# huggingface/distil-whisper

Measured on AMD Instinct MI355X. Metric: training audio-seconds/s (distil-large-v3 student, 30 s clips), higher is better.
Workload: dtype bf16

## Files before the change

### distil_whisper_amd/build.py

```python
import os
import subprocess
import sys

HERE = os.path.dirname(os.path.abspath(__file__))
CSRC = os.path.join(HERE, "csrc")
LIB = os.path.join(HERE, "libdwamd.so")
SOURCES = ["gemm.hip", "gemm_tile256.hip", "gemm_tile128.hip", "gemm_wp8_nn.hip", "gemm_wp8_nt.hip", "gemm_wp8_m320.hip", "gemm_wp8_m128.hip",
           "gemm_wp16_nn.hip", "gemm_wp16_tt.hip", "gemm_wp16_small.hip", "gemm_skinny.hip", "attention.hip", "norm.hip", "loss.hip", "logmel.hip", "elementwise.hip", "optim.hip", "decode.hip"]
FLAGS = ["--offload-arch=gfx950", "-O3", "-std=c++17", "-fPIC", "-ffp-contract=fast", "-munsafe-fp-atomics"]


def kernels_sha16() -> str:
    import hashlib
    h = hashlib.sha256()
    files = sorted(os.path.join(CSRC, f) for f in os.listdir(CSRC) if f.endswith((".hip", ".h")))
    files.append(os.path.join(HERE, "..", "include", "dwamd.h"))
    for f in files:
        h.update(os.path.basename(f).encode())
        with open(f, "rb") as fh:
            h.update(fh.read())
    return h.hexdigest()[:16]


def _stale(obj, deps):
    if not os.path.exists(obj):
        return True
    t = os.path.getmtime(obj)
    return any(os.path.getmtime(d) > t for d in deps)


def build(force: bool = False, verbose: bool = False) -> str:
    hipcc = os.environ.get("HIPCC", "/opt/rocm/bin/hipcc")
    objdir = os.path.join(HERE, "build")
    os.makedirs(objdir, exist_ok=True)
    headers = [os.path.join(CSRC, "common.h"), os.path.join(CSRC, "gemm_common.h"), os.path.join(CSRC, "gemm_kernel.h"), os.path.join(CSRC, "gemm_wp.h"), os.path.join(CSRC, "gemm_wp16.h"),
               os.path.join(HERE, "..", "include", "dwamd.h")]
    objs, procs = [], []
    flags = FLAGS + (["-DDW_ABLATE"] if os.environ.get("DW_ABLATE") else [])
    flags += os.environ.get("DW_EXTRA_FLAGS", "").split()
    for src in SOURCES:
        s = os.path.join(CSRC, src)
        o = os.path.join(objdir, src.replace(".hip", ".o"))
        objs.append(o)
        if force or _stale(o, [s] + headers):
            cmd = [hipcc] + flags + ["-c", s, "-o", o]
            if verbose:
                print(" ".join(cmd))
            procs.append((src, subprocess.Popen(cmd, stdout=subprocess.PIPE, stderr=subprocess.STDOUT)))
    for src, p in procs:
        out, _ = p.communicate()
        if p.returncode != 0:
            sys.stderr.write(out.decode())
            raise RuntimeError(f"hipcc failed on {src}")
    if force or procs or _stale(LIB, objs):
        cmd = [hipcc, "--offload-arch=gfx950", "-shared", "-fPIC", "-o", LIB] + objs
        subprocess.check_call(cmd)
    return LIB



if __name__ == "__main__":
    print(build(force="--force" in sys.argv, verbose=True))
```

### distil_whisper_amd/csrc/gemm.hip

```cpp
#include "gemm_common.h"
#include <mutex>
#include <unordered_map>

bool dw_gemm_skinny_ok(const GemmP& p, int trans_a, int trans_b);
int dw_gemm_skinny_launch(const GemmP& p, hipStream_t s);
int dw_gemm_tile256_launch(const GemmP& p, int ta, int tb, hipStream_t s);
int dw_gemm_tile128_launch(const GemmP& p, int ta, int tb, hipStream_t s);
int dw_gemm_wp8_nn_launch(const GemmP& p, hipStream_t s);
int dw_gemm_wp8_nt_launch(const GemmP& p, hipStream_t s);
int dw_gemm_wp8_nn320_launch(const GemmP& p, hipStream_t s);
int dw_gemm_wp8_nt320_launch(const GemmP& p, hipStream_t s);
int dw_gemm_wp8_nn128_launch(const GemmP& p, hipStream_t s);
int dw_gemm_wp8_nt128_launch(const GemmP& p, hipStream_t s);
int dw_gemm_wp16_nn_launch(const GemmP& p, hipStream_t s);
int dw_gemm_wp16_tt_launch(const GemmP& p, hipStream_t s);
int dw_gemm_wp16_nn_small_launch(const GemmP& p, hipStream_t s);
int dw_gemm_wp16_nt_small_launch(const GemmP& p, hipStream_t s);

extern int g_attn_bwd_stage;
extern int g_attn_decode;
extern int g_attn_ablate;
extern int g_attn_fwd_waves;
extern int g_attn_fwd_pipe;
extern int g_attn_plain_order;
extern int g_attn_defer;
extern int g_attn_bwd_waves;
extern int g_logmel_mfma;
extern int g_decode_fuse_off;
extern int g_skinny_wide;
extern int g_ln_variant;
enum { GEMM_RULE = 0,
       GEMM_REFERENCE = 1,
       GEMM_FORCE_320 = 2 };
static int g_gemm_mode = GEMM_RULE;
int g_gemm_strip = 0;
int g_gemm_cus = 256;
static int g_gemm_stage_next = 1;
static int g_gemm_dynamic = 1;
static int g_gemm_small_m = 1;
static int g_gemm_row_tail = 1;

static int* gemm_sched_slot(hipStream_t s) {
    static std::mutex mu;
    static std::unordered_map<hipStream_t, int*> slots;
    std::lock_guard<std::mutex> lock(mu);
    auto it = slots.find(s);
    if (it != slots.end()) return it->second;
    hipStreamCaptureStatus st = hipStreamCaptureStatusNone;
    if (hipStreamIsCapturing(s, &st) != hipSuccess || st != hipStreamCaptureStatusNone) { (void)hipGetLastError(); return nullptr; }
    int* ptr = nullptr;
    if (hipMalloc((void**)&ptr, 64) != hipSuccess || hipMemsetAsync(ptr, 0, 64, s) != hipSuccess) { (void)hipGetLastError(); return nullptr; }
    slots[s] = ptr;
    return ptr;
}
int g_gemm_strip_budget = 4;
extern "C" int dw_debug_set(int key, int value) {
    if (key == 0) { if (value < GEMM_RULE || value > GEMM_FORCE_320) return DW_EINVAL; g_gemm_mode = value; return DW_OK; }
    if (key == 1) { g_gemm_strip = value; return DW_OK; }
    if (key == 3) { g_attn_bwd_stage = value; return DW_OK; }
    if (key == 4) { g_attn_decode = value; return DW_OK; }
    if (key == 5) { g_logmel_mfma = value; return DW_OK; }
    if (key == 6) { g_gemm_strip_budget = value; return DW_OK; }
    if (key == 7) { g_decode_fuse_off = value; return DW_OK; }
    if (key == 8) { g_skinny_wide = value; return DW_OK; }
    if (key == 10) { g_gemm_dynamic = value; return DW_OK; }
    if (key == 11) { g_gemm_stage_next = value; return DW_OK; }
    if (key == 17) { g_attn_bwd_waves = value; return DW_OK; }
    if (key == 21) { g_ln_variant = value; return DW_OK; }
    if (key == 22) { g_gemm_row_tail = value; return DW_OK; }
    if (key == 25) { if (value < 0 || value > 1) return DW_EINVAL; g_gemm_small_m = value; return DW_OK; }
    if (key == 26) { g_attn_fwd_pipe = value; return DW_OK; }
    if (key == 18) { g_attn_plain_order = value; return DW_OK; }
    if (key == 23) { if (value < 0 || value > 64) return DW_EINVAL; g_attn_defer = value; return DW_OK; }
    if (key == 16) { g_attn_fwd_waves = value; return DW_OK; }
    if (key == 15) { g_attn_ablate = value; return DW_OK; }
    if (key == 9) { if (value < 8 || value > 256 || (value & 7)) return DW_EINVAL; g_gemm_cus = value; return DW_OK; }
    return DW_EINVAL;
}

__global__ __launch_bounds__(256) void reduce_slices_kernel(const float* part, long stride, int slices, float* out,
                                                            long n, int accumulate) {
    const long i = ((long)blockIdx.x * 256 + threadIdx.x) * 4;
    if (i >= n) return;
    f32x4 acc = accumulate ? *(const f32x4*)(out + i) : f32x4{0.f, 0.f, 0.f, 0.f};
    for (int s = 0; s < slices; ++s) {
        const f32x4 v = *(const f32x4*)(part + s * stride + i);
#pragma unroll
        for (int e = 0; e < 4; ++e) acc[e] += v[e];
    }
    *(f32x4*)(out + i) = acc;
}

extern "C" int dw_reduce_slices(const float* part, int64_t stride, int slices, float* out, int64_t n, int accumulate,
                                void* stream) {
    DW_CLEAR_ERR();
    if (!part || !out || slices < 1 || n <= 0 || (n & 3) || (stride & 3) || ((uintptr_t)part & 15) ||
        ((uintptr_t)out & 15))
        return DW_EINVAL;
    hipLaunchKernelGGL(reduce_slices_kernel, dim3((n / 4 + 255) / 256), dim3(256), 0, (hipStream_t)stream, part,
                       (long)stride, slices, out, (long)n, accumulate);
    DW_CHECK_LAUNCH();
    return DW_OK;
}

__global__ __launch_bounds__(256) void reduce_slices_ld_kernel(const float* part, long slice_stride, long ld_part, int slices,
                                                               float* out, long ld_out, int rows, int cols4, int accumulate) {
    const long i = (long)blockIdx.x * 256 + threadIdx.x;
    if (i >= (long)rows * cols4) return;
    const int r = (int)(i / cols4), c = (int)(i - (long)r * cols4) * 4;
    float* o = out + (long)r * ld_out + c;
    f32x4 acc = accumulate ? *(const f32x4*)o : f32x4{0.f, 0.f, 0.f, 0.f};
    const float* src = part + (long)r * ld_part + c;
    for (int s = 0; s < slices; ++s) {
        const f32x4 v = *(const f32x4*)(src + s * slice_stride);
#pragma unroll
        for (int e = 0; e < 4; ++e) acc[e] += v[e];
    }
    *(f32x4*)o = acc;
}
extern "C" int dw_reduce_slices_ld(const float* part, int64_t slice_stride, int64_t ld_part, int slices, float* out, int64_t ld_out,
                                   int rows, int cols, int accumulate, void* stream) {
    DW_CLEAR_ERR();
    if (!part || !out || slices < 1 || rows <= 0 || cols <= 0 || (cols & 3) || (ld_part & 3) || (ld_out & 3) || (slice_stride & 3) ||
        ld_part < cols || ld_out < cols || ((uintptr_t)part & 15) || ((uintptr_t)out & 15))
        return DW_EINVAL;
    const long n = (long)rows * (cols / 4);
    hipLaunchKernelGGL(reduce_slices_ld_kernel, dim3((n + 255) / 256), dim3(256), 0, (hipStream_t)stream, part, (long)slice_stride,
                       (long)ld_part, slices, out, (long)ld_out, rows, cols / 4, accumulate);
    DW_CHECK_LAUNCH();
    return DW_OK;
}

enum GemmKernel {
    K_SKINNY,
    K_TILE128,
    K_TILE256,
    K_WP8_M128,
    K_WP16_SMALL,
    K_WP8_320,
    K_WP16_NN,
    K_WP8_NN,
    K_WP8_NT,
    K_WP16_TT,
};

static GemmKernel gemm_choose(const DwGemm* g, const GemmP& p) {
    const bool ta = g->trans_a, tb = g->trans_b, nn = !ta && !tb;
    const bool one_slice = p.split_k == 1 && !p.atomic;
    const bool ref = g_gemm_mode == GEMM_REFERENCE;
    const bool res_f32 = g->r && g->r_dtype == DW_F32 && g->c_dtype == DW_F32;
    const long cus = g_gemm_cus, tn = (g->n + 255) / 256;
    const long t256 = (long)((g->m + 255) / 256) * tn;
    const bool fits320 = !ta && one_slice && g->m % 320 == 0 && g->n % 256 == 0;
    int tile = g->tile;
    if ((tile == 0 || tile == 16) && dw_gemm_skinny_ok(p, ta, tb)) return K_SKINNY;
    bool one_round_320 = false, small_m_256 = false;
    if (tile != 128 && tile != 256) {
        tile = t256 >= 512 ? 256 : 128;
        if (tile == 128 && !ref && g_gemm_small_m && !ta && one_slice) {
            const long r128 = (((long)(g->m + 127) / 128) * tn + cus - 1) / cus;
            const long r256 = (t256 + cus - 1) / cus;
            const long r320 = fits320 ? ((long)(g->m / 320) * tn + cus - 1) / cus : 0;
            const long c128 = r128 * 100, c256 = r256 * 165, c320 = fits320 ? r320 * 205 : (1L << 40);
            if (c320 <= c128 && c320 <= c256) { tile = 256; one_round_320 = true; }
            else if (c256 <= c128) { tile = 256; small_m_256 = true; }
            else return K_WP8_M128;
        }
    }
    if (tile == 256 && g->tile != 256 && nn && res_f32 && g->k <= 1024 && one_slice) tile = 128;
    if (tile == 128) return K_TILE128;
    const long spanA = ta ? (long)g->k * g->lda * 2 : 256L * g->lda * 2 + (long)g->k * 2;
    const long spanB = tb ? (long)g->k * g->ldb * 2 : 256L * g->ldb * 2 + (long)g->k * 2;
    if (ref || spanA >= 0x7fffffffL || spanB >= 0x7fffffffL) return K_TILE256;
    if (small_m_256) return K_WP16_SMALL;
    if (fits320 && (one_round_320 || g_gemm_mode == GEMM_FORCE_320)) return K_WP8_320;
    if (nn && g->k <= 2560 && g->n >= 3840 && !g->r && !g->z_out && !g->zgrad_in && g->c_dtype != DW_F32) return K_WP16_NN;
    if (fits320) {
        const long r256 = (((g->m + 255) / 256) * tn + cus - 1) / cus * 4;
        const long r320 = ((g->m / 320) * tn + cus - 1) / cus * 5;
        if (tb ? r320 < r256 && !g->zgrad_in : r320 <= r256) return K_WP8_320;
    }
    if (nn) return res_f32 && g->k <= 2560 ? K_TILE256 : K_WP8_NN;
    if (!ta) return K_WP8_NT;
    if (tb) return K_WP16_TT;
    return K_TILE256;
}

extern "C" int dw_gemm_bf16(const DwGemm* g, void* stream) {
    DW_CLEAR_ERR();
    if (!g || (!g->a && !g->ln_x) || !g->b || !g->c) return DW_EINVAL;
    if (g->m <= 0 || g->n <= 0 || g->k <= 0 || (g->k & 63)) return DW_EINVAL;
    if ((g->lda & 7) || (g->ldb & 7)) return DW_EINVAL;
    if ((g->a && ((uintptr_t)g->a & 15)) || ((uintptr_t)g->b & 15)) return DW_EINVAL;
    if (g->trans_a && g->lda < ((g->m + 7) & ~7)) return DW_EINVAL;
    if (g->trans_b && g->ldb < ((g->n + 7) & ~7)) return DW_EINVAL;
    GemmP p;
    p.a = (const bf16*)g->a; p.b = (const bf16*)g->b; p.c = g->c; p.bias = g->bias;
    p.z_out = (bf16*)g->z_out; p.zgrad = (const bf16*)g->zgrad_in; p.r = g->r;
    p.lda = g->lda; p.ldb = g->ldb; p.ldc = g->ldc; p.ldz = g->ldz; p.ldzg = g->ldzg; p.ldr = g->ldr;
    p.m = g->m; p.n = g->n; p.k = g->k;
    p.act = g->act; p.c_dtype = g->c_dtype; p.r_dtype = g->r_dtype; p.r_row_mod = g->r_row_mod;
    p.round_res = g->round_res; p.tiles_n = 0; p.nwg = 0;
    p.split_k = g->split_k > 1 ? g->split_k : 1;
    p.atomic = g->atomic_acc ? 1 : 0;
    if (p.split_k > (g->k >> 6)) p.split_k = g->k >> 6;
    p.slice_stride = 0;
    p.sched = nullptr;
    p.zg_f16 = g->z_is_gelu_grad ? 1 : 0;
    p.colsum = g->colsum_out;
    if (g->colsum_out && (g->split_k > 1 || g->atomic_acc || ((uintptr_t)g->colsum_out & 3))) return DW_EINVAL;
    p.stage_next = g_gemm_stage_next;
    if (p.zg_f16 && g->z_out && g->act != 1) return DW_EINVAL;
    p.ln_x = g->ln_x; p.ln_g = g->ln_gamma; p.ln_b = g->ln_beta; p.ld_lnx = g->ld_lnx; p.ln_x_dtype = g->ln_x_dtype;
    p.ln_eps = g->ln_eps;
    p.kv_out = (bf16*)g->kv_out; p.kv_ld = g->kv_ld; p.kv_split = g->kv_split; p.kv_rpb = g->kv_rows_per_batch;
    p.kv_pitch = g->kv_batch_pitch; p.kv_row0 = g->kv_row0;
    const bool fused = g->ln_x || g->kv_out;
    if (g->ln_x && (!g->ln_gamma || !g->ln_beta || g->k > 1280 || g->m > 32 || (g->ld_lnx & 7) ||
                    ((uintptr_t)g->ln_x & 15) || ((uintptr_t)g->ln_gamma & 15) || ((uintptr_t)g->ln_beta & 15)))
        return DW_EINVAL;
    if (g->kv_out && (g->c_dtype != DW_BF16 || g->act || g->r || g->z_out || g->zgrad_in || (g->kv_split & 15) ||
                      g->kv_split <= 0 || g->kv_split >= g->n || g->kv_rows_per_batch <= 0 || (g->kv_ld & 3) ||
                      ((uintptr_t)g->kv_out & 7)))
        return DW_EINVAL;
    if (p.split_k > 1 && !p.atomic) {
        if (g->c_dtype != DW_F32 || g->bias || g->z_out || g->zgrad_in || g->r || g->act || g->slice_stride <= 0)
            return DW_EINVAL;
        p.slice_stride = g->slice_stride;
    }
    if (p.atomic && (g->c_dtype != DW_F32 || g->bias || g->z_out || g->zgrad_in || g->r || g->act)) return DW_EINVAL;
    {
        const int es = g->c_dtype == DW_F32 ? 4 : 2;
        bool v = ((uintptr_t)g->c % (4 * es)) == 0 && (g->ldc & 3) == 0;
        if (g->bias) v = v && ((uintptr_t)g->bias & 15) == 0;
        if (g->z_out) v = v && ((uintptr_t)g->z_out & 7) == 0 && (g->ldz & 3) == 0;
        if (g->zgrad_in) v = v && ((uintptr_t)g->zgrad_in & 7) == 0 && (g->ldzg & 3) == 0;
        if (g->r) v = v && ((uintptr_t)g->r % (g->r_dtype == DW_F32 ? 16 : 8)) == 0 && (g->ldr & 3) == 0;
        p.vec = v ? 1 : 0;
    }
    hipStream_t s = (hipStream_t)stream;
    if (g->tile == 16 && !dw_gemm_skinny_ok(p, g->trans_a, g->trans_b)) return DW_EINVAL;
    const GemmKernel kern = gemm_choose(g, p);
    if (kern == K_SKINNY) {
        if (g->colsum_out) return DW_EINVAL;
        return dw_gemm_skinny_launch(p, s);
    }
    if (fused) return DW_EINVAL;
    if (g->tile == 129 && (g->trans_a || p.split_k != 1 || p.atomic)) return DW_EINVAL;
    if (kern == K_TILE128) return dw_gemm_tile128_launch(p, g->trans_a, g->trans_b, s);
    p.strip = g_gemm_strip;
    if (g_gemm_dynamic) p.sched = gemm_sched_slot(s);
    if (kern == K_WP8_M128) return g->trans_b ? dw_gemm_wp8_nt128_launch(p, s) : dw_gemm_wp8_nn128_launch(p, s);
    if (g->k <= 1024) p.stage_next |= 128;
    switch (kern) {
    case K_WP16_SMALL: return g->trans_b ? dw_gemm_wp16_nt_small_launch(p, s) : dw_gemm_wp16_nn_small_launch(p, s);
    case K_WP8_320: return g->trans_b ? dw_gemm_wp8_nt320_launch(p, s) : dw_gemm_wp8_nn320_launch(p, s);
    case K_WP8_NN: return dw_gemm_wp8_nn_launch(p, s);
    case K_WP8_NT: return dw_gemm_wp8_nt_launch(p, s);
    case K_WP16_TT: return dw_gemm_wp16_tt_launch(p, s);
    case K_WP16_NN: {
        const int tm_full = p.m / 256, rem = p.m - tm_full * 256;
        const long tn = (p.n + 255) / 256;
        const long rounds_all = ((long)(tm_full + 1) * tn + g_gemm_cus - 1) / g_gemm_cus;
        const long rounds_full = ((long)tm_full * tn + g_gemm_cus - 1) / g_gemm_cus;
        if (g_gemm_row_tail && g->tile != 256 && rem > 0 && rem <= 128 && tm_full > 0 && rounds_full < rounds_all && !p.colsum) {
            GemmP q1 = p, q2 = p;
            q1.m = tm_full * 256;
            const size_t es = p.c_dtype == DW_F32 ? 4 : 2;
            q2.m = rem;
            q2.a = p.a + (long)q1.m * p.lda;
            q2.c = (char*)p.c + (size_t)q1.m * p.ldc * es;
            q2.sched = nullptr;
            const int rc1 = dw_gemm_wp16_nn_launch(q1, s);
            if (rc1 != DW_OK) return rc1;
            return dw_gemm_tile128_launch(q2, 0, 0, s);
        }
        return dw_gemm_wp16_nn_launch(p, s);
    }
    default: return dw_gemm_tile256_launch(p, g->trans_a, g->trans_b, s);
    }
}
```

### distil_whisper_amd/csrc/gemm_common.h

```cpp
#pragma once
#include "common.h"
#include "../../include/dwamd.h"

struct GemmP {
    const bf16* a;
    const bf16* b;
    void* c;
    const float* bias;
    bf16* z_out;
    const bf16* zgrad;
    const void* r;
    long lda, ldb, ldc, ldz, ldzg, ldr;
    int m, n, k;
    int act, c_dtype, r_dtype, r_row_mod, round_res;
    int tiles_n, nwg;
    int strip;
    int split_k, atomic;
    int vec;
    long slice_stride;
    const void* ln_x;
    const float* ln_g;
    const float* ln_b;
    long ld_lnx;
    int ln_x_dtype;
    float ln_eps;
    bf16* kv_out;
    long kv_ld;
    int kv_split, kv_rpb, kv_pitch, kv_row0;
    int stage_next;
    int zg_f16;
    int* sched;
    float* colsum;
};

__device__ __forceinline__ void gemm_job_range(const GemmP& p, int& job_first, int& job_count, int& job_step) {
    const int total = p.nwg * p.split_k;
    const int bid = blockIdx.x;
    const int xcd = bid & 7, local = bid >> 3;
    const int q = total >> 3, r = total & 7;
    if ((int)gridDim.x == total) {
        job_first = (xcd < r ? xcd * (q + 1) : r * (q + 1) + (xcd - r) * q) + local;
        job_count = 1;
        job_step = 1;
    } else {
        const int start = xcd < r ? xcd * (q + 1) : r * (q + 1) + (xcd - r) * q;
        const int cnt = q + (xcd < r ? 1 : 0);
        job_step = gridDim.x >> 3;
        job_first = start + local;
        job_count = local < cnt ? (cnt - local + job_step - 1) / job_step : 0;
    }
}

struct GemmJobs {
    int start, cnt;
    int step, local;
    int cur;
    int iter;
    bool dynamic;
};
__device__ __forceinline__ int gemm_jobs_fetch(const GemmP& p) {
    return __hip_atomic_fetch_add(p.sched + (blockIdx.x & 7), 1, __ATOMIC_RELAXED, __HIP_MEMORY_SCOPE_AGENT);
}
__device__ __forceinline__ void gemm_jobs_begin(const GemmP& p, GemmJobs& J, int* slot) {
    const int total = p.nwg * p.split_k;
    const int bid = blockIdx.x;
    const int xcd = bid & 7;
    const int q = total >> 3, r = total & 7;
    J.start = xcd < r ? xcd * (q + 1) : r * (q + 1) + (xcd - r) * q;
    J.iter = 0;
    if ((int)gridDim.x == total) {
        J.cnt = q + (xcd < r ? 1 : 0);
        J.local = bid >> 3; J.step = J.cnt > 0 ? J.cnt : 1; J.cur = J.local; J.dynamic = false;
        J.cnt = J.local < J.cnt ? J.local + 1 : 0;
        return;
    }
    J.cnt = q + (xcd < r ? 1 : 0);
    J.step = gridDim.x >> 3;
    J.local = bid >> 3;
    J.dynamic = p.sched != nullptr;
    if (J.dynamic) {
        if (threadIdx.x == 0) slot[0] = gemm_jobs_fetch(p);
        __syncthreads();
        J.cur = slot[0];
    } else {
        J.cur = J.local;
    }
}
__device__ __forceinline__ void gemm_jobs_prefetch(const GemmP& p, GemmJobs& J, int* slot) {
    if (J.dynamic && threadIdx.x == 0) slot[(J.iter + 1) & 1] = gemm_jobs_fetch(p);
}
__device__ __forceinline__ void gemm_jobs_advance(GemmJobs& J, const int* slot) {
    ++J.iter;
    J.cur = J.dynamic ? slot[J.iter & 1] : J.cur + J.step;
}
__device__ __forceinline__ void gemm_jobs_end(const GemmP& p, const GemmJobs& J) {
    if (J.dynamic && threadIdx.x == 0) {
        const int done = __hip_atomic_fetch_add(p.sched + 8, 1, __ATOMIC_RELAXED, __HIP_MEMORY_SCOPE_AGENT);
        if (done == (int)gridDim.x - 1) {
#pragma unroll
            for (int i = 0; i < 9; ++i) __hip_atomic_store(p.sched + i, 0, __ATOMIC_RELAXED, __HIP_MEMORY_SCOPE_AGENT);
        }
    }
}

__device__ __forceinline__ void gemm_job_decode(const GemmP& p, int id, int& tm, int& tn, int& ks) {
    ks = id / p.nwg;
    id -= ks * p.nwg;
    const int tiles_m = p.nwg / p.tiles_n;
    const int nstrips = (p.tiles_n + p.strip - 1) / p.strip;
    const int sw = (p.tiles_n + nstrips - 1) / nstrips;
    const int per_strip = sw * tiles_m;
    int strip = id / per_strip;
    int within = id - strip * per_strip;
    int width = sw;
    const int full = p.tiles_n - (nstrips - 1) * sw;
    if (strip >= nstrips - 1) {
        strip = nstrips - 1;
        within = id - strip * per_strip;
        width = full;
    }
    tm = within / width;
    tn = strip * sw + (within - tm * width);
}

extern int g_gemm_strip_budget;
extern int g_gemm_cus;
inline int gemm_strip_width(int k, int tiles_n, int override_) {
    if (override_ > 0) return override_;
    const long tile_bytes = 256L * k * 2;
    int sw = (int)(((long)g_gemm_strip_budget << 19) / tile_bytes);
    if (sw < 2 || sw >= tiles_n) sw = tiles_n;
    return sw;
}

template <int BX>
__device__ __forceinline__ bf16x8 frag_kmajor(const char* tile, int x, int kk, int lane) {
    constexpr int RB = BX * 2;
    const int g = lane >> 4, p = lane & 15;
    const int col = x + ((g & 1) << 4) + ((p & 3) << 2);
    const int k0 = kk * 16 + ((g >> 1) << 3) + (p >> 2);
    const int ls = col >> 3;
    const int inb = (p & 1) << 3;
    const int sw = ((p >> 2) & 3) << 2;
    const char* a0 = tile + k0 * RB + ((ls ^ sw) << 4) + inb;
    const char* a1 = a0 + 4 * RB;
    bf16x4 lo = __builtin_amdgcn_ds_read_tr16_b64_v4bf16((lds_bf16x4_t*)a0);
    bf16x4 hi = __builtin_amdgcn_ds_read_tr16_b64_v4bf16((lds_bf16x4_t*)a1);
    bf16x8 r;
    r[0] = lo[0]; r[1] = lo[1]; r[2] = lo[2]; r[3] = lo[3];
    r[4] = hi[0]; r[5] = hi[1]; r[6] = hi[2]; r[7] = hi[3];
    return r;
}


typedef __attribute__((ext_vector_type(4))) unsigned u32x4;
enum { EPI_BIAS = 1, EPI_ZBF16 = 2, EPI_GELU = 4, EPI_STOREG = 8, EPI_ZG16 = 16, EPI_ZGBF = 32, EPI_RES = 64, EPI_RES_F32 = 128,
       EPI_ROUND = 256, EPI_OUT_F32 = 512, EPI_COLSUM = 1024 };
__device__ __forceinline__ int gemm_epi_flavour(const GemmP& p) {
    return (p.bias ? EPI_BIAS : 0) | ((p.z_out && !p.zg_f16) ? EPI_ZBF16 : 0) | (p.act == 1 ? EPI_GELU : 0) |
           ((p.z_out && p.zg_f16) ? EPI_STOREG : 0) | ((p.zgrad && p.zg_f16) ? EPI_ZG16 : 0) |
           ((p.zgrad && !p.zg_f16) ? EPI_ZGBF : 0) | (p.r ? EPI_RES : 0) | ((p.r && p.r_dtype == DW_F32) ? EPI_RES_F32 : 0) |
           ((p.r && p.round_res) ? EPI_ROUND : 0) | (p.c_dtype == DW_F32 ? EPI_OUT_F32 : 0) | (p.colsum ? EPI_COLSUM : 0);
}
template <class T>
__device__ __forceinline__ void gemm_store_out(T* dst, const T& v) {
    __builtin_nontemporal_store(v, dst);
}
template <int F = -1>
__device__ __forceinline__ void gemm_epi_vec4(const GemmP& p, float (&v)[4], const f32x4& b4, bool plain, bool have_side,
                                              const bf16x4& zs, const f32x4& rs, char* cdst, char* zdst, float (&cs)[4]) {
    constexpr bool RT = F < 0;
    const bool any = RT ? !plain : (F & ~(EPI_OUT_F32 | EPI_COLSUM)) != 0;
    const bool colsum = RT ? p.colsum != nullptr : bool(F & EPI_COLSUM);
    if (any) {
        if (RT || (F & EPI_BIAS)) {
#pragma unroll
            for (int e = 0; e < 4; ++e) v[e] += b4[e];
        }
        if (RT ? (p.z_out && !p.zg_f16) : bool(F & EPI_ZBF16)) {
            bf16x4 z4;
#pragma unroll
            for (int e = 0; e < 4; ++e) z4[e] = f2bf(v[e]);
            gemm_store_out((bf16x4*)zdst, z4);
        }
        if (RT ? p.act == 1 : bool(F & EPI_GELU)) {
            const bool store_g = RT ? (p.z_out && p.zg_f16) : bool(F & EPI_STOREG);
            f16x4 g4;
#pragma unroll
            for (int e = 0; e < 4; e += 2) {
                f32x2 vin; vin[0] = v[e]; vin[1] = v[e + 1];
                const f32x2 x2 = round_bf16_pair(vin);
                f32x2 y2, s2, pdf;
                gelu_y_s_pdf2(x2, y2, s2, pdf);
                v[e] = y2[0]; v[e + 1] = y2[1];
                if (store_g) {
                    const f32x2 g2 = gelu_cdf_from_s2(x2, s2) + x2 * pdf;
                    g4[e] = (_Float16)g2[0]; g4[e + 1] = (_Float16)g2[1];
                }
            }
            if (store_g) gemm_store_out((f16x4*)zdst, g4);
        }
        if (RT ? have_side : (F & (EPI_ZG16 | EPI_ZGBF | EPI_RES)) != 0) {
            if (RT ? (p.zgrad && p.zg_f16) : bool(F & EPI_ZG16)) {
                const f16x4 g4 = __builtin_bit_cast(f16x4, zs);
#pragma unroll
                for (int e = 0; e < 4; ++e) v[e] *= (float)g4[e];
            } else if (RT ? p.zgrad != nullptr : bool(F & EPI_ZGBF)) {
#pragma unroll
                for (int e = 0; e < 4; e += 2) {
                    f32x2 x2; x2[0] = bf2f(zs[e]); x2[1] = bf2f(zs[e + 1]);
                    const f32x2 g2 = gelu_grad_fast2(x2);
                    v[e] *= g2[0]; v[e + 1] *= g2[1];
                }
            }
            if (RT ? p.r != nullptr : bool(F & EPI_RES)) {
                float rv[4];
                if (RT ? p.r_dtype == DW_F32 : bool(F & EPI_RES_F32)) {
#pragma unroll
                    for (int e = 0; e < 4; ++e) rv[e] = rs[e];
                } else {
                    const unsigned u0 = __float_as_uint(rs[0]), u1 = __float_as_uint(rs[1]);
                    rv[0] = __uint_as_float(u0 << 16); rv[1] = __uint_as_float(u0 & 0xffff0000u);
                    rv[2] = __uint_as_float(u1 << 16); rv[3] = __uint_as_float(u1 & 0xffff0000u);
                }
                const bool rnd = RT ? p.round_res != 0 : bool(F & EPI_ROUND);
#pragma unroll
                for (int e = 0; e < 4; ++e) v[e] = (rnd ? round_bf16(v[e]) : v[e]) + rv[e];
            }
        }
    }
    if (RT ? p.c_dtype == DW_F32 : bool(F & EPI_OUT_F32)) {
        f32x4 o;
#pragma unroll
        for (int e = 0; e < 4; ++e) o[e] = v[e];
        *(f32x4*)cdst = o;
        if (colsum) {
#pragma unroll
            for (int e = 0; e < 4; ++e) cs[e] += v[e];
        }
    } else {
        bf16x4 o;
#pragma unroll
        for (int e = 0; e < 4; ++e) o[e] = f2bf(v[e]);
        gemm_store_out((bf16x4*)cdst, o);
        if (colsum) {
#pragma unroll
            for (int e = 0; e < 4; ++e) cs[e] += bf2f(o[e]);
        }
    }
}

template <int LPR>
__device__ __forceinline__ void gemm_colsum_flush(const GemmP& p, float (&cs)[4], int lane, int n) {
#pragma unroll
    for (int e = 0; e < 4; ++e) {
#pragma unroll
        for (int o = LPR; o < 64; o <<= 1) cs[e] += __shfl_xor(cs[e], o);
    }
    if (lane < LPR) {
#pragma unroll
        for (int e = 0; e < 4; ++e)
            if (n + e < p.n) atomicAdd(p.colsum + n + e, cs[e]);
    }
}

struct GemmNoHook { __device__ __forceinline__ void operator()() const {} };
__device__ __forceinline__ void gemm_lds_barrier() {
    asm volatile("s_waitcnt lgkmcnt(0)" ::: "memory");
    __builtin_amdgcn_s_barrier();
    asm volatile("" ::: "memory");
}
template <int FM, int FN, int TN, int PFDIST = 0, class Hook = GemmNoHook, bool SWZ = false, int LAY = 32, int JOFF = 0, class Acc = f32x16[FM][FN]>
__device__ __forceinline__ void gemm_epilogue(const GemmP& p, Acc& acc, char* smem, int wave, int lane,
                                              int m0_, int wm0_, int n0_, int wn0_, int ks_, Hook hook = Hook(),
                                              const float* lds_bias = nullptr) {
    static_assert(!SWZ || TN == 64, "swizzled patch: 16 slots of 16 bytes per row");
    asm volatile("" : "+v"(lane));
    const int m0 = __builtin_amdgcn_readfirstlane(m0_), wm0 = __builtin_amdgcn_readfirstlane(wm0_);
    const int n0 = __builtin_amdgcn_readfirstlane(n0_), wn0 = __builtin_amdgcn_readfirstlane(wn0_);
    const int ks = __builtin_amdgcn_readfirstlane(ks_);
    constexpr int PLD = SWZ ? TN : TN + 4;
    constexpr int LPR = TN / 4;
    constexpr int RPI = 64 / LPR;
    constexpr int NIT = 32 / RPI;
    float* patch = (float*)smem + wave * (32 * PLD);
    const int hi = lane >> 5, ln = lane & 31;
    const int lrow = LAY == 32 ? ln : (lane & 15);
    const int lcol = LAY == 32 ? hi * 4 : (lane >> 4) * 4;
    auto qrow = [](int q) constexpr -> int { return LAY == 32 ? 0 : (q / (FN * 2)) * 16; };
    auto qcol = [](int q) constexpr -> int { return LAY == 32 ? (q / 4) * 32 + (q % 4) * 8 : (q % (FN * 2)) * 16; };
    auto quad = [&](auto ic, auto qc) __attribute__((always_inline)) -> f32x4 {
        constexpr int i = decltype(ic)::value, q = decltype(qc)::value;
        f32x4 v4;
        if constexpr (LAY == 32) {
            constexpr int j = q / 4, g = q % 4;
            v4[0] = acc[i][j][g * 4 + 0]; v4[1] = acc[i][j][g * 4 + 1]; v4[2] = acc[i][j][g * 4 + 2]; v4[3] = acc[i][j][g * 4 + 3];
        } else {
            constexpr int h = q / (FN * 2), j = q % (FN * 2);
            v4 = acc[2 * i + h][j + JOFF];
        }
        return v4;
    };
    const bool plain = !p.bias && !p.z_out && p.act == 0 && !p.zgrad && !p.r;
    float* const cf = (float*)p.c + (long)ks * p.slice_stride;
    const int pr = lane / LPR, pc = (lane % LPR) * 4;
    const int n = n0 + wn0 + pc;
    const bool n_in = n < p.n;
    const bool full = p.vec && n + 3 < p.n;
    const bool interior = p.vec && !p.atomic && p.r_row_mod <= 0 && n0 + wn0 + TN <= p.n && m0 + wm0 + FM * 32 <= p.m;
    f32x4 b4 = {0.f, 0.f, 0.f, 0.f};
    if (p.bias && lds_bias && interior) b4 = *(const f32x4*)(lds_bias + wn0 + pc);
    else if (p.bias && n_in) {
        if (full) b4 = *(const f32x4*)(p.bias + n);
        else {
#pragma unroll
            for (int e = 0; e < 4; ++e) if (n + e < p.n) b4[e] = p.bias[n + e];
        }
    }
    auto to_patch = [&](auto ic) __attribute__((always_inline)) {
        int l2 = lane;
        asm volatile("" : "+v"(l2));
        const int lrow2 = LAY == 32 ? (l2 & 31) : (l2 & 15), lcol2 = LAY == 32 ? (l2 >> 5) * 4 : (l2 >> 4) * 4;
        static_for<0, FN * 4>([&](auto qc) __attribute__((always_inline)) {
            constexpr int q = decltype(qc)::value;
            const f32x4 v4 = quad(ic, qc);
            const int row = lrow2 + qrow(q), col = lcol2 + qcol(q);
            if constexpr (SWZ) *(f32x4*)(patch + row * PLD + (((col >> 2) ^ (row & 15)) << 2)) = v4;
            else *(f32x4*)(patch + row * PLD + col) = v4;
        });
    };

    if (interior) {
        const bool pf_z = p.zgrad != nullptr, pf_r = p.r != nullptr;
        constexpr int PFD = PFDIST > 0 ? (PFDIST < NIT ? PFDIST : NIT) : NIT;
        const int es_c = p.c_dtype == DW_F32 ? 4 : 2;
// ... 263 lines not shown
```

### distil_whisper_amd/csrc/gemm_wp.h

```cpp
#pragma once
#include "gemm_common.h"

#define PINF(f) asm volatile("" : "+v"((f)[0]), "+v"((f)[1]), "+v"((f)[2]), "+v"((f)[3]))
#define PINF2(f) asm volatile("" : "+v"((f)[0]), "+v"((f)[1]))
#define PIN_SET(set)                                                                                              \
    do {          \
        if constexpr (FM == 4 && FN == 2)                                                                                 \
            asm volatile("" : "+v"(af[set][0]), "+v"(af[set][1]), "+v"(af[set][2]), "+v"(af[set][3]), "+v"(bfr[set][0]), "+v"(bfr[set][1]));   \
        else if constexpr (FM == 5 && FN == 2)                                                                            \
            asm volatile("" : "+v"(af[set][0]), "+v"(af[set][1]), "+v"(af[set][2]), "+v"(af[set][3]), "+v"(af[set][4]), "+v"(bfr[set][0]),     \
                         "+v"(bfr[set][1]));                                                                              \
        else {                                                                                                            \
            if constexpr (FM == 4) PINF(af[set]);                                                                         \
            else if constexpr (FM == 5) { PINF(af[set]); asm volatile("" : "+v"(af[set][4])); }                          \
            else PINF2(af[set]);                                                                                          \
            if constexpr (FN == 4) PINF(bfr[set]); else PINF2(bfr[set]);                                                  \
        }                                                                                                                 \
    } while (0)

typedef __attribute__((ext_vector_type(4))) int i32x4_t;
__device__ __forceinline__ i32x4_t wp_rsrc(const void* base) {
    const unsigned long long a = (unsigned long long)base;
    i32x4_t r;
    r[0] = (int)(unsigned)a; r[1] = (int)((unsigned)(a >> 32) & 0xffffu); r[2] = 0x7fffffff; r[3] = 0x00020000;
    return r;
}
__device__ __forceinline__ void wp_dma16(const i32x4_t& rsrc, const char* lds_dst, unsigned voffset, int soffset) {
    const unsigned m0v = __builtin_amdgcn_readfirstlane((unsigned)(unsigned long long)(const lds_void_t*)lds_dst);
    asm volatile("s_mov_b32 m0, %0\n\ts_nop 0\n\tbuffer_load_dwordx4 %1, %2, %3 offen lds"
                 :: "s"(m0v), "v"(voffset), "s"(rsrc), "s"(soffset));
}
__device__ __forceinline__ unsigned wp_lds_addr(const void* lds_ptr) {
    return __builtin_amdgcn_readfirstlane((unsigned)(unsigned long long)(const lds_void_t*)lds_ptr);
}
__device__ __forceinline__ void wp_dma16u(const i32x4_t& rsrc, unsigned lds_addr, unsigned voffset, int soffset) {
    asm volatile("s_mov_b32 m0, %0\n\ts_nop 0\n\tbuffer_load_dwordx4 %1, %2, %3 offen lds"
                 :: "s"(lds_addr), "v"(voffset), "s"(rsrc), "s"(soffset));
}
template <int IMM>
__device__ __forceinline__ void wp_dma16p(const i32x4_t& rsrc, unsigned lds_base, unsigned voffset, int kbase, int piece_off) {
    int so;
    asm volatile("s_add_u32 m0, %1, %5\n\ts_add_u32 %0, %4, %6\n\tbuffer_load_dwordx4 %2, %3, %0 offen lds"
                 : "=&s"(so) : "s"(lds_base), "v"(voffset), "s"(rsrc), "s"(kbase), "i"(IMM), "s"(piece_off) : "scc");
}
template <int IMM>
__device__ __forceinline__ void wp_dma16i(const i32x4_t& rsrc, unsigned lds_base, unsigned voffset, int soffset) {
    asm volatile("s_add_u32 m0, %0, %4\n\ts_nop 0\n\tbuffer_load_dwordx4 %1, %2, %3 offen lds"
                 :: "s"(lds_base), "v"(voffset), "s"(rsrc), "s"(soffset), "i"(IMM) : "scc");
}

template <bool TA, bool TB, int WM, int WN, bool ASMDMA, int DBG, int BM, int NST>
__global__ __launch_bounds__(64 * WM * WN, WM * WN / 4) void gemm_wp_kernel(const GemmP p) {
    static_assert(ASMDMA && DBG == 0, "one build of the loop: inline-assembly operand DMA, no ablation");
    constexpr int BN = 256, NW = WM * WN, FM = BM / WM / 32, FN = BN / WN / 32, TN = BN / WN;
    static_assert(NST == 2 || (NST == 3 && BM < 256), "three stages: the 128-row tile");
    static_assert(NW * 32 * (TN + 4) * 4 <= 2 * (BM + BN) * 128, "epilogue patches must fit the operand buffers");
    static_assert(BM == 256 || !TA, "the k-major A image is built for 256-row tiles");
    constexpr int CPA = BM / 8 / NW, CPB = BN / 8 / NW;
    constexpr int CP = CPB;
    constexpr bool UNI = BM == 320;
    constexpr int EPF = 4;
    static_assert(CPA * 8 * NW == BM && CPB * 8 * NW == BN && CPA <= 8 && CPB <= 8, "piece split");
    constexpr int NA0 = (CPA + 1) / 2, NB0 = CPB / 2;
    constexpr int NH0 = NA0 + NB0, NH1 = CPA + CPB - NH0;
    constexpr int STAGE = (BM + BN) * 128;
    __shared__ __attribute__((aligned(1024))) char smem[NST * STAGE];
    __shared__ __attribute__((aligned(1024))) float bias_lds[BN];

    const int tid = threadIdx.x;
    const int lane = tid & 63;
    const int wave = __builtin_amdgcn_readfirstlane(tid >> 6);
    const int wm0 = (wave / WN) * (BM / WM), wn0 = (wave % WN) * TN;
    const unsigned smem_w = wp_lds_addr(smem) + (unsigned)(wave * 1024);

    __shared__ int job_slot[2];
    GemmJobs jobs;
    gemm_jobs_begin(p, jobs, job_slot);
    bool prefetched = false;
    while (jobs.cur < jobs.cnt) {
        int lane_k = lane;
        asm volatile("" : "+v"(lane_k));
        gemm_jobs_prefetch(p, jobs, job_slot);
        int tm, tn, ks;
        gemm_job_decode(p, jobs.start + jobs.cur, tm, tn, ks);
        const int m0 = tm * BM, n0 = tn * BN;

        unsigned offA[8], offB[8];
        const bf16* gA;
        const bf16* gB;
        int stepA, stepB;
        if (!TA) {
            gA = p.a + (long)m0 * p.lda;
            stepA = 128;
#pragma unroll
            for (int i = 0; i < CPA; ++i) {
                const int row = (wave + i * NW) * 8 + (lane_k >> 3);
                const int ls = (lane_k & 7) ^ swz7(row);
                const int grow = m0 + row < p.m ? row : p.m - 1 - m0;
                offA[i] = (unsigned)((grow * p.lda + ls * 8) * 2);
            }
        } else {
            gA = p.a + m0;
            stepA = 128 * (int)p.lda;
#pragma unroll
            for (int i = 0; i < CPA; ++i) {
                const int krow = (wave + i * NW) * 2 + (lane_k >> 5);
                const int ls = (lane_k & 31) ^ ((krow & 3) << 2);
                const int gcol = m0 + ls * 8 < p.m ? ls * 8 : 0;
                offA[i] = (unsigned)((krow * p.lda + gcol) * 2);
            }
        }
        if (!TB) {
            gB = p.b + (long)n0 * p.ldb;
            stepB = 128;
#pragma unroll
            for (int i = 0; i < CP; ++i) {
                const int row = (wave + i * NW) * 8 + (lane_k >> 3);
                const int ls = (lane_k & 7) ^ swz7(row);
                const int grow = n0 + row < p.n ? row : p.n - 1 - n0;
                offB[i] = (unsigned)((grow * p.ldb + ls * 8) * 2);
            }
        } else {
            gB = p.b + n0;
            stepB = 128 * (int)p.ldb;
#pragma unroll
            for (int i = 0; i < CP; ++i) {
                const int krow = (wave + i * NW) * 2 + (lane_k >> 5);
                const int ls = (lane_k & 31) ^ ((krow & 3) << 2);
                const int gcol = n0 + ls * 8 < p.n ? ls * 8 : 0;
                offB[i] = (unsigned)((krow * p.ldb + gcol) * 2);
            }
        }
        const int pieceA = UNI ? NW * (TA ? 2 : 8) * (int)p.lda * 2 : 0;
        const int pieceB = UNI ? NW * (TB ? 2 : 8) * (int)p.ldb * 2 : 0;
        int nt = p.k >> 6;
        {
            const int base = nt / p.split_k, rem = nt - base * p.split_k;
            const int first = ks * base + (ks < rem ? ks : rem);
            nt = base + (ks < rem ? 1 : 0);
            gA = (const bf16*)((const char*)gA + (long)first * stepA);
            gB = (const bf16*)((const char*)gB + (long)first * stepB);
        }
        const i32x4_t rsA = wp_rsrc(gA), rsB = wp_rsrc(gB);
        int kA = 0, kB = 0;

        f32x16 acc[FM][FN];
#pragma unroll
        for (int i = 0; i < FM; ++i)
#pragma unroll
            for (int j = 0; j < FN; ++j)
#pragma unroll
                for (int r = 0; r < 16; ++r) acc[i][j][r] = 0.f;

        auto dma1x = [&](const i32x4_t& ra, const i32x4_t& rb, auto hc, auto jc, int buf) __attribute__((always_inline)) {
            constexpr int h = decltype(hc)::value, j = decltype(jc)::value;
            constexpr int na = h ? CPA - NA0 : NA0, nb = h ? CPB - NB0 : NB0, nmin = na < nb ? na : nb;
            constexpr bool isA = j < 2 * nmin ? (j & 1) == 0 : na > nb;
            constexpr int idx = j < 2 * nmin ? j / 2 : j - nmin;
            constexpr int i = (isA ? (h ? NA0 : 0) : (h ? NB0 : 0)) + idx;
            static_assert(j < na + nb, "load index");
            const unsigned lb = smem_w + (unsigned)(buf * STAGE);
            if constexpr (UNI) {
                if constexpr (isA) wp_dma16p<i * (NW * 1024)>(ra, lb, offA[0], kA, i * pieceA);
                else wp_dma16p<i * (NW * 1024) + BM * 128>(rb, lb, offB[0], kB, i * pieceB);
            } else {
                if constexpr (isA) wp_dma16i<i * (NW * 1024)>(ra, lb, offA[i], kA);
                else wp_dma16i<i * (NW * 1024) + BM * 128>(rb, lb, offB[i], kB);
            }
        };
        auto dma1 = [&](auto hc, auto jc, int buf) __attribute__((always_inline)) { dma1x(rsA, rsB, hc, jc, buf); };
        auto dma = [&](auto hc, int buf) __attribute__((always_inline)) {
            static_for<0, (decltype(hc)::value ? NH1 : NH0)>([&](auto jc) __attribute__((always_inline)) { dma1(hc, jc, buf); });
        };
        bf16x8 af[2][FM], bfr[2][FN];
        auto frags = [&](auto sc, auto kc, int buf) {
            constexpr int set = decltype(sc)::value, kk = decltype(kc)::value;
            const char* tA = smem + buf * STAGE;
            const char* tB = tA + BM * 128;
#pragma unroll
            for (int i = 0; i < FM; ++i) {
                if (TA) af[set][i] = frag_kmajor<BM>(tA, wm0 + i * 32, kk, lane_k);
                else af[set][i] = frag_rows(tA, (wm0 >> 5) + i, kk, lane_k);
            }
#pragma unroll
            for (int j = 0; j < FN; ++j) {
                if (TB) bfr[set][j] = frag_kmajor<BN>(tB, wn0 + j * 32, kk, lane_k);
                else bfr[set][j] = frag_rows(tB, (wn0 >> 5) + j, kk, lane_k);
            }
        };
        auto mfma1 = [&](auto sc, auto qc) __attribute__((always_inline)) {
            constexpr int set = decltype(sc)::value, i = decltype(qc)::value / FN, j = decltype(qc)::value % FN;
            acc[i][j] = __builtin_amdgcn_mfma_f32_32x32x16_bf16(bfr[set][j], af[set][i], acc[i][j], 0, 0, 0);
        };
        auto substep = [&](auto sc, auto rc, auto vhc, int dbuf) __attribute__((always_inline)) {
            constexpr bool R = decltype(rc)::value != 0;
            constexpr int VH = decltype(vhc)::value;
            constexpr int NMF = FM * FN;
            constexpr int DSI = FM * (TA ? 2 : 1) + FN * (TB ? 2 : 1);
            constexpr int RG = VH ? NMF / 4 : NMF / 2;
            constexpr int PER = (DSI + RG - 1) / RG;
            constexpr int NLD = VH == 1 ? NH0 : NH1;
            static_assert(VH == 0 || RG + NLD <= NMF, "not enough MFMA gaps for the operand loads");
            static_for<0, RG>([&](auto qc) __attribute__((always_inline)) { mfma1(sc, qc); });
#pragma unroll
            for (int q = 0; q < RG; ++q) {
                __builtin_amdgcn_sched_group_barrier(0x8, 1, 0);
                if (R) __builtin_amdgcn_sched_group_barrier(0x100, PER, 0);
            }
            __builtin_amdgcn_sched_barrier(0);
            if constexpr (VH != 0) {
                static_for<0, NLD>([&](auto jc) __attribute__((always_inline)) {
                    mfma1(sc, std::integral_constant<int, RG + decltype(jc)::value>{});
                    dma1(std::integral_constant<int, VH - 1>{}, jc, dbuf);
                    __builtin_amdgcn_sched_barrier(0);
                });
                static_for<RG + NLD, NMF>([&](auto qc) __attribute__((always_inline)) { mfma1(sc, qc); });
            } else {
                static_for<RG, NMF>([&](auto qc) __attribute__((always_inline)) { mfma1(sc, qc); });
            }
            __builtin_amdgcn_sched_barrier(0);
        };
        using I0 = std::integral_constant<int, 0>;
        using I1 = std::integral_constant<int, 1>;
        using I2 = std::integral_constant<int, 2>;
        using I3 = std::integral_constant<int, 3>;

        const bool tile_in = m0 + BM <= p.m && n0 + BN <= p.n;
        if (p.bias && tile_in && wave == 0) glds16_so(p.bias + n0, (unsigned)lane_k * 16u, lds_addr_of(bias_lds));
        if constexpr (NST == 3) {
            dma(I0{}, 0); dma(I1{}, 0);
            kA += stepA; kB += stepB;
            if (nt > 1) { dma(I0{}, 1); dma(I1{}, 1); kA += stepA; kB += stepB; }
            if (nt > 2) dma(I0{}, 2);
            if (nt > 2) asm volatile("s_waitcnt vmcnt(%0)" :: "n"(2 * NH0 + NH1) : "memory");
            else if (nt > 1) asm volatile("s_waitcnt vmcnt(%0)" :: "n"(NH0 + NH1) : "memory");
            else wait_vm0();
            __syncthreads();
            frags(I0{}, I0{}, 0);
            __builtin_amdgcn_sched_barrier(0);
            auto body3 = [&](auto m1c, auto m2c, auto m3c, int b0, int b1, int b2) {
                constexpr bool M1 = decltype(m1c)::value, M2 = decltype(m2c)::value, M3 = decltype(m3c)::value;
                PIN_SET(0);
                frags(I1{}, I1{}, b0);
                if constexpr (M2) { substep(I0{}, I1{}, I2{}, b2); kA += stepA; kB += stepB; }
                else substep(I0{}, I1{}, I0{}, 0);
                PIN_SET(1);
                frags(I0{}, I2{}, b0);
                substep(I1{}, I1{}, I0{}, 0);
                PIN_SET(0);
                frags(I1{}, I3{}, b0);
                substep(I0{}, I1{}, I0{}, 0);
                PIN_SET(1);
                if constexpr (M1) {
                    if constexpr (M2) asm volatile("s_waitcnt vmcnt(%0)" :: "n"(NH0 + NH1) : "memory");
                    else wait_vm0();
                    __builtin_amdgcn_s_barrier();
                    __builtin_amdgcn_sched_barrier(0);
                }
                if constexpr (M1) frags(I0{}, I0{}, b1);
                if constexpr (M3) substep(I1{}, I1{}, I1{}, b0);
                else if constexpr (M1) substep(I1{}, I1{}, I0{}, 0);
                else substep(I1{}, I0{}, I0{}, 0);
            };
            int t = 0, b0 = 0, b1 = 1, b2 = 2;
            auto rot = [&]() { const int x = b0; b0 = b1; b1 = b2; b2 = x; ++t; };
            for (; t + 3 < nt; rot()) body3(std::true_type{}, std::true_type{}, std::true_type{}, b0, b1, b2);
            if (nt >= 3) { body3(std::true_type{}, std::true_type{}, std::false_type{}, b0, b1, b2); rot(); }
            if (nt >= 2) { body3(std::true_type{}, std::false_type{}, std::false_type{}, b0, b1, b2); rot(); }
            body3(std::false_type{}, std::false_type{}, std::false_type{}, b0, b1, b2);
        } else {
        if (!prefetched) { dma(I0{}, 0); dma(I1{}, 0); }
        kA += stepA; kB += stepB;
        if (nt > 1) dma(I0{}, 1);
        if (nt > 1) {
            if constexpr (NH0 == 8) asm volatile("s_waitcnt vmcnt(8)" ::: "memory");
            else if constexpr (NH0 == 5) asm volatile("s_waitcnt vmcnt(5)" ::: "memory");
            else if constexpr (NH0 == 3) asm volatile("s_waitcnt vmcnt(3)" ::: "memory");
            else { static_assert(NH0 == 4 || NH0 == 8 || NH0 == 5 || NH0 == 3, "vmcnt immediate"); asm volatile("s_waitcnt vmcnt(4)" ::: "memory"); }
        } else wait_vm0();
        __syncthreads();
        frags(I0{}, I0{}, 0);
        __builtin_amdgcn_sched_barrier(0);

        auto body = [&](auto m1c, auto m2c, int t) {
            constexpr bool MORE1 = decltype(m1c)::value, MORE2 = decltype(m2c)::value;
            const int buf = t & 1;
            PIN_SET(0);
            frags(I1{}, I1{}, buf);
            if constexpr (MORE1) { substep(I0{}, I1{}, I2{}, buf ^ 1); kA += stepA; kB += stepB; }
            else substep(I0{}, I1{}, I0{}, 0);
            PIN_SET(1);
            frags(I0{}, I2{}, buf);
            substep(I1{}, I1{}, I0{}, 0);
            PIN_SET(0);
            frags(I1{}, I3{}, buf);
            substep(I0{}, I1{}, I0{}, 0);
            PIN_SET(1);
            if constexpr (MORE1) {
                wait_vm0();
                __builtin_amdgcn_s_barrier();
                __builtin_amdgcn_sched_barrier(0);
            }
            if constexpr (MORE1) frags(I0{}, I0{}, buf ^ 1);
            if constexpr (MORE2) substep(I1{}, I1{}, I1{}, buf);
            else if constexpr (MORE1) substep(I1{}, I1{}, I0{}, 0);
            else substep(I1{}, I0{}, I0{}, 0);
        };
        int t = 0;
        for (; t + 2 < nt; ++t) body(std::true_type{}, std::true_type{}, t);
        if (nt >= 2) { body(std::true_type{}, std::false_type{}, t); ++t; }
        body(std::false_type{}, std::false_type{}, t);
        }

        prefetched = false;
        if constexpr (TN == 64 && BM >= 256) {
            const int nxt = jobs.dynamic ? job_slot[(jobs.iter + 1) & 1] : jobs.cur + jobs.step;
            if ((p.stage_next & 128) && (nt & 1) == 0 && nt >= 2 && nxt < jobs.cnt && tile_in && !p.zgrad && !p.r) {
                int tm2, tn2, ks2;
                gemm_job_decode(p, jobs.start + nxt, tm2, tn2, ks2);
                if ((tm2 + 1) * BM <= p.m && (tn2 + 1) * BN <= p.n) {
                    const int ntall = p.k >> 6, base2 = ntall / p.split_k, rem2 = ntall - base2 * p.split_k;
                    const long first2 = (long)ks2 * base2 + (ks2 < rem2 ? ks2 : rem2);
                    const char* a2 = (const char*)(TA ? p.a + tm2 * BM : p.a + (long)tm2 * BM * p.lda) + first2 * stepA;
                    const char* b2 = (const char*)(TB ? p.b + tn2 * BN : p.b + (long)tn2 * BN * p.ldb) + first2 * stepB;
                    const i32x4_t ra2 = wp_rsrc(a2), rb2 = wp_rsrc(b2);
                    kA = 0; kB = 0;
                    static_for<0, NH0>([&](auto jc) __attribute__((always_inline)) { dma1x(ra2, rb2, I0{}, jc, 0); });
                    static_for<0, NH1>([&](auto jc) __attribute__((always_inline)) { dma1x(ra2, rb2, I1{}, jc, 0); });
                    prefetched = true;
                }
            }
        }
        gemm_epilogue<FM, FN, TN, (BM == 320 ? EPF : 8), GemmNoHook, TN == 64>(p, acc, smem + (TN == 64 && STAGE >= NW * 8192 ? STAGE : 0), wave, lane, m0,
                                                                          wm0, n0, wn0, ks, GemmNoHook(), tile_in ? bias_lds : nullptr);
        gemm_lds_barrier();
        gemm_jobs_advance(jobs, job_slot);
    }
    gemm_jobs_end(p, jobs);
}

template <bool TA, bool TB, int WM, int WN, int BM = 256, int NST = 2>
static int launch_wp(const GemmP& p0, hipStream_t s) {
    GemmP p = p0;
    const int tiles_m = (p.m + BM - 1) / BM;
    p.tiles_n = (p.n + 255) / 256;
    p.nwg = tiles_m * p.tiles_n;
    p.strip = gemm_strip_width(p.k, p.tiles_n, p.strip);
    int nblk = p.nwg * p.split_k;
    if (nblk > g_gemm_cus) nblk = g_gemm_cus;
    hipLaunchKernelGGL((gemm_wp_kernel<TA, TB, WM, WN, true, 0, BM, NST>), dim3(nblk), dim3(64 * WM * WN), 0, s, p);
    DW_CHECK_LAUNCH();
    return DW_OK;
}
```

### distil_whisper_amd/csrc/norm.hip

```cpp
#include "common.h"
#include "../../include/dwamd.h"

#define LN_MAXV 8
#ifndef DW_NT_LN_IN
#define DW_NT_LN_IN 1
#endif

template <bool XBF>
__device__ __forceinline__ f32x4 ld4b(const void* x, long off) {
    if constexpr (DW_NT_LN_IN >= 2) {
        if (XBF) {
            const bf16x4 t = __builtin_nontemporal_load((const bf16x4*)((const bf16*)x + off));
            f32x4 r; r[0] = bf2f(t[0]); r[1] = bf2f(t[1]); r[2] = bf2f(t[2]); r[3] = bf2f(t[3]);
            return r;
        } else return __builtin_nontemporal_load((const f32x4*)((const float*)x + off));
    } else {
        if (XBF) {
            const bf16x4 t = *(const bf16x4*)((const bf16*)x + off);
            f32x4 r; r[0] = bf2f(t[0]); r[1] = bf2f(t[1]); r[2] = bf2f(t[2]); r[3] = bf2f(t[3]);
            return r;
        } else return *(const f32x4*)((const float*)x + off);
    }
}
template <bool XBF>
__device__ __forceinline__ f32x4 ld4(const void* x, long off) {
    if (XBF) {
        const bf16x4 t = *(const bf16x4*)((const bf16*)x + off);
        f32x4 r; r[0] = bf2f(t[0]); r[1] = bf2f(t[1]); r[2] = bf2f(t[2]); r[3] = bf2f(t[3]);
        return r;
    } else {
        return *(const f32x4*)((const float*)x + off);
    }
}

#ifndef DW_NT_LN
#define DW_NT_LN 0
#endif
template <class T>
__device__ __forceinline__ T ln_load_in(const T* src) {
    if constexpr (DW_NT_LN_IN != 0) return __builtin_nontemporal_load(src);
    else return *src;
}
template <int LEVEL, class T>
__device__ __forceinline__ void ln_store(T* dst, const T& v) {
    if constexpr (LEVEL <= DW_NT_LN) __builtin_nontemporal_store(v, dst);
    else *dst = v;
}

template <bool XBF, int NV>
__global__ __launch_bounds__(256) void ln_fwd_kernel(const void* x, const float* gamma, const float* beta, bf16* y,
                                                     float* mean, float* rstd, int rows, int cols, float eps, long ldx, long ldy) {
    const int lane = threadIdx.x & 63;
    const int row = blockIdx.x * 4 + (threadIdx.x >> 6);
    if (row >= rows) return;
    const int nvec = cols >> 2;
    f32x4 v[NV];
    float s = 0.f;
#pragma unroll
    for (int j = 0; j < NV; ++j) {
        const int idx = lane + 64 * j;
        if (idx < nvec) {
            v[j] = ld4<XBF>(x, (long)row * ldx + idx * 4);
            s += v[j][0] + v[j][1] + v[j][2] + v[j][3];
        }
    }
    s = wave_sum(s);
    const float mu = s / cols;
    float q = 0.f;
#pragma unroll
    for (int j = 0; j < NV; ++j) {
        const int idx = lane + 64 * j;
        if (idx < nvec) {
#pragma unroll
            for (int e = 0; e < 4; ++e) { const float d = v[j][e] - mu; q += d * d; }
        }
    }
    q = wave_sum(q);
    const float rs = rsqrtf(q / cols + eps);
#pragma unroll
    for (int j = 0; j < NV; ++j) {
        const int idx = lane + 64 * j;
        if (idx < nvec) {
            const f32x4 g = *(const f32x4*)(gamma + idx * 4);
            const f32x4 bt = *(const f32x4*)(beta + idx * 4);
            bf16x4 o;
#pragma unroll
            for (int e = 0; e < 4; ++e) o[e] = f2bf((v[j][e] - mu) * rs * g[e] + bt[e]);
            ln_store<1>((bf16x4*)(y + (long)row * ldy + idx * 4), o);
        }
    }
    if (lane == 0 && mean) { mean[row] = mu; rstd[row] = rs; }
}

template <int NV>
__global__ __launch_bounds__(256) void ln_fwd_persist_kernel(const float* x, const float* gamma, const float* beta, bf16* y,
                                                             float* mean, float* rstd, int rows, int cols, float eps, long ldx, long ldy) {
    const int lane = threadIdx.x & 63;
    const int nvec = cols >> 2;
    const int stride = gridDim.x * 4;
    int row = blockIdx.x * 4 + (threadIdx.x >> 6);
    if (row >= rows) return;
    f32x4 v[NV], nx[NV];
#pragma unroll
    for (int j = 0; j < NV; ++j) {
        const int idx = lane + 64 * j;
        if (idx < nvec) v[j] = ln_load_in((const f32x4*)(x + (long)row * ldx + idx * 4));
    }
    for (; row < rows; row += stride) {
        const int nrow = row + stride;
        if (nrow < rows) {
#pragma unroll
            for (int j = 0; j < NV; ++j) {
                const int idx = lane + 64 * j;
                if (idx < nvec) nx[j] = ln_load_in((const f32x4*)(x + (long)nrow * ldx + idx * 4));
            }
        }
        float s = 0.f;
#pragma unroll
        for (int j = 0; j < NV; ++j)
            if (lane + 64 * j < nvec) s += v[j][0] + v[j][1] + v[j][2] + v[j][3];
        s = wave_sum(s);
        const float mu = s / cols;
        float q = 0.f;
#pragma unroll
        for (int j = 0; j < NV; ++j)
            if (lane + 64 * j < nvec) {
#pragma unroll
                for (int e = 0; e < 4; ++e) { const float d = v[j][e] - mu; q += d * d; }
            }
        q = wave_sum(q);
        const float rs = rsqrtf(q / cols + eps);
#pragma unroll
        for (int j = 0; j < NV; ++j) {
            const int idx = lane + 64 * j;
            if (idx < nvec) {
                const f32x4 g = *(const f32x4*)(gamma + idx * 4);
                const f32x4 bt = *(const f32x4*)(beta + idx * 4);
                bf16x4 o;
#pragma unroll
                for (int e = 0; e < 4; ++e) o[e] = f2bf((v[j][e] - mu) * rs * g[e] + bt[e]);
                ln_store<1>((bf16x4*)(y + (long)row * ldy + idx * 4), o);
            }
        }
        if (lane == 0 && mean) { mean[row] = mu; rstd[row] = rs; }
#pragma unroll
        for (int j = 0; j < NV; ++j) v[j] = nx[j];
    }
}

template <int NV8>
__global__ __launch_bounds__(256) void ln_fwd_bf16x8_kernel(const bf16* x, const float* gamma, const float* beta, bf16* y,
                                                            float* mean, float* rstd, int rows, int cols, float eps, long ldx, long ldy) {
    const int lane = threadIdx.x & 63;
    const int row = blockIdx.x * 4 + (threadIdx.x >> 6);
    if (row >= rows) return;
    const int nvec = cols >> 3;
    float v[NV8][8];
    float s = 0.f;
#pragma unroll
    for (int j = 0; j < NV8; ++j) {
        const int idx = lane + 64 * j;
        if (idx < nvec) {
            const bf16x8 t = ln_load_in((const bf16x8*)(x + (long)row * ldx + idx * 8));
#pragma unroll
            for (int e = 0; e < 8; ++e) { v[j][e] = bf2f(t[e]); s += v[j][e]; }
        }
    }
    s = wave_sum(s);
    const float mu = s / cols;
    float q = 0.f;
#pragma unroll
    for (int j = 0; j < NV8; ++j) {
        const int idx = lane + 64 * j;
        if (idx < nvec) {
#pragma unroll
            for (int e = 0; e < 8; ++e) { const float d = v[j][e] - mu; q += d * d; }
        }
    }
    q = wave_sum(q);
    const float rs = rsqrtf(q / cols + eps);
#pragma unroll
    for (int j = 0; j < NV8; ++j) {
        const int idx = lane + 64 * j;
        if (idx < nvec) {
            const f32x4 g0 = *(const f32x4*)(gamma + idx * 8), g1 = *(const f32x4*)(gamma + idx * 8 + 4);
            const f32x4 b0 = *(const f32x4*)(beta + idx * 8), b1 = *(const f32x4*)(beta + idx * 8 + 4);
            bf16x8 o;
#pragma unroll
            for (int e = 0; e < 4; ++e) {
                o[e] = f2bf((v[j][e] - mu) * rs * g0[e] + b0[e]);
                o[e + 4] = f2bf((v[j][e + 4] - mu) * rs * g1[e] + b1[e]);
            }
            ln_store<1>((bf16x8*)(y + (long)row * ldy + idx * 8), o);
        }
    }
    if (lane == 0 && mean) { mean[row] = mu; rstd[row] = rs; }
}

template <bool XBF, int NV, int NW>
__global__ __launch_bounds__(NW * 64) void ln_bwd_kernel(const bf16* dy, const void* x, const float* mean,
                                                     const float* rstd, const float* gamma, float* dres,
                                                     int accumulate, float* dgamma, float* dbeta, bf16* dres_lowp,
                                                     float* dres_colsum, int rows, int cols, long lddy, long ldx, long lddres,
                                                         long ldlowp) {
    __shared__ float red[3 * NW * 512];
    const int lane = threadIdx.x & 63;
    const int wave = threadIdx.x >> 6;
    const int nvec = cols >> 2;
    f32x4 gm[NV], ag[NV], ab[NV], ac[NV];
#pragma unroll
    for (int j = 0; j < NV; ++j) {
        const int idx = lane + 64 * j;
#pragma unroll
        for (int e = 0; e < 4; ++e) { ag[j][e] = 0.f; ab[j][e] = 0.f; gm[j][e] = 0.f; ac[j][e] = 0.f; }
        if (idx < nvec) gm[j] = *(const f32x4*)(gamma + idx * 4);
    }
    for (int row = blockIdx.x * NW + wave; row < rows; row += gridDim.x * NW) {
        const float mu = mean[row], rs = rstd[row];
        f32x4 xh[NV], g[NV];
        float c1 = 0.f, c2 = 0.f;
#pragma unroll
        for (int j = 0; j < NV; ++j) {
            const int idx = lane + 64 * j;
            if (idx < nvec) {
                const f32x4 xv = ld4b<XBF>(x, (long)row * ldx + idx * 4);
                const f32x4 dv = ld4b<true>(dy, (long)row * lddy + idx * 4);
#pragma unroll
                for (int e = 0; e < 4; ++e) {
                    xh[j][e] = (xv[e] - mu) * rs;
                    g[j][e] = dv[e] * gm[j][e];
                    c1 += g[j][e];
                    c2 += g[j][e] * xh[j][e];
                    ag[j][e] += dv[e] * xh[j][e];
                    ab[j][e] += dv[e];
                }
            }
        }
        c1 = wave_sum(c1) / cols;
        c2 = wave_sum(c2) / cols;
#pragma unroll
        for (int j = 0; j < NV; ++j) {
            const int idx = lane + 64 * j;
            if (idx < nvec) {
                float* dst = dres + (long)row * lddres + idx * 4;
                f32x4 o;
#pragma unroll
                for (int e = 0; e < 4; ++e) o[e] = rs * (g[j][e] - c1 - xh[j][e] * c2);
                if (accumulate) {
                    const f32x4 old = *(const f32x4*)dst;
#pragma unroll
                    for (int e = 0; e < 4; ++e) o[e] += old[e];
                }
                ln_store<2>((f32x4*)dst, o);
                if (dres_lowp) {
                    bf16x4 lo;
#pragma unroll
                    for (int e = 0; e < 4; ++e) { lo[e] = f2bf(o[e]); ac[j][e] += bf2f(lo[e]); }
                    ln_store<3>((bf16x4*)(dres_lowp + (long)row * ldlowp + idx * 4), lo);
                }
            }
        }
    }
    float* r0 = red;
    float* r1 = red + NW * 512;
    float* r2 = red + 2 * NW * 512;
    for (int base = 0; base < cols; base += 512) {
#pragma unroll
        for (int j = 0; j < NV; ++j) {
            const int idx = lane + 64 * j;
            const int col = idx * 4;
            if (idx < nvec && col >= base && col < base + 512) {
#pragma unroll
                for (int e = 0; e < 4; ++e) {
                    r0[wave * 512 + (col - base) + e] = ag[j][e];
                    r1[wave * 512 + (col - base) + e] = ab[j][e];
                    r2[wave * 512 + (col - base) + e] = ac[j][e];
                }
            }
        }
        __syncthreads();
        for (int cidx = threadIdx.x; cidx < 512 && base + cidx < cols; cidx += NW * 64) {
            float sg = 0.f, sb = 0.f, sc = 0.f;
#pragma unroll
            for (int w = 0; w < NW; ++w) { sg += r0[w * 512 + cidx]; sb += r1[w * 512 + cidx]; sc += r2[w * 512 + cidx]; }
            atomicAdd(dgamma + base + cidx, sg);
            atomicAdd(dbeta + base + cidx, sb);
            if (dres_colsum) atomicAdd(dres_colsum + base + cidx, sc);
        }
        __syncthreads();
    }
}

template <bool XBF, int NV, int NW>
__global__ __launch_bounds__(NW * 64) void ln_bwd_pf_kernel(const bf16* dy, const void* x, const float* mean,
                                                         const float* rstd, const float* gamma, float* dres,
                                                         int accumulate, float* dgamma, float* dbeta, bf16* dres_lowp,
                                                         float* dres_colsum, int rows, int cols, long lddy, long ldx, long lddres,
                                                         long ldlowp) {
    __shared__ float red[3 * NW * 512];
    const int lane = threadIdx.x & 63;
    const int wave = threadIdx.x >> 6;
    const int nvec = cols >> 2;
    f32x4 gm[NV], ag[NV], ab[NV], ac[NV];
#pragma unroll
    for (int j = 0; j < NV; ++j) {
        const int idx = lane + 64 * j;
#pragma unroll
        for (int e = 0; e < 4; ++e) { ag[j][e] = 0.f; ab[j][e] = 0.f; gm[j][e] = 0.f; ac[j][e] = 0.f; }
        if (idx < nvec) gm[j] = *(const f32x4*)(gamma + idx * 4);
    }
    const int stride = gridDim.x * NW;
    int row = blockIdx.x * NW + wave;
    f32x4 xv[NV], dv[NV];
    float mu = 0.f, rs = 0.f;
    if (row < rows) {
        mu = mean[row]; rs = rstd[row];
#pragma unroll
        for (int j = 0; j < NV; ++j) {
            const int idx = lane + 64 * j;
            if (idx < nvec) { xv[j] = ld4b<XBF>(x, (long)row * ldx + idx * 4); dv[j] = ld4b<true>(dy, (long)row * lddy + idx * 4); }
        }
    }
    for (; row < rows; row += stride) {
        const int nrow = row + stride;
        f32x4 old[NV], nxv[NV], ndv[NV];
        float nmu = 0.f, nrs = 0.f;
        if (accumulate) {
#pragma unroll
            for (int j = 0; j < NV; ++j) {
                const int idx = lane + 64 * j;
                if (idx < nvec) old[j] = *(const f32x4*)(dres + (long)row * lddres + idx * 4);
            }
        }
        if (nrow < rows) {
            nmu = mean[nrow]; nrs = rstd[nrow];
#pragma unroll
            for (int j = 0; j < NV; ++j) {
                const int idx = lane + 64 * j;
                if (idx < nvec) { nxv[j] = ld4b<XBF>(x, (long)nrow * ldx + idx * 4); ndv[j] = ld4b<true>(dy, (long)nrow * lddy + idx * 4); }
            }
        }
        f32x4 xh[NV], g[NV];
        float c1 = 0.f, c2 = 0.f;
#pragma unroll
        for (int j = 0; j < NV; ++j) {
            const int idx = lane + 64 * j;
            if (idx < nvec) {
#pragma unroll
                for (int e = 0; e < 4; ++e) {
                    xh[j][e] = (xv[j][e] - mu) * rs;
                    g[j][e] = dv[j][e] * gm[j][e];
                    c1 += g[j][e];
                    c2 += g[j][e] * xh[j][e];
                    ag[j][e] += dv[j][e] * xh[j][e];
                    ab[j][e] += dv[j][e];
                }
            }
        }
        c1 = wave_sum(c1) / cols;
        c2 = wave_sum(c2) / cols;
#pragma unroll
        for (int j = 0; j < NV; ++j) {
            const int idx = lane + 64 * j;
            if (idx < nvec) {
                float* dst = dres + (long)row * lddres + idx * 4;
                f32x4 o;
#pragma unroll
                for (int e = 0; e < 4; ++e) o[e] = rs * (g[j][e] - c1 - xh[j][e] * c2);
                if (accumulate) {
#pragma unroll
                    for (int e = 0; e < 4; ++e) o[e] += old[j][e];
                }
                ln_store<2>((f32x4*)dst, o);
                if (dres_lowp) {
                    bf16x4 lo;
#pragma unroll
                    for (int e = 0; e < 4; ++e) { lo[e] = f2bf(o[e]); ac[j][e] += bf2f(lo[e]); }
                    ln_store<3>((bf16x4*)(dres_lowp + (long)row * ldlowp + idx * 4), lo);
                }
            }
        }
        mu = nmu; rs = nrs;
#pragma unroll
        for (int j = 0; j < NV; ++j) { xv[j] = nxv[j]; dv[j] = ndv[j]; }
    }
    float* r0 = red;
    float* r1 = red + NW * 512;
    float* r2 = red + 2 * NW * 512;
    for (int base = 0; base < cols; base += 512) {
#pragma unroll
        for (int j = 0; j < NV; ++j) {
            const int idx = lane + 64 * j;
            const int col = idx * 4;
            if (idx < nvec && col >= base && col < base + 512) {
#pragma unroll
                for (int e = 0; e < 4; ++e) {
                    r0[wave * 512 + (col - base) + e] = ag[j][e];
                    r1[wave * 512 + (col - base) + e] = ab[j][e];
                    r2[wave * 512 + (col - base) + e] = ac[j][e];
                }
            }
        }
        __syncthreads();
        for (int cidx = threadIdx.x; cidx < 512 && base + cidx < cols; cidx += NW * 64) {
            float sg = 0.f, sb = 0.f, sc = 0.f;
#pragma unroll
            for (int w = 0; w < NW; ++w) { sg += r0[w * 512 + cidx]; sb += r1[w * 512 + cidx]; sc += r2[w * 512 + cidx]; }
            atomicAdd(dgamma + base + cidx, sg);
            atomicAdd(dbeta + base + cidx, sb);
            if (dres_colsum) atomicAdd(dres_colsum + base + cidx, sc);
        }
        __syncthreads();
    }
}

int g_ln_variant = 3;

extern "C" int dw_layernorm_fwd_ld(const void* x, int x_dtype, const float* gamma, const float* beta, void* y,
                                   float* mean, float* rstd, int rows, int cols, float eps, int64_t ldx_, int64_t ldy_, void* stream);
extern "C" int dw_layernorm_fwd(const void* x, int x_dtype, const float* gamma, const float* beta, void* y,
                                float* mean, float* rstd, int rows, int cols, float eps, void* stream) {
    return dw_layernorm_fwd_ld(x, x_dtype, gamma, beta, y, mean, rstd, rows, cols, eps, cols, cols, stream);
}
extern "C" int dw_layernorm_fwd_ld(const void* x, int x_dtype, const float* gamma, const float* beta, void* y,
                                   float* mean, float* rstd, int rows, int cols, float eps, int64_t ldx_, int64_t ldy_, void* stream) {
    DW_CLEAR_ERR();
    if (!x || !gamma || !beta || !y || rows <= 0 || cols <= 0 || (cols & 3) || cols > LN_MAXV * 256) return DW_EINVAL;
    if (ldx_ < cols || ldy_ < cols || (ldx_ & 3) || (ldy_ & 3)) return DW_EINVAL;
    const long ldx = ldx_, ldy = ldy_;
    if ((mean == nullptr) != (rstd == nullptr)) return DW_EINVAL;
    dim3 grid((rows + 3) / 4), block(256);
    hipStream_t s = (hipStream_t)stream;
    if (x_dtype == DW_BF16 && (cols & 7) == 0 && ((ldx | ldy) & 7) == 0 && ((uintptr_t)x & 15) == 0 && ((uintptr_t)y & 15) == 0 &&
        ((uintptr_t)gamma & 15) == 0 && ((uintptr_t)beta & 15) == 0) {
        const int nv8 = ((cols >> 3) + 63) / 64;
        if (nv8 <= 1) hipLaunchKernelGGL((ln_fwd_bf16x8_kernel<1>), grid, block, 0, s, (const bf16*)x, gamma, beta, (bf16*)y, mean, rstd, rows, cols, eps, ldx, ldy);
        else if (nv8 <= 2) hipLaunchKernelGGL((ln_fwd_bf16x8_kernel<2>), grid, block, 0, s, (const bf16*)x, gamma, beta, (bf16*)y, mean, rstd, rows, cols, eps, ldx, ldy);
        else if (nv8 <= 3) hipLaunchKernelGGL((ln_fwd_bf16x8_kernel<3>), grid, block, 0, s, (const bf16*)x, gamma, beta, (bf16*)y, mean, rstd, rows, cols, eps, ldx, ldy);
        else hipLaunchKernelGGL((ln_fwd_bf16x8_kernel<4>), grid, block, 0, s, (const bf16*)x, gamma, beta, (bf16*)y, mean, rstd, rows, cols, eps, ldx, ldy);
        DW_CHECK_LAUNCH();
        return DW_OK;
    }
    const int nv = ((cols >> 2) + 63) / 64;
    if ((g_ln_variant & 1) && x_dtype != DW_BF16 && nv <= 5 && rows >= 8192) {
        dim3 pg(256 * ((g_ln_variant >> 8) & 15 ? (g_ln_variant >> 8) & 15 : 5));
        hipLaunchKernelGGL((ln_fwd_persist_kernel<5>), pg, block, 0, s, (const float*)x, gamma, beta, (bf16*)y, mean, rstd, rows, cols, eps, ldx, ldy);
        DW_CHECK_LAUNCH();
        return DW_OK;
    }
#define LN_FWD(NVV)                                                                                                   \
    do {                                                                                                              \
        if (x_dtype == DW_BF16)                                                                                       \
            hipLaunchKernelGGL((ln_fwd_kernel<true, NVV>), grid, block, 0, s, x, gamma, beta, (bf16*)y, mean, rstd,   \
                               rows, cols, eps, ldx, ldy);                                                                      \
        else                                                                                                          \
            hipLaunchKernelGGL((ln_fwd_kernel<false, NVV>), grid, block, 0, s, x, gamma, beta, (bf16*)y, mean, rstd,  \
                               rows, cols, eps, ldx, ldy);                                                                      \
    } while (0)
    if (nv <= 2) LN_FWD(2); else if (nv <= 3) LN_FWD(3); else if (nv <= 5) LN_FWD(5); else LN_FWD(8);
#undef LN_FWD
    DW_CHECK_LAUNCH();
    return DW_OK;
}

extern "C" int dw_layernorm_bwd_ld(const void* dy, const void* x, int x_dtype, const float* mean, const float* rstd,
                                   const float* gamma, float* dres, int accumulate, float* dgamma, float* dbeta,
                                   void* dres_lowp, float* dres_colsum, int rows, int cols, int64_t lddy_, int64_t ldx_,
                                   int64_t lddres_, int64_t ldlowp_, void* stream);
extern "C" int dw_layernorm_bwd(const void* dy, const void* x, int x_dtype, const float* mean, const float* rstd,
                                const float* gamma, float* dres, int accumulate, float* dgamma, float* dbeta,
                                void* dres_lowp, float* dres_colsum, int rows, int cols, void* stream) {
    return dw_layernorm_bwd_ld(dy, x, x_dtype, mean, rstd, gamma, dres, accumulate, dgamma, dbeta, dres_lowp, dres_colsum, rows,
                               cols, cols, cols, cols, cols, stream);
}
extern "C" int dw_layernorm_bwd_ld(const void* dy, const void* x, int x_dtype, const float* mean, const float* rstd,
                                   const float* gamma, float* dres, int accumulate, float* dgamma, float* dbeta,
                                   void* dres_lowp, float* dres_colsum, int rows, int cols, int64_t lddy_, int64_t ldx_,
                                   int64_t lddres_, int64_t ldlowp_, void* stream) {
    DW_CLEAR_ERR();
    if (!dy || !x || !mean || !rstd || !gamma || !dres || !dgamma || !dbeta) return DW_EINVAL;
    if (rows <= 0 || cols <= 0 || (cols & 3) || cols > LN_MAXV * 256) return DW_EINVAL;
    if (lddy_ < cols || ldx_ < cols || lddres_ < cols || ldlowp_ < cols || ((lddy_ | ldx_ | lddres_ | ldlowp_) & 3)) return DW_EINVAL;
    const long lddy = lddy_, ldx = ldx_, lddres = lddres_, ldlowp = ldlowp_;
    hipStream_t s = (hipStream_t)stream;
    const int nv = ((cols >> 2) + 63) / 64;
#define LN_BWD(NVV, NWW)                                                                                              \
    do {                                                                                                              \
        int nb = (rows + NWW - 1) / NWW;                                                                              \
        const int resident = 256 * ((NVV <= 3 ? 16 : NVV <= 5 ? 12 : 4) / NWW);                                       \
        if (nb > resident) nb = resident;                                                                             \
        if (x_dtype == DW_BF16)                                                                                       \
            hipLaunchKernelGGL((ln_bwd_kernel<true, NVV, NWW>), dim3(nb), dim3(NWW * 64), 0, s, (const bf16*)dy, x,   \
                               mean, rstd, gamma, dres, accumulate, dgamma, dbeta, (bf16*)dres_lowp, dres_colsum,     \
                               rows, cols, lddy, ldx, lddres, ldlowp);                                                                           \
// ... 23 lines not shown
```

### distil_whisper_amd/engine.py

```python
from dataclasses import dataclass

import ctypes as C

import torch


@dataclass
class WhisperDims:
    d_model: int
    heads: int
    ffn: int
    enc_layers: int
    dec_layers: int
    vocab: int
    n_mels: int
    max_src: int = 1500
    max_tgt: int = 448
    pad_token_id: int = 50256
    decoder_start_token_id: int = 50257

    @staticmethod
    def from_any(c):
        if isinstance(c, WhisperDims):
            return c
        if hasattr(c, "encoder_attention_heads"):
            return WhisperDims(c.d_model, c.encoder_attention_heads, c.encoder_ffn_dim, c.encoder_layers,
                               c.decoder_layers, c.vocab_size, c.num_mel_bins, c.max_source_positions,
                               c.max_target_positions, c.pad_token_id, c.decoder_start_token_id)
        return WhisperDims(c.d_model, c.heads, c.ffn, c.enc_layers, c.dec_layers, c.vocab, c.n_mels, c.max_src,
                           c.max_tgt, c.pad_token_id, c.decoder_start_token_id)


def _rup(x, m):
    return (x + m - 1) // m * m


def layer_names(prefix, cross):
    blocks = ["self_attn", "encoder_attn"] if cross else ["self_attn"]
    out = []
    for b in blocks:
        out += [(f"{prefix}.{b}.q_proj.weight", "w"), (f"{prefix}.{b}.k_proj.weight", "w"),
                (f"{prefix}.{b}.v_proj.weight", "w"), (f"{prefix}.{b}.q_proj.bias", "b"),
                (f"{prefix}.{b}.k_proj.bias", "zero"), (f"{prefix}.{b}.v_proj.bias", "b"),
                (f"{prefix}.{b}.out_proj.weight", "w"), (f"{prefix}.{b}.out_proj.bias", "b"),
                (f"{prefix}.{b}_layer_norm.weight", "ln"), (f"{prefix}.{b}_layer_norm.bias", "ln")]
    out += [(f"{prefix}.fc1.weight", "w"), (f"{prefix}.fc1.bias", "b"), (f"{prefix}.fc2.weight", "w"),
            (f"{prefix}.fc2.bias", "b"), (f"{prefix}.final_layer_norm.weight", "ln"),
            (f"{prefix}.final_layer_norm.bias", "ln")]
    return out


class ParamStore:

    def __init__(self, ops, dims: WhisperDims, state_dict, trainable=False, frozen_prefixes=(), round_bf16=False):
        self.ops, self.dims, self.trainable = ops, dims, trainable
        D, Fd = dims.d_model, dims.ffn
        spec = [("model.encoder.conv1.weight", (D, dims.n_mels, 3), "conv"), ("model.encoder.conv1.bias", (D,), "b"),
                ("model.encoder.conv2.weight", (D, D, 3), "conv"), ("model.encoder.conv2.bias", (D,), "b"),
                ("model.encoder.embed_positions.weight", (dims.max_src, D), "frozen")]

        def shapes(name, kind):
            if kind == "w":
                if name.endswith("fc1.weight"):
                    return (Fd, D)
                if name.endswith("fc2.weight"):
                    return (D, Fd)
                return (D, D)
            if name.endswith("fc1.bias"):
                return (Fd,)
            return (D,)

        for i in range(dims.enc_layers):
            spec += [(n, shapes(n, k), k) for n, k in layer_names(f"model.encoder.layers.{i}", False)]
        spec += [("model.encoder.layer_norm.weight", (D,), "ln"), ("model.encoder.layer_norm.bias", (D,), "ln"),
                 ("model.decoder.embed_positions.weight", (dims.max_tgt, D), "emb")]
        for i in range(dims.dec_layers):
            spec += [(n, shapes(n, k), k) for n, k in layer_names(f"model.decoder.layers.{i}", True)]
        spec += [("model.decoder.layer_norm.weight", (D,), "ln"), ("model.decoder.layer_norm.bias", (D,), "ln"),
                 ("model.decoder.embed_tokens.weight", (dims.vocab, D), "emb")]

        def is_frozen(name, kind):
            if kind == "frozen" or not trainable:
                return True
            return any(name.startswith(pf) for pf in frozen_prefixes)

        ordered = [e for e in spec if is_frozen(e[0], e[2])] + [e for e in spec if not is_frozen(e[0], e[2])]
        self.entries, off = {}, 0
        self.train_start = None
        for name, shape, kind in ordered:
            if self.train_start is None and not is_frozen(name, kind):
                self.train_start = off
            n = 1
            for d in shape:
                n *= d
            self.entries[name] = (off, shape, kind)
            off += _rup(n, 64)
        self.train_end = off
        if self.train_start is None:
            self.train_start = off
        dec_offs = [o for n, (o, _, _) in self.entries.items() if n.startswith("model.decoder.") and o >= self.train_start]
        self.dec_start = min(dec_offs) if dec_offs else self.train_end
        total = off + 64 * max(D, 64)
        self.total = total
        self.P = ops.zeros((total,), torch.float32)
        self.S = ops.zeros((total,), ops.lowp)
        self.G = self.M = self.V = None
        if trainable and self.train_end > self.train_start:
            self.G = ops.zeros((total,), torch.float32)
            self.M = ops.zeros((total,), torch.float32)
            self.V = ops.zeros((total,), torch.float32)
        self.p, self.s, self.g = {}, {}, {}
        for name, (o, shape, kind) in self.entries.items():
            n = 1
            for d in shape:
                n *= d
            self.p[name] = self.P[o:o + n].view(shape)
            self.s[name] = self.S[o:o + n].view(shape)
            if self.G is not None and o >= self.train_start:
                self.g[name] = self.G[o:o + n].view(shape)
        self.small_grad_views = []
        if self.G is not None:
            rng = []
            for name, (o, shape, kind) in self.entries.items():
                if o < self.train_start or kind == "w":
                    continue
                n = 1
                for d in shape:
                    n *= d
                if rng and rng[-1][1] == o:
                    rng[-1][1] = o + _rup(n, 64)
                else:
                    rng.append([o, o + _rup(n, 64)])
            self.small_grad_views = [self.G[a:b] for a, b in rng]
        self.kpad1 = _rup(3 * dims.n_mels, 64)
        self.conv1_packed = ops.zeros((D, self.kpad1), ops.lowp)
        self.conv2_packed = ops.zeros((D, 3 * D), ops.lowp)
        self.load_state_dict(state_dict, round_bf16=round_bf16)

    def real_names(self):
        return [n for n, (_, _, k) in self.entries.items() if k != "zero"]

    def load_state_dict(self, sd, round_bf16=False):
        dev = self.P.device
        for name in self.real_names():
            src = sd[name].detach().to(device=dev, dtype=torch.float32)
            if round_bf16:
                src = src.to(torch.bfloat16).to(torch.float32)
            self.p[name].copy_(src)
        self.refresh_shadow()

    def state_dict(self):
        sd = {n: self.p[n].detach().clone() for n in self.real_names()}
        sd["proj_out.weight"] = sd["model.decoder.embed_tokens.weight"]
        return sd

    def refresh_shadow(self):
        self.ops.cast_bf16(self.P, out=self.S)
        self.repack_conv()

    def repack_conv(self):
        self.ops.pack_conv_weight(self.p["model.encoder.conv1.weight"], self.kpad1, out=self.conv1_packed)
        self.ops.pack_conv_weight(self.p["model.encoder.conv2.weight"], 3 * self.dims.d_model, out=self.conv2_packed)

    def is_trainable(self, name):
        return self.G is not None and self.entries[name][0] >= self.train_start

    def attn_views(self, prefix, cross_kv=False):
        D = self.dims.d_model
        oq = self.entries[f"{prefix}.q_proj.weight"][0]
        ob = self.entries[f"{prefix}.q_proj.bias"][0]
        assert self.entries[f"{prefix}.k_proj.weight"][0] == oq + D * D
        assert self.entries[f"{prefix}.v_proj.bias"][0] == ob + 2 * D
        v = {"wqkv": self.S[oq:oq + 3 * D * D].view(3 * D, D), "bqkv": self.P[ob:ob + 3 * D],
             "wo": self.s[f"{prefix}.out_proj.weight"], "bo": self.p[f"{prefix}.out_proj.bias"]}
        if self.is_trainable(f"{prefix}.q_proj.weight"):
            v["g_wqkv"] = self.G[oq:oq + 3 * D * D].view(3 * D, D)
            v["g_bqkv"] = self.G[ob:ob + 3 * D]
            v["g_wo"] = self.g[f"{prefix}.out_proj.weight"]
            v["g_bo"] = self.g[f"{prefix}.out_proj.bias"]
        return v

    def adam_segments(self, weight_decay, decay_filter=None):
        segs = []
        for name, (o, shape, kind) in self.entries.items():
            if o < self.train_start:
                continue
            n = 1
            for d in shape:
                n *= d
            wd = weight_decay if kind in ("w", "conv", "emb") else 0.0
            end = o + _rup(n, 64)
            if segs and segs[-1][2] == wd and segs[-1][1] == o:
                segs[-1] = (segs[-1][0], end, wd)
            else:
                segs.append((o, end, wd))
        return segs


class LiveRows:

    def __init__(self, idx, n, B, T, seq_start=None, seq_len=None, max_q=0, attn_flops=(0.0, 0.0)):
        self.idx, self.n, self.B, self.T = idx, int(n), int(B), int(T)
        self.seq_start, self.seq_len, self.max_q = seq_start, seq_len, int(max_q)
        self.attn_flops = attn_flops

    @staticmethod
    def seq_table(lens, T, fill_to=None, entries=None):
        lens = [max(1, min(int(T), int(x))) for x in lens]
        n_live = sum(lens)
        fill = max(0, int(fill_to) - n_live) if fill_to is not None else 0
        lens = lens + [min(T, fill - o) for o in range(0, fill, T)]
        if entries is not None:
            if len(lens) > entries:
                raise ValueError("LiveRows.seq_table: more filler sequences than the table holds")
            lens = lens + [0] * (entries - len(lens))
        ln = torch.tensor(lens, dtype=torch.int32)
        st = torch.cumsum(ln, 0, dtype=torch.int32) - ln
        return st, ln

    @staticmethod
    def host_index(lens, T, fill_to=None):
        lens = [max(1, min(int(T), int(x))) for x in lens]
        idx = torch.cat([b * T + torch.arange(n, dtype=torch.int32) for b, n in enumerate(lens)])
        if fill_to is not None and fill_to > idx.numel():
            need = int(fill_to) - idx.numel()
            dead = torch.cat([b * T + torch.arange(n, T, dtype=torch.int32) for b, n in enumerate(lens)])
            if dead.numel() < need:
                raise ValueError("LiveRows.host_index: not enough dead rows to fill the list")
            idx = torch.cat([idx, dead[:need]])
        return idx

    @classmethod
    def build(cls, lens, T, device):
        h = cls.host_index(lens, T)
        st, ln = cls.seq_table(lens, T)
        lf = ln.double()
        return cls(h.to(device), h.numel(), len(lens), T, st.to(device), ln.to(device), int(ln.max()),
                   attn_flops=(float((lf * lf).sum()), float(lf.sum())))


class WhisperEngine:

    def __init__(self, ops, store: ParamStore, stream_dtype=torch.float32):
        self.ops, self.st, self.dims = ops, store, store.dims
        self.stream = stream_dtype
        self.lowp = ops.lowp
        self.ldv = _rup(self.dims.vocab, 64)
        self.wgrad_stream = None
        self._wgrad_held, self._wgrad_fences = [], []
        self.pad_gemm_rows = False
        self.pad_gemm_rows_min = 2560
        self.pad_gemm_rows_slack = 1 / 32
        self.pad_lm_rows = True

    ffn_row_pad = 64
    row_pad = 64
    stream_row_pad = 128
    dx_row_pad = 64

    def act(self, rows, cols, dtype=None, zero_pad=True, pad=0):
        dtype = self.lowp if dtype is None else dtype
        rp = _rup(rows, 64)
        t = self.ops.empty((rp, cols + pad), dtype)
        if pad:
            t = t[:, :cols]
        if rp > rows and zero_pad:
            t[rows:].zero_()
        return t

    def _gemm_rows(self, R, save):
        if save or not self.pad_gemm_rows or R < self.pad_gemm_rows_min:
            return R
        Rg = _rup(R, 320)
        return Rg if Rg - R <= R * self.pad_gemm_rows_slack else R

    def _ln(self, name, x, R, save, rows_alloc=None, zero_pad=None, pad=0):
        y = self.act(R if rows_alloc is None else rows_alloc, x.shape[1], zero_pad=save if zero_pad is None else zero_pad, pad=pad)
        _, mu, rs = self.ops.layernorm_fwd(x[:R] if x.shape[0] != R else x, self.st.p[f"{name}.weight"],
                                           self.st.p[f"{name}.bias"], 1e-5, save_stats=save, out=y[:R])
        return y, mu, rs

    def _ln_bwd(self, name, dy, x, mu, rs, dres, R, emit=False, colsum_to=None):
        if self.st.is_trainable(f"{name}.weight"):
            dg, db = self.st.g[f"{name}.weight"], self.st.g[f"{name}.bias"]
        else:
            dg, db = self._scratch_vec(x.shape[1]), self._scratch_vec(x.shape[1], 1)
        nxt = self.act(R, x.shape[1], pad=self.row_pad) if emit else None
        dres = self.ops.layernorm_bwd(dy[:R], x[:R] if x.shape[0] != R else x, mu, rs, self.st.p[f"{name}.weight"],
                                      dres, dg, db, out_lowp=nxt[:R] if emit else None,
                                      colsum=colsum_to if emit else None)
        return dres, nxt

    def _train_scatter_buf(self, slot, rows, cols):
        if not hasattr(self, "_tsb"):
            self._tsb = {}
        fits = [b for b in self._tsb.get((slot, cols), []) if b.shape[0] >= rows]
        if fits:
            return min(fits, key=lambda b: b.shape[0])
        buf = self.ops.zeros((_rup(rows, 64), cols), self.lowp)
        self._tsb.setdefault((slot, cols), []).append(buf)
        return buf

    def _scatter_buf(self, rows, cols):
        if not hasattr(self, "_sb"):
            self._sb = {}
        fits = [b for b in self._sb.get(cols, []) if b.shape[0] >= rows]
        if fits:
            return min(fits, key=lambda b: b.shape[0])
        buf = self.ops.zeros((_rup(rows, 64), cols), self.lowp)
        self._sb.setdefault(cols, []).append(buf)
        return buf

    def _scratch_vec(self, n, slot=0):
        key = (n, slot)
        if not hasattr(self, "_sv"):
            self._sv = {}
        if key not in self._sv:
            self._sv[key] = self.ops.zeros((n,), torch.float32)
        return self._sv[key]

    def _wgrad(self, dy, x, gout, gbias, R, bias_cols=None):
        ws = self.wgrad_stream
        if ws is not None:
            main = torch.cuda.current_stream(dy.device)
            ws.wait_stream(main)
            with torch.cuda.stream(ws):
                self._wgrad_issue(dy, x, gout, gbias, R, bias_cols)
            self._wgrad_held += [dy, x]
        else:
            self._wgrad_issue(dy, x, gout, gbias, R, bias_cols)

    pack_train_layers = True
    varlen_attention = True
    wgrad_overwrite = False
    wgrad_lag = 2

    def _wgrad_fence(self):
        ws = self.wgrad_stream
        if ws is None or not (self._wgrad_held or self._wgrad_fences):
            return
        ev = torch.cuda.Event()
        ev.record(ws)
        self._wgrad_fences.append((ev, self._wgrad_held))
        self._wgrad_held = []
        while len(self._wgrad_fences) > self.wgrad_lag:
            ev, held = self._wgrad_fences.pop(0)
            torch.cuda.current_stream(self.st.P.device).wait_event(ev)
            held.clear()

    def _wgrad_issue(self, dy, x, gout, gbias, R, bias_cols):
        if gout is not None:
            self.ops.gemm(dy, x, trans_a=True, trans_b=True, out_dtype=torch.float32, out=gout, atomic_acc=True,
                          overwrite=self.wgrad_overwrite)
        if gbias is not None:
            if bias_cols is None:
                self.ops.colsum(dy[:R], gbias, accumulate=True)
            else:
                for lo, hi in bias_cols:
                    self.ops.colsum(dy[:R, lo:hi], gbias[lo:hi], accumulate=True)

    def join_wgrad_stream(self):
        if self.wgrad_stream is not None:
            torch.cuda.current_stream(self.st.P.device).wait_stream(self.wgrad_stream)
        self._wgrad_fences.clear()
        self._wgrad_held = []

    def encode(self, mel, save=False):
        ops, st, d = self.ops, self.st, self.dims
        B, _, T = mel.shape
        D, H = d.d_model, d.heads
        R1, R = B * T, B * T // 2
        L = T // 2
        ctx = {"B": B, "T": T, "R": R, "layers": []} if save else None
        xcol1 = self.act(R1, st.kpad1, zero_pad=save)
        ops.im2col_mel(mel, st.kpad1, out=xcol1[:R1])
        a1 = self.act(R1, D, zero_pad=save)
        _, z1 = ops.gemm(xcol1[:R1], st.conv1_packed, bias=st.p["model.encoder.conv1.bias"], act=1, want_z=True,
                         out=a1[:R1])
        xcol2 = self.act(R, 3 * D, zero_pad=save)
        ops.im2col_s2(a1[:R1], B, T, out=xcol2[:R])
        x = ops.empty((R, D), self.stream)
        _, z2 = ops.gemm(xcol2[:R], st.conv2_packed, bias=st.p["model.encoder.conv2.bias"], act=1, want_z=True,
                         residual=st.p["model.encoder.embed_positions.weight"], r_row_mod=L, round_res=True, out=x)
        if save:
            ctx.update(xcol1=xcol1, z1=z1, xcol2=xcol2, z2=z2)
        else:
            del xcol1, a1, z1, xcol2, z2
        for i in range(d.enc_layers):
            x, lc = self._layer_fwd(f"model.encoder.layers.{i}", x, B, L, None, 0, False, save)
            if save:
                ctx["layers"].append(lc)
        y, mu, rs = self._ln("model.encoder.layer_norm", x, R, save, zero_pad=True)
        if save:
            ctx.update(x_final=x, mu=mu, rs=rs, enc_out=y)
        return y, ctx

    def _layer_fwd(self, p, x, B, L, enc_out, Lk, causal, save, Rg=None, live=None):
        ops, st, d = self.ops, self.st, self.dims
        D, H, Rp = d.d_model, d.heads, B * L
        R = Rp if live is None else live.n
        Rg = R if Rg is None else Rg
        assert Rg == R or not save
        lc = {} if save else None
        rect = {}

        def attend(q_src, k, v, Lkv, is_causal, cols):
            o = self.act(Rg, D, zero_pad=save, pad=self.row_pad)
            if live is None:
                _, lse = ops.attn_fwd(q_src[:R, :D], k, v, B, H, L, Lkv, is_causal, 0.125, out=o[:R])
                return o, lse
            if save:
                tag = "x" if k is not None else "s"
                qp = self._train_scatter_buf((p, tag, "q"), Rp, cols)
                ops.scatter_rows(q_src[:R], live.idx, qp)
                op = self._train_scatter_buf((p, tag, "o"), Rp, D)
                kk, vv = (qp[:Rp, D:2 * D], qp[:Rp, 2 * D:]) if k is None else (k, v)
                _, lse = ops.attn_fwd(qp[:Rp, :D], kk, vv, B, H, L, Lkv, is_causal, 0.125, out=op[:Rp])
                ops.gather_rows(op, live.idx, o)
                rect[tag] = (qp, op)
                return o, lse
            if live.seq_start is not None and self.varlen_attention:
                if k is None:
                    ops.attn_fwd_varlen(q_src[:R, :D], q_src[:R, D:2 * D], q_src[:R, 2 * D:], H, live.max_q, live.seq_start,
                                        live.seq_len, is_causal, 0.125, o[:R], self_attention=True,
                                        flops=256.0 * H * live.attn_flops[0])
                else:
                    ops.attn_fwd_varlen(q_src[:R, :D], k, v, H, live.max_q, live.seq_start, live.seq_len, is_causal, 0.125, o[:R],
                                        Lk=Lkv, kv_batches=B, self_attention=False, flops=256.0 * H * Lkv * live.attn_flops[1])
                return o, None
            qp = self._scatter_buf(Rp, cols)
            ops.scatter_rows(q_src[:R], live.idx, qp)
            op = self.act(Rp, D, zero_pad=False)
            kk, vv = (qp[:Rp, D:2 * D], qp[:Rp, 2 * D:]) if k is None else (k, v)
            ops.attn_fwd(qp[:Rp, :D], kk, vv, B, H, L, Lkv, is_causal, 0.125, out=op[:Rp])
            ops.gather_rows(op, live.idx, o)
            return o, None
        av = st.attn_views(f"{p}.self_attn")
        h, mu, rs = self._ln(f"{p}.self_attn_layer_norm", x, R, save, Rg, pad=self.row_pad)
        qkv = self.act(Rg, 3 * D, zero_pad=save, pad=self.row_pad)
        ops.gemm(h[:Rg], av["wqkv"], bias=av["bqkv"], out=qkv[:Rg])
        if live is None:
            o, lse = attend(qkv, qkv[:R, D:2 * D], qkv[:R, 2 * D:], L, causal, 3 * D)
        else:
            o, lse = attend(qkv, None, None, L, causal, 3 * D)
        xp = self.stream_row_pad // (4 if self.stream == torch.float32 else 2)
        x1 = ops.gemm(o[:Rg], av["wo"], bias=av["bo"], residual=x, round_res=True, out_dtype=self.stream, out_row_pad=xp)
        if save:
            lc.update(x0=x, mu0=mu, rs0=rs, h0=h, qkv=qkv, o0=o, lse0=lse)
            if live is not None:
                lc.update(qkv_r=rect["s"][0], o0_r=rect["s"][1])
        x = x1
        if enc_out is not None:
            cv = st.attn_views(f"{p}.encoder_attn")
            Re = B * Lk
            h, mu, rs = self._ln(f"{p}.encoder_attn_layer_norm", x, R, save, Rg, pad=self.row_pad)
            q = self.act(Rg, D, zero_pad=save, pad=self.row_pad)
            ops.gemm(h[:Rg], cv["wqkv"][:D], bias=cv["bqkv"][:D], out=q[:Rg])
            kv = self.act(Re, 2 * D, zero_pad=save, pad=self.row_pad)
            ops.gemm(enc_out[:Re], cv["wqkv"][D:], bias=cv["bqkv"][D:], out=kv[:Re])
            o, lse = attend(q, kv[:Re, :D], kv[:Re, D:], Lk, False, D)
            x1 = ops.gemm(o[:Rg], cv["wo"], bias=cv["bo"], residual=x, round_res=True, out_dtype=self.stream, out_row_pad=xp)
            if save:
                lc.update(x1=x, mu1=mu, rs1=rs, h1=h, q1=q, kv1=kv, o1=o, lse1=lse)
                if live is not None:
                    lc.update(q1_r=rect["x"][0], o1_r=rect["x"][1])
            x = x1
        h, mu, rs = self._ln(f"{p}.final_layer_norm", x, R, save, Rg, pad=self.row_pad)
        a = self.act(Rg, d.ffn, zero_pad=save, pad=self.ffn_row_pad)
        res = ops.gemm(h[:Rg], st.s[f"{p}.fc1.weight"], bias=st.p[f"{p}.fc1.bias"], act=1,
                       want_z=("grad" if self.ffn_keeps_gelu_grad else True) if save else False, out=a[:Rg],
                       z_row_pad=self.ffn_row_pad)
        z = res[1] if save else None
        x2 = ops.gemm(a[:Rg], st.s[f"{p}.fc2.weight"], bias=st.p[f"{p}.fc2.bias"], residual=x, round_res=True,
                      out_dtype=self.stream, out_row_pad=xp)
        if save:
            lc.update(x2=x, mu2=mu, rs2=rs, h2=h, a=a, z=z)
        return x2, lc

    def decode(self, ids, enc_out, save=False, live=None):
        ops, st, d = self.ops, self.st, self.dims
        B, T = ids.shape
        R, Lk = B * T, d.max_src
        assert live is None or (live.B == B and live.T == T)
        ctx = {"B": B, "T": T, "R": R, "ids": ids, "layers": [], "enc_out": enc_out} if save else None
        packed = live is not None and (not save or self.pack_train_layers)
        if packed and not save and getattr(self, "_sb", None):
            for bufs in self._sb.values():
                for b_ in bufs:
                    b_.zero_()
        Rv = live.n if packed else R
        self._last_decode_rows = Rv
        Rg = self._gemm_rows(Rv, save)
        if self.stream == torch.float32:
            x = ops.embed_fwd(ids, st.p["model.decoder.embed_tokens.weight"],
                              st.p["model.decoder.embed_positions.weight"], torch.float32, rows_alloc=R if packed else Rg)
        else:
            x = ops.embed_fwd(ids, st.s["model.decoder.embed_tokens.weight"],
                              st.s["model.decoder.embed_positions.weight"], self.lowp, rows_alloc=R if packed else Rg)
        if packed:
            xp, x = x, ops.empty((Rg, d.d_model), self.stream)
            ops.gather_rows(xp, live.idx, x)
            del xp
        for i in range(d.dec_layers):
            x, lc = self._layer_fwd(f"model.decoder.layers.{i}", x, B, T, enc_out, Lk, True, save, Rg,
                                    live if packed else None)
            if save:
                ctx["layers"].append(lc)
        Rh = live.n if live is not None else R
        Rl = Rh
        if save and self.pad_lm_rows and Rh >= self.pad_gemm_rows_min:
            Rl = _rup(Rh, 320)
            Rl = Rl if Rl - Rh <= Rh * self.pad_gemm_rows_slack else Rh
        hf, mu, rs = self._ln("model.decoder.layer_norm", x, Rv, save, max(Rl, Rv))
        if live is not None and save and not packed:
            hfp, hf = hf, self.act(Rl, d.d_model)
            ops.gather_rows(hfp, live.idx, hf)
            del hfp
        logits = self.act(Rl, self.ldv, zero_pad=save)
        if Rl > Rh:
            hf[Rh:Rl].zero_()
            logits[Rh:Rl].zero_()
        eo = st.entries["model.decoder.embed_tokens.weight"][0]
        e_pad = st.S[eo:eo + self.ldv * d.d_model].view(self.ldv, d.d_model)
        ops.gemm(hf[:Rh], e_pad, out=logits[:Rh])
        if save:
            ctx.update(x_final=x, mu=mu, rs=rs, hf=hf, lm_rows=Rl, live=live, packed=packed, Rv=Rv)
        return logits, ctx

    def decode_init(self, enc_out, B, max_len, cache=None):
        ops, st, d = self.ops, self.st, self.dims
        D, Re = d.d_model, B * d.max_src
        if cache is None:
            cache = {"B": B, "max_len": max_len, "t": 0, "cross": [None] * d.dec_layers,
                     "self": [ops.zeros((B * max_len, 2 * D), self.lowp) for _ in range(d.dec_layers)]}
        assert cache["B"] == B and cache["max_len"] == max_len
        cache["t"] = 0
        for i in range(d.dec_layers):
            cv = st.attn_views(f"model.decoder.layers.{i}.encoder_attn")
            cache["cross"][i] = ops.gemm(enc_out[:Re], cv["wqkv"][D:], bias=cv["bqkv"][D:], out=cache["cross"][i],
                                         out_row_pad=self.kv_row_pad)
        return cache

    ffn_keeps_gelu_grad = True
    fuse_fc1_bias_grad = True
    fuse_attn_bias_grad = False
    use_c_decode = True
    kv_row_pad = 64

    def _decode_desc(self, cache, n):
        key = ("desc", n)
        if key in cache:
            return cache[key]
        from .ops_hip import DwDecodeStep, DwDecoderLayer, DW_BF16, DW_F32
        ops, st, d = self.ops, self.st, self.dims
        B, D, F = cache["B"], d.d_model, d.ffn
        rows = B * n
        f32 = self.stream == torch.float32
        tab = st.p if f32 else st.s
        ws = {"x": ops.empty((rows, D), self.stream), "h": ops.empty((rows, D), self.lowp),
              "qkv": ops.empty((rows, 3 * D), self.lowp), "o": ops.empty((rows, D), self.lowp),
              "a": ops.empty((rows, F), self.lowp), "logits": ops.empty((rows, self.ldv), self.lowp)}
        layers = (DwDecoderLayer * d.dec_layers)()
        keep = [ws]
        for i in range(d.dec_layers):
            p = f"model.decoder.layers.{i}"
            av, cv = st.attn_views(f"{p}.self_attn"), st.attn_views(f"{p}.encoder_attn")
            L = layers[i]
            L.ln1_g, L.ln1_b = st.p[f"{p}.self_attn_layer_norm.weight"].data_ptr(), st.p[f"{p}.self_attn_layer_norm.bias"].data_ptr()
            L.wqkv, L.bqkv = av["wqkv"].data_ptr(), av["bqkv"].data_ptr()
            L.wo, L.bo = av["wo"].data_ptr(), av["bo"].data_ptr()
            L.ln2_g, L.ln2_b = st.p[f"{p}.encoder_attn_layer_norm.weight"].data_ptr(), st.p[f"{p}.encoder_attn_layer_norm.bias"].data_ptr()
            L.wq, L.bq = cv["wqkv"][:D].data_ptr(), cv["bqkv"][:D].data_ptr()
            L.wo2, L.bo2 = cv["wo"].data_ptr(), cv["bo"].data_ptr()
            L.ln3_g, L.ln3_b = st.p[f"{p}.final_layer_norm.weight"].data_ptr(), st.p[f"{p}.final_layer_norm.bias"].data_ptr()
            L.w1, L.b1 = st.s[f"{p}.fc1.weight"].data_ptr(), st.p[f"{p}.fc1.bias"].data_ptr()
            L.w2, L.b2 = st.s[f"{p}.fc2.weight"].data_ptr(), st.p[f"{p}.fc2.bias"].data_ptr()
            L.self_kv, L.cross_kv = cache["self"][i].data_ptr(), cache["cross"][i].data_ptr()
            keep += [av, cv]
        eo = st.entries["model.decoder.embed_tokens.weight"][0]
        desc = DwDecodeStep()
        desc.batch, desc.n_new, desc.d_model, desc.heads, desc.ffn, desc.n_layers = B, n, D, d.heads, F, d.dec_layers
        desc.src_len, desc.max_len, desc.vocab, desc.ldv = d.max_src, cache["max_len"], d.vocab, self.ldv
        desc.stream_dtype = DW_F32 if f32 else DW_BF16
        desc.cross_kv_ld = cache["cross"][0].stride(0)
        assert all(c.stride(0) == desc.cross_kv_ld for c in cache["cross"])
        desc.tok_emb = tab["model.decoder.embed_tokens.weight"].data_ptr()
        desc.pos_emb = tab["model.decoder.embed_positions.weight"].data_ptr()
        desc.lnf_g, desc.lnf_b = st.p["model.decoder.layer_norm.weight"].data_ptr(), st.p["model.decoder.layer_norm.bias"].data_ptr()
        desc.lm_head = st.S[eo:eo + self.ldv * D].data_ptr()
        desc.layers = C.cast(layers, C.c_void_p)
        for k, v in ws.items():
            setattr(desc, k, v.data_ptr())
        cache[key] = (desc, ws, layers, keep)
        return cache[key]

    def _decode_pass_c(self, ids, cache, n):
        desc, ws, _, _ = self._decode_desc(cache, n)
        ids = ids.contiguous()
        desc.ids, desc.t = ids.data_ptr(), cache["t"]
        self.ops.decode_pass(desc)
        cache["t"] += n
        return ws["logits"]

    def _decoder_layers_cached(self, x, cache, n):
        ops, st, d = self.ops, self.st, self.dims
        B, t, ML = cache["B"], cache["t"], cache["max_len"]
        D, H, Lk = d.d_model, d.heads, d.max_src
        rows = B * n
        fuse_ln, fuse_kv = rows <= 32 and D <= 1280, rows <= 64
        causal = 2 if n > 1 else False
        for i in range(d.dec_layers):
            p = f"model.decoder.layers.{i}"
            av = st.attn_views(f"{p}.self_attn")
            ln1 = (st.p[f"{p}.self_attn_layer_norm.weight"], st.p[f"{p}.self_attn_layer_norm.bias"], 1e-5)
            kvc = cache["self"][i]
            h = x if fuse_ln else ops.layernorm_fwd(x, *ln1, save_stats=False)[0]
            qkv = ops.gemm(h, av["wqkv"], bias=av["bqkv"], ln=ln1[:2] if fuse_ln else None,
                           kv_append=(kvc, D, n, ML, t) if fuse_kv else None)
            if not fuse_kv:
                kvc.view(B, ML, 2 * D)[:, t:t + n].copy_(qkv[:, D:].view(B, n, 2 * D))
            o, _ = ops.attn_fwd(qkv[:, :D], kvc[:, :D], kvc[:, D:], B, H, n, t + n, causal, 0.125, kv_batch_rows=ML)
            x = ops.gemm(o, av["wo"], bias=av["bo"], residual=x, round_res=True, out_dtype=self.stream)
            cv = st.attn_views(f"{p}.encoder_attn")
            ln2 = (st.p[f"{p}.encoder_attn_layer_norm.weight"], st.p[f"{p}.encoder_attn_layer_norm.bias"], 1e-5)
            h = x if fuse_ln else ops.layernorm_fwd(x, *ln2, save_stats=False)[0]
            q = ops.gemm(h, cv["wqkv"][:D], bias=cv["bqkv"][:D], ln=ln2[:2] if fuse_ln else None)
            kv = cache["cross"][i]
            o, _ = ops.attn_fwd(q, kv[:, :D], kv[:, D:], B, H, n, Lk, False, 0.125)
            x = ops.gemm(o, cv["wo"], bias=cv["bo"], residual=x, round_res=True, out_dtype=self.stream)
            ln3 = (st.p[f"{p}.final_layer_norm.weight"], st.p[f"{p}.final_layer_norm.bias"], 1e-5)
            h = x if fuse_ln else ops.layernorm_fwd(x, *ln3, save_stats=False)[0]
            a = ops.gemm(h, st.s[f"{p}.fc1.weight"], bias=st.p[f"{p}.fc1.bias"], act=1, ln=ln3[:2] if fuse_ln else None)
            x = ops.gemm(a, st.s[f"{p}.fc2.weight"], bias=st.p[f"{p}.fc2.bias"], residual=x, round_res=True,
                         out_dtype=self.stream)
        return x

    def decode_step(self, ids_t, cache):
        ops, st, d = self.ops, self.st, self.dims
        B, t, ML = cache["B"], cache["t"], cache["max_len"]
        D, H, Lk = d.d_model, d.heads, d.max_src
        assert ids_t.shape == (B, 1) and t < ML and t < d.max_tgt
        if self.use_c_decode and hasattr(ops, "decode_pass"):
            return self._decode_pass_c(ids_t, cache, 1)
        f32 = self.stream == torch.float32
        tok = (st.p if f32 else st.s)["model.decoder.embed_tokens.weight"]
        pos = (st.p if f32 else st.s)["model.decoder.embed_positions.weight"][t:t + 1]
        x = ops.embed_fwd(ids_t.contiguous(), tok, pos, torch.float32 if f32 else self.lowp)
        x = self._decoder_layers_cached(x, cache, 1)
        hf, _, _ = ops.layernorm_fwd(x, st.p["model.decoder.layer_norm.weight"], st.p["model.decoder.layer_norm.bias"],
                                     1e-5, save_stats=False)
        eo = st.entries["model.decoder.embed_tokens.weight"][0]
        e_pad = st.S[eo:eo + self.ldv * D].view(self.ldv, D)
        logits = ops.gemm(hf, e_pad)
        cache["t"] = t + 1
        return logits

    def decode_multi(self, ids, cache):
        ops, st, d = self.ops, self.st, self.dims
        B, t, ML = cache["B"], cache["t"], cache["max_len"]
        n = ids.shape[1]
        D, H, Lk = d.d_model, d.heads, d.max_src
        assert ids.shape[0] == B and t + n <= ML and t + n <= d.max_tgt
        if self.use_c_decode and hasattr(ops, "decode_pass"):
            return self._decode_pass_c(ids, cache, n)
        f32 = self.stream == torch.float32
        tok = (st.p if f32 else st.s)["model.decoder.embed_tokens.weight"]
        pos = (st.p if f32 else st.s)["model.decoder.embed_positions.weight"][t:t + n]
        x = ops.embed_fwd(ids.contiguous(), tok, pos.contiguous(), torch.float32 if f32 else self.lowp)
        x = self._decoder_layers_cached(x, cache, n)
        hf, _, _ = ops.layernorm_fwd(x, st.p["model.decoder.layer_norm.weight"], st.p["model.decoder.layer_norm.bias"],
                                     1e-5, save_stats=False)
        eo = st.entries["model.decoder.embed_tokens.weight"][0]
        e_pad = st.S[eo:eo + self.ldv * D].view(self.ldv, D)
        logits = ops.gemm(hf, e_pad)
        cache["t"] = t + n
        return logits

    def _bias_grad(self, name):
        return self.st.g[name] if self.st.is_trainable(name) else None

    def _layer_bwd(self, p, lc, dres, dy, B, L, Lk, causal, denc, emit_last, colsum_last, live=None):
        ops, st, d = self.ops, self.st, self.dims
        D, H, Rp = d.d_model, d.heads, B * L
        R = Rp if live is None else live.n
        tr = st.is_trainable(f"{p}.fc1.weight")
        cross = "x1" in lc

        def to_rect(t, cols):
            r = ops.zeros((_rup(Rp, 64), cols), t.dtype)
            ops.scatter_rows(t[:R], live.idx, r)
            return r
        dz = self.act(R, d.ffn, pad=self.ffn_row_pad)
        fuse_cs = tr and self.fuse_fc1_bias_grad and R > 64
        ops.gemm(dy[:R], st.s[f"{p}.fc2.weight"], trans_b=True, zgrad=lc["z"], out=dz[:R],
                 colsum=st.g[f"{p}.fc1.bias"] if fuse_cs else None)
        if tr:
            self._wgrad(dy, lc["a"], st.g[f"{p}.fc2.weight"], None, R)
            self._wgrad(dz, lc["h2"], st.g[f"{p}.fc1.weight"], None if fuse_cs else st.g[f"{p}.fc1.bias"], R)
        dh = ops.gemm(dz[:R], st.s[f"{p}.fc1.weight"], trans_b=True, out_row_pad=self.dx_row_pad)
        nb = f"{p}.encoder_attn.out_proj.bias" if cross else f"{p}.self_attn.out_proj.bias"
        dres, dy = self._ln_bwd(f"{p}.final_layer_norm", dh, lc["x2"], lc["mu2"], lc["rs2"], dres, R, emit=True,
                                colsum_to=self._bias_grad(nb))
        del dz, dh
        if cross:
            cv = st.attn_views(f"{p}.encoder_attn")
            Re = B * Lk
            do = ops.gemm(dy[:R], cv["wo"], trans_b=True, out_row_pad=self.dx_row_pad)
            dq = self.act(R, D, pad=self.row_pad)
            dkv = self.act(Re, 2 * D, pad=self.row_pad)
            fb = tr and self.fuse_attn_bias_grad
            if live is None:
                ops.attn_bwd(lc["q1"][:R], lc["kv1"][:Re, :D], lc["kv1"][:Re, D:], lc["o1"][:R], do, lc["lse1"], B, H, L,
                             Lk, False, 0.125, dq=dq[:R], dk=dkv[:Re, :D], dv=dkv[:Re, D:],
                             dq_colsum=cv["g_bqkv"][:D] if fb else None, dv_colsum=cv["g_bqkv"][2 * D:] if fb else None)
            else:
                do_r = to_rect(do, D)
                dq_r = self.act(Rp, D, zero_pad=False)
                ops.attn_bwd(lc["q1_r"][:Rp], lc["kv1"][:Re, :D], lc["kv1"][:Re, D:], lc["o1_r"][:Rp], do_r[:Rp], lc["lse1"], B, H, L,
                             Lk, False, 0.125, dq=dq_r[:Rp], dk=dkv[:Re, :D], dv=dkv[:Re, D:],
                             dq_colsum=cv["g_bqkv"][:D] if fb else None, dv_colsum=cv["g_bqkv"][2 * D:] if fb else None)
                ops.gather_rows(dq_r, live.idx, dq)
                del do_r, dq_r
            if tr:
                self._wgrad(dy, lc["o1"], cv["g_wo"], None, R)
                self._wgrad(dq, lc["h1"], cv["g_wqkv"][:D], None if fb else cv["g_bqkv"][:D], R)
                self._wgrad(dkv, lc["enc_out"], cv["g_wqkv"][D:], None if fb else cv["g_bqkv"][D:], Re, bias_cols=[(D, 2 * D)])
            if denc is not None:
                ops.gemm(dkv[:Re], cv["wqkv"][D:], trans_b=True, residual=denc, round_res=True,
                         out_dtype=torch.float32, out=denc)
            dh = ops.gemm(dq[:R], cv["wqkv"][:D], trans_b=True, out_row_pad=self.dx_row_pad)
            dres, dy = self._ln_bwd(f"{p}.encoder_attn_layer_norm", dh, lc["x1"], lc["mu1"], lc["rs1"], dres, R,
                                    emit=True, colsum_to=self._bias_grad(f"{p}.self_attn.out_proj.bias"))
            del do, dq, dkv, dh
        av = st.attn_views(f"{p}.self_attn")
        do = ops.gemm(dy[:R], av["wo"], trans_b=True, out_row_pad=self.dx_row_pad)
        dqkv = self.act(R, 3 * D, pad=self.row_pad)
        qkv = lc["qkv"]
        fb = tr and self.fuse_attn_bias_grad
        if live is None:
            ops.attn_bwd(qkv[:R, :D], qkv[:R, D:2 * D], qkv[:R, 2 * D:], lc["o0"][:R], do, lc["lse0"], B, H, L, L, causal,
                         0.125, dq=dqkv[:R, :D], dk=dqkv[:R, D:2 * D], dv=dqkv[:R, 2 * D:],
                         dq_colsum=av["g_bqkv"][:D] if fb else None, dv_colsum=av["g_bqkv"][2 * D:] if fb else None)
        else:
            qr = lc["qkv_r"]
            do_r = to_rect(do, D)
            dqkv_r = self.act(Rp, 3 * D, zero_pad=False)
            ops.attn_bwd(qr[:Rp, :D], qr[:Rp, D:2 * D], qr[:Rp, 2 * D:], lc["o0_r"][:Rp], do_r[:Rp], lc["lse0"], B, H, L, L, causal,
                         0.125, dq=dqkv_r[:Rp, :D], dk=dqkv_r[:Rp, D:2 * D], dv=dqkv_r[:Rp, 2 * D:],
                         dq_colsum=av["g_bqkv"][:D] if fb else None, dv_colsum=av["g_bqkv"][2 * D:] if fb else None)
            ops.gather_rows(dqkv_r, live.idx, dqkv)
            del do_r, dqkv_r
        if tr:
            self._wgrad(dy, lc["o0"], av["g_wo"], None, R)
            self._wgrad(dqkv, lc["h0"], av["g_wqkv"], None if fb else av["g_bqkv"], R, bias_cols=[(0, D), (2 * D, 3 * D)])
        dh = ops.gemm(dqkv[:R], av["wqkv"], trans_b=True, out_row_pad=self.dx_row_pad)
        return self._ln_bwd(f"{p}.self_attn_layer_norm", dh, lc["x0"], lc["mu0"], lc["rs0"], dres, R, emit=emit_last,
                            colsum_to=colsum_last)

    def backward_decoder(self, ctx, dlogits, want_denc=True, accumulate=False):
        ops, st, d = self.ops, self.st, self.dims
        self._accumulate = accumulate
        B, T, R, D = ctx["B"], ctx["T"], ctx["R"], d.d_model
        Lk = d.max_src
        emb = "model.decoder.embed_tokens.weight"
        tr_emb = st.is_trainable(emb)
        if tr_emb:
            ops.gemm(dlogits[:, :d.vocab], ctx["hf"], trans_a=True, trans_b=True, out_dtype=torch.float32,
                     out=st.g[emb], atomic_acc=True, overwrite=self.wgrad_overwrite)
        eo = st.entries[emb][0]
        e_pad = st.S[eo:eo + self.ldv * D].view(self.ldv, D)
        Rl = ctx.get("lm_rows", R)
        assert dlogits.shape[0] >= Rl
        dh = ops.gemm(dlogits[:Rl], e_pad, trans_b=True)
        live = ctx.get("live")
        packed = bool(ctx.get("packed")) and live is not None
        Rv = ctx["Rv"] if packed else R
        if live is not None and not packed:
            dhp = self.act(R, D)
            dhp[:R].zero_()
            ops.scatter_rows(dh, live.idx, dhp)
            dh = dhp
        nl = d.dec_layers
        dres, dy = self._ln_bwd("model.decoder.layer_norm", dh, ctx["x_final"], ctx["mu"], ctx["rs"], None, Rv,
                                emit=True, colsum_to=self._bias_grad(f"model.decoder.layers.{nl - 1}.fc2.bias"))
        denc = ops.zeros((B * Lk, D), torch.float32) if want_denc else None
        for i in reversed(range(nl)):
            lc = ctx["layers"][i]
            lc["enc_out"] = ctx["enc_out"]
            below = self._bias_grad(f"model.decoder.layers.{i - 1}.fc2.bias") if i > 0 else None
            dres, dy = self._layer_bwd(f"model.decoder.layers.{i}", lc, dres, dy, B, T, Lk, True, denc, i > 0, below,
                                       live=live if packed else None)
            ctx["layers"][i] = None
            self._wgrad_fence()
        if tr_emb or st.is_trainable("model.decoder.embed_positions.weight"):
            dtok = st.g[emb] if tr_emb else self._scratch_tok()
            dpos = st.g.get("model.decoder.embed_positions.weight")
            if packed:
                dres_r = ops.zeros((R, D), dres.dtype)
                ops.scatter_rows(dres[:Rv], live.idx, dres_r)
                dres = dres_r
            ops.embed_bwd(dres, ctx["ids"], dtok, dpos)
        return denc

    def _scratch_tok(self):
        if not hasattr(self, "_stok"):
            self._stok = self.ops.zeros((self.dims.vocab, self.dims.d_model), torch.float32)
        return self._stok

    def param_range(self, prefix):
        st = self.st
        offs = [(o, o + _rup(int(torch.tensor(shape).prod()), 64)) for n, (o, shape, _) in st.entries.items()
                if n.startswith(prefix) and o >= st.train_start]
        if not offs:
            return None
        return min(a for a, _ in offs), max(b for _, b in offs)

# ... 50 lines not shown
```

### distil_whisper_amd/ops_hip.py

```python
import ctypes as C
import math
import os

import torch

_HERE = os.path.dirname(os.path.abspath(__file__))
LIB_PATH = os.path.join(_HERE, "libdwamd.so")

DW_F32, DW_BF16 = 0, 1


class DwGemm(C.Structure):
    _fields_ = [
        ("a", C.c_void_p), ("b", C.c_void_p), ("c", C.c_void_p), ("bias", C.c_void_p), ("z_out", C.c_void_p),
        ("zgrad_in", C.c_void_p), ("r", C.c_void_p),
        ("lda", C.c_int64), ("ldb", C.c_int64), ("ldc", C.c_int64), ("ldz", C.c_int64), ("ldzg", C.c_int64),
        ("ldr", C.c_int64),
        ("m", C.c_int32), ("n", C.c_int32), ("k", C.c_int32),
        ("trans_a", C.c_int32), ("trans_b", C.c_int32), ("act", C.c_int32), ("c_dtype", C.c_int32),
        ("r_dtype", C.c_int32), ("r_row_mod", C.c_int32), ("round_res", C.c_int32), ("tile", C.c_int32),
        ("split_k", C.c_int32), ("atomic_acc", C.c_int32), ("slice_stride", C.c_int64),
        ("ln_x", C.c_void_p), ("ln_gamma", C.c_void_p), ("ln_beta", C.c_void_p), ("kv_out", C.c_void_p),
        ("ld_lnx", C.c_int64), ("kv_ld", C.c_int64),
        ("ln_x_dtype", C.c_int32), ("kv_split", C.c_int32), ("kv_rows_per_batch", C.c_int32),
        ("kv_batch_pitch", C.c_int32), ("kv_row0", C.c_int32), ("ln_eps", C.c_float),
        ("z_is_gelu_grad", C.c_int32), ("colsum_out", C.c_void_p),
    ]


class DwDecoderLayer(C.Structure):
    _fields_ = [(n, C.c_void_p) for n in (
        "ln1_g", "ln1_b", "wqkv", "bqkv", "wo", "bo", "ln2_g", "ln2_b", "wq", "bq", "wo2", "bo2", "ln3_g", "ln3_b",
        "w1", "b1", "w2", "b2", "self_kv", "cross_kv")]


class DwDecodeStep(C.Structure):
    _fields_ = [(n, C.c_int32) for n in (
        "batch", "n_new", "d_model", "heads", "ffn", "n_layers", "src_len", "max_len", "t", "vocab", "ldv",
        "stream_dtype", "cross_kv_ld")] + [(n, C.c_void_p) for n in (
            "ids", "tok_emb", "pos_emb", "lnf_g", "lnf_b", "lm_head", "layers", "x", "h", "qkv", "o", "a", "logits")]


_SIGS = {
    "dw_version": ([], C.c_int),
    "dw_decode_step": ([C.POINTER(DwDecodeStep), C.c_void_p], C.c_int),
    "dw_logmel": ([C.c_void_p, C.c_int, C.c_int, C.c_void_p, C.c_int, C.c_void_p, C.c_void_p, C.c_void_p, C.c_void_p,
                   C.c_void_p], C.c_int),
    "dw_gemm_bf16": ([C.POINTER(DwGemm), C.c_void_p], C.c_int),
    "dw_layernorm_fwd": ([C.c_void_p, C.c_int, C.c_void_p, C.c_void_p, C.c_void_p, C.c_void_p, C.c_void_p, C.c_int,
                          C.c_int, C.c_float, C.c_void_p], C.c_int),
    "dw_layernorm_bwd": ([C.c_void_p, C.c_void_p, C.c_int, C.c_void_p, C.c_void_p, C.c_void_p, C.c_void_p, C.c_int,
                          C.c_void_p, C.c_void_p, C.c_void_p, C.c_void_p, C.c_int, C.c_int, C.c_void_p], C.c_int),
    "dw_reduce_slices_ld": ([C.c_void_p, C.c_int64, C.c_int64, C.c_int, C.c_void_p, C.c_int64, C.c_int, C.c_int, C.c_int, C.c_void_p], C.c_int),
    "dw_layernorm_fwd_ld": ([C.c_void_p, C.c_int, C.c_void_p, C.c_void_p, C.c_void_p, C.c_void_p, C.c_void_p, C.c_int,
                             C.c_int, C.c_float, C.c_int64, C.c_int64, C.c_void_p], C.c_int),
    "dw_layernorm_bwd_ld": ([C.c_void_p, C.c_void_p, C.c_int, C.c_void_p, C.c_void_p, C.c_void_p, C.c_void_p, C.c_int,
                             C.c_void_p, C.c_void_p, C.c_void_p, C.c_void_p, C.c_int, C.c_int] + [C.c_int64] * 4 + [C.c_void_p], C.c_int),
    "dw_attn_fwd": ([C.c_void_p] * 5 + [C.c_int] * 4 + [C.c_int64] * 4 + [C.c_int, C.c_float, C.c_void_p], C.c_int),
    "dw_attn_fwd_ex": ([C.c_void_p] * 5 + [C.c_int] * 4 + [C.c_int64] * 6 + [C.c_int, C.c_float, C.c_void_p], C.c_int),
    "dw_attn_fwd_varlen": ([C.c_void_p] * 4 + [C.c_int] * 4 + [C.c_int64] * 4 + [C.c_void_p] * 4 + [C.c_int, C.c_int64, C.c_int, C.c_float,
                                                                                                           C.c_void_p], C.c_int),
    "dw_attn_bwd": ([C.c_void_p] * 10 + [C.c_int] * 4 + [C.c_int64] * 8 + [C.c_int, C.c_float, C.c_void_p], C.c_int),
    "dw_attn_bwd_ex": ([C.c_void_p] * 10 + [C.c_int] * 4 + [C.c_int64] * 8 + [C.c_int, C.c_float] + [C.c_void_p] * 3, C.c_int),
    "dw_distill_loss": ([C.c_void_p, C.c_void_p, C.c_void_p, C.c_int, C.c_int, C.c_int64, C.c_float, C.c_float,
                         C.c_float, C.c_float, C.c_void_p, C.c_void_p, C.c_void_p, C.c_void_p, C.c_void_p,
                         C.c_void_p], C.c_int),
    "dw_distill_loss_w": ([C.c_void_p, C.c_void_p, C.c_void_p, C.c_int, C.c_int, C.c_int64, C.c_float, C.c_void_p,
                           C.c_float, C.c_void_p, C.c_void_p, C.c_void_p, C.c_void_p, C.c_void_p, C.c_void_p], C.c_int),
    "dw_embed_fwd": ([C.c_void_p, C.c_void_p, C.c_void_p, C.c_int, C.c_void_p, C.c_int, C.c_int, C.c_int, C.c_int,
                      C.c_void_p], C.c_int),
    "dw_embed_bwd": ([C.c_void_p, C.c_void_p, C.c_void_p, C.c_void_p, C.c_int, C.c_int, C.c_int, C.c_void_p], C.c_int),
    "dw_im2col_mel": ([C.c_void_p, C.c_void_p, C.c_int, C.c_int, C.c_int, C.c_int, C.c_void_p], C.c_int),
    "dw_im2col_s2": ([C.c_void_p, C.c_void_p, C.c_int, C.c_int, C.c_int, C.c_void_p], C.c_int),
    "dw_col2im_s2_gelu_bwd": ([C.c_void_p, C.c_void_p, C.c_void_p, C.c_int, C.c_int, C.c_int, C.c_void_p], C.c_int),
    "dw_gelu_bwd": ([C.c_void_p, C.c_int, C.c_void_p, C.c_void_p, C.c_int64, C.c_void_p], C.c_int),
    "dw_pack_conv_weight": ([C.c_void_p, C.c_void_p, C.c_int, C.c_int, C.c_int, C.c_void_p], C.c_int),
    "dw_unpack_conv_grad": ([C.c_void_p, C.c_void_p, C.c_int, C.c_int, C.c_int, C.c_int, C.c_void_p], C.c_int),
    "dw_cast_f32_bf16": ([C.c_void_p, C.c_void_p, C.c_int64, C.c_void_p], C.c_int),
    "dw_cast_bf16_f32": ([C.c_void_p, C.c_void_p, C.c_int64, C.c_void_p], C.c_int),
    "dw_colsum_bf16": ([C.c_void_p, C.c_int64, C.c_int, C.c_int, C.c_void_p, C.c_int, C.c_void_p], C.c_int),
    "dw_add": ([C.c_void_p, C.c_int, C.c_void_p, C.c_int, C.c_void_p, C.c_int, C.c_int64, C.c_void_p], C.c_int),
    "dw_move_rows": ([C.c_void_p, C.c_int64, C.c_void_p, C.c_int64, C.c_void_p, C.c_int, C.c_int, C.c_int, C.c_void_p], C.c_int),
    "dw_sumsq_f32": ([C.c_void_p, C.c_int64, C.c_void_p, C.c_void_p, C.c_void_p], C.c_int),
    "dw_adamw": ([C.c_void_p] * 5 + [C.c_int64, C.c_void_p] + [C.c_float] * 2 + [C.c_double] * 5 + [C.c_int, C.c_void_p], C.c_int),
    "dw_adam_tick": ([C.c_void_p, C.c_void_p, C.c_void_p], C.c_int),
    "dw_adamw_dev": ([C.c_void_p] * 5 + [C.c_int64, C.c_void_p] + [C.c_float] * 2 + [C.c_void_p] + [C.c_double] * 2 +
                     [C.c_void_p], C.c_int),
    "dw_selftest_tr16": ([C.c_void_p, C.c_void_p], C.c_int),
    "dw_debug_set": ([C.c_int, C.c_int], C.c_int),
    "dw_reduce_slices": ([C.c_void_p, C.c_int64, C.c_int, C.c_void_p, C.c_int64, C.c_int, C.c_void_p], C.c_int),
    "dw_greedy_select": ([C.c_void_p, C.c_int, C.c_int, C.c_int64, C.c_void_p, C.c_void_p] + [C.c_int] * 5 +
                         [C.c_void_p, C.c_int64, C.c_int, C.c_int, C.c_int, C.c_int, C.c_void_p, C.c_void_p,
                          C.c_void_p], C.c_int),
}

EXPORTED_SYMBOLS = tuple(_SIGS.keys())


def load_library(path: str = LIB_PATH):
    if not os.path.exists(path):
        raise RuntimeError(
            f"{path} not found: build it with `python -m distil_whisper_amd.build` (hipcc --offload-arch=gfx950). "
            "The MI355X path has no CPU fallback.")
    lib = C.CDLL(path)
    for name, (args, res) in _SIGS.items():
        fn = getattr(lib, name)
        fn.argtypes = args
        fn.restype = res
    return lib


def _dt(t):
    if t.dtype == torch.float32:
        return DW_F32
    if t.dtype == torch.bfloat16:
        return DW_BF16
    raise TypeError(f"unsupported dtype {t.dtype}")


def _p(t):
    return None if t is None else t.data_ptr()


class HipOps:

    name = "hip"
    lowp = torch.bfloat16

    def __init__(self, device="cuda:0"):
        if not torch.cuda.is_available():
            raise RuntimeError("HipOps needs a ROCm GPU (torch.cuda.is_available() is False); there is no CPU path.")
        self.lib = load_library()
        self.device = torch.device(device)
        i = torch.arange(400, dtype=torch.float64)
        ang = 2.0 * math.pi * i / 400.0
        self._twiddle = torch.stack([torch.cos(ang), torch.sin(ang)], 1).to(torch.float32).contiguous().to(self.device)
        self._window = torch.hann_window(400, periodic=True, dtype=torch.float64).to(torch.float32).to(self.device)
        self.profile = None
        self._prof_events = []
        self.profile_detail = False

    def _stream(self):
        return C.c_void_p(torch.cuda.current_stream(self.device).cuda_stream)

    @staticmethod
    def _chk(rc, what):
        if rc != 0:
            raise RuntimeError(f"libdwamd: {what} failed with code {rc}")

    def _t0(self):
        if self.profile is None:
            return None
        e = torch.cuda.Event(enable_timing=True)
        e.record(torch.cuda.current_stream(self.device))
        return e

    def _t1(self, e0, key, flops=0.0, nbytes=0.0):
        if e0 is None:
            return
        e1 = torch.cuda.Event(enable_timing=True)
        e1.record(torch.cuda.current_stream(self.device))
        self._prof_events.append((key, flops, nbytes, e0, e1))

    def collect_profile(self):
        torch.cuda.synchronize(self.device)
        out = {}
        for key, flops, nbytes, e0, e1 in self._prof_events:
            d = out.setdefault(key, {"n": 0, "ms": 0.0, "flops": 0.0, "bytes": 0.0})
            d["n"] += 1
            d["ms"] += e0.elapsed_time(e1)
            d["flops"] += flops
            d["bytes"] += nbytes
        self._prof_events = []
        return out

    @staticmethod
    def pick_tile(M, N):
        t256 = ((M + 255) // 256) * ((N + 255) // 256)
        return 256 if t256 >= 512 else 128

    wgrad_slab_pad = 0

    def empty(self, shape, dtype):
        return torch.empty(shape, dtype=dtype, device=self.device)

    def zeros(self, shape, dtype):
        return torch.zeros(shape, dtype=dtype, device=self.device)

    def selftest_tr16(self):
        out = self.empty((64, 4), torch.int32)
        self._chk(self.lib.dw_selftest_tr16(_p(out), self._stream()), "selftest_tr16")
        return out

    def logmel(self, audio, filters):
        assert audio.dtype == torch.float32 and audio.dim() == 2 and audio.is_contiguous()
        assert filters.dtype == torch.float32 and filters.shape[0] == 201 and filters.is_contiguous()
        B, N = audio.shape
        M = filters.shape[1]
        out = self.empty((B, M, N // 160), torch.float32)
        clip = self.empty((B,), torch.float32)
        self._chk(self.lib.dw_logmel(_p(audio), B, N, _p(filters), M, _p(self._twiddle), _p(self._window), _p(out),
                                     _p(clip), self._stream()), "logmel")
        return out

    def gemm(self, a, b, *, trans_a=False, trans_b=False, bias=None, act=0, want_z=False, zgrad=None, residual=None,
             r_row_mod=0, round_res=True, out_dtype=None, out=None, tile=0, atomic_acc=False, split_k=0, ln=None,
             kv_append=None, colsum=None, z_row_pad=0, out_row_pad=0, overwrite=False):
        assert b.dtype == torch.bfloat16 and (a.dtype == torch.bfloat16 or ln is not None)
        assert a.stride(1) == 1 and b.stride(1) == 1
        if trans_a:
            K, M = a.shape
        else:
            M, K = a.shape
        if trans_b:
            Kb, N = b.shape
        else:
            N, Kb = b.shape
        assert K == Kb, (a.shape, b.shape, trans_a, trans_b)
        if out is None:
            out = self.empty((M, N + out_row_pad), self.lowp if out_dtype is None else out_dtype)
            if out_row_pad:
                out = out[:, :N]
        assert out.shape == (M, N) and out.stride(1) == 1
        g = DwGemm()
        g.a, g.b, g.c = a.data_ptr(), b.data_ptr(), out.data_ptr()
        g.lda, g.ldb, g.ldc = a.stride(0), b.stride(0), out.stride(0)
        g.m, g.n, g.k = M, N, K
        g.trans_a, g.trans_b = int(trans_a), int(trans_b)
        g.act = int(act)
        g.c_dtype = _dt(out)
        g.tile = int(tile) if tile else 0
        tile_key = g.tile if tile or M <= 64 else self.pick_tile(M, N)
        ws = None
        if atomic_acc:
            assert out.dtype == torch.float32 and bias is None and residual is None and not want_z and zgrad is None
            if not tile:
                g.tile = tile_key = 256
            tiles = ((M + g.tile - 1) // g.tile) * ((N + g.tile - 1) // g.tile)
            nt = K // 64
            if split_k:
                sk = int(split_k)
            else:
                best, sk = -1.0, 1
                for cand in range(1, max(1, min(16, nt // 16)) + 1):
                    jobs = tiles * cand
                    eff = jobs / (-(-jobs // 256) * 256) - 0.004 * cand
                    if eff > best + 1e-9:
                        best, sk = eff, cand
            sk = max(1, min(sk, nt // 16))
            if sk > 1 and out.stride(1) == 1 and N % 4 == 0 and out.stride(0) % 4 == 0:
                ldw = N + self.wgrad_slab_pad
                ws = self.empty((sk, M, ldw), torch.float32)
                g.c, g.ldc = ws.data_ptr(), ldw
                g.split_k, g.slice_stride = sk, M * ldw
            elif overwrite:
                g.atomic_acc, g.split_k = 0, 1
            else:
                g.atomic_acc, g.split_k = 1, 1
        if ln is not None:
            gamma, beta = ln[0], ln[1]
            assert a.dtype in (torch.float32, torch.bfloat16) and not trans_a
            assert gamma.dtype == torch.float32 and beta.dtype == torch.float32 and gamma.numel() == K == beta.numel()
            g.a, g.ln_x, g.ld_lnx, g.ln_x_dtype = None, a.data_ptr(), a.stride(0), _dt(a)
            g.ln_gamma, g.ln_beta, g.ln_eps = gamma.data_ptr(), beta.data_ptr(), float(ln[2]) if len(ln) > 2 else 1e-5
        if kv_append is not None:
            cache, split, rpb, pitch, row0 = kv_append
            assert cache.dtype == torch.bfloat16 and cache.stride(-1) == 1
            g.kv_out, g.kv_ld, g.kv_split = cache.data_ptr(), N - split, int(split)
            g.kv_rows_per_batch, g.kv_batch_pitch, g.kv_row0 = int(rpb), int(pitch), int(row0)
        z = None
        if bias is not None:
            assert bias.dtype == torch.float32 and bias.numel() == N and bias.is_contiguous()
            g.bias = bias.data_ptr()
        if want_z:
            as_grad = want_z == "grad"
            assert not as_grad or act == 1
            z = self.empty((M, N + z_row_pad), torch.float16 if as_grad else torch.bfloat16)
            if z_row_pad:
                z = z[:, :N]
            g.z_out, g.ldz, g.z_is_gelu_grad = z.data_ptr(), z.stride(0), int(as_grad)
        if zgrad is not None:
            assert zgrad.dtype in (torch.bfloat16, torch.float16) and zgrad.shape == (M, N) and zgrad.stride(1) == 1
            assert not (want_z and (zgrad.dtype == torch.float16) != (want_z == "grad"))
            g.zgrad_in, g.ldzg = zgrad.data_ptr(), zgrad.stride(0)
            g.z_is_gelu_grad = int(zgrad.dtype == torch.float16)
        if colsum is not None:
            assert colsum.dtype == torch.float32 and colsum.numel() == N and colsum.is_contiguous() and not atomic_acc and M > 64
            g.colsum_out = colsum.data_ptr()
        if residual is not None:
            assert residual.stride(1) == 1 and residual.shape[1] == N
            g.r, g.ldr, g.r_dtype = residual.data_ptr(), residual.stride(0), _dt(residual)
            g.r_row_mod = int(r_row_mod)
            g.round_res = int(bool(round_res))
        e0 = self._t0()
        self._chk(self.lib.dw_gemm_bf16(C.byref(g), self._stream()), f"gemm m={M} n={N} k={K} ta={trans_a} tb={trans_b}")
        if ws is not None:
            self._chk(self.lib.dw_reduce_slices_ld(ws.data_ptr(), g.slice_stride, g.ldc, g.split_k, out.data_ptr(), out.stride(0),
                                                   M, N, 0 if overwrite else 1, self._stream()), "reduce_slices")
        key = f"gemm_t{tile_key}_{'T' if trans_a else 'N'}{'T' if trans_b else 'N'}"
        if self.profile_detail:
            key += (f" m{M} n{N} k{K} c{'f32' if out.dtype == torch.float32 else 'bf16'}"
                    f"{' bias' if bias is not None else ''}{' act%d' % act if act else ''}{' z' if want_z else ''}"
                    f"{' zg' if zgrad is not None else ''}"
                    f"{' r' + ('f32' if residual.dtype == torch.float32 else 'bf16') if residual is not None else ''}"
                    f"{' sk%d' % g.split_k if g.split_k else ''}")
        self._t1(e0, key, 2.0 * M * N * K)
        return (out, z) if want_z else out

    def decode_pass(self, desc):
        e0 = self._t0()
        self._chk(self.lib.dw_decode_step(C.byref(desc), self._stream()), "decode_step")
        self._t1(e0, "decode_step", 0.0)

    def layernorm_fwd(self, x, gamma, beta, eps=1e-5, save_stats=True, out=None):
        rows, cols = x.shape
        assert x.stride(1) == 1 and gamma.dtype == torch.float32 and beta.dtype == torch.float32
        y = self.empty((rows, cols), torch.bfloat16) if out is None else out
        assert y.stride(1) == 1 and y.shape == (rows, cols) and y.dtype == torch.bfloat16
        mean = self.empty((rows,), torch.float32) if save_stats else None
        rstd = self.empty((rows,), torch.float32) if save_stats else None
        self._chk(self.lib.dw_layernorm_fwd_ld(_p(x), _dt(x), _p(gamma), _p(beta), _p(y), _p(mean), _p(rstd), rows, cols,
                                               float(eps), x.stride(0), y.stride(0), self._stream()), "layernorm_fwd")
        return y, mean, rstd

    def layernorm_bwd(self, dy, x, mean, rstd, gamma, dres, dgamma, dbeta, out_lowp=None, colsum=None):
        rows, cols = x.shape
        assert dy.dtype == torch.bfloat16 and dy.stride(1) == 1 and x.stride(1) == 1 and dy.shape == (rows, cols)
        acc = dres is not None
        if dres is None:
            dres = self.empty((rows, cols), torch.float32)
        assert dres.dtype == torch.float32 and dres.stride(1) == 1 and dres.shape == (rows, cols)
        ldl = cols
        if out_lowp is not None:
            assert out_lowp.dtype == torch.bfloat16 and out_lowp.stride(1) == 1 and out_lowp.shape == (rows, cols)
            ldl = out_lowp.stride(0)
        assert colsum is None or out_lowp is not None
        self._chk(self.lib.dw_layernorm_bwd_ld(_p(dy), _p(x), _dt(x), _p(mean), _p(rstd), _p(gamma), _p(dres), int(acc),
                                               _p(dgamma), _p(dbeta), _p(out_lowp), _p(colsum), rows, cols,
                                               dy.stride(0), x.stride(0), dres.stride(0), ldl, self._stream()), "layernorm_bwd")
        return dres

    def attn_fwd_varlen(self, q, k, v, H, max_q, q_start, q_len, causal, scale, out, Lk=0, kv_batches=0, self_attention=True,
                        flops=0.0):
        for t in (q, k, v, out):
            assert t.dtype == torch.bfloat16 and t.stride(1) == 1
        assert q_start.dtype == torch.int32 and q_len.dtype == torch.int32 and q_start.numel() == q_len.numel()
        n = q_start.numel()
        e0 = self._t0()
        self._chk(self.lib.dw_attn_fwd_varlen(_p(q), _p(k), _p(v), _p(out), n, H, int(max_q), int(Lk), q.stride(0), k.stride(0),
                                              v.stride(0), out.stride(0), _p(q_start), _p(q_len),
                                              _p(q_start) if self_attention else None, _p(q_len) if self_attention else None,
                                              int(kv_batches), int(Lk), int(causal), float(scale), self._stream()), "attn_fwd_varlen")
        self._t1(e0, "attn_fwd", flops)
        return out

    def attn_fwd(self, q, k, v, B, H, Lq, Lk, causal, scale, out=None, kv_batch_rows=None):
        for t in (q, k, v):
            assert t.dtype == torch.bfloat16 and t.stride(1) == 1
        o = self.empty((B * Lq, H * 64), torch.bfloat16) if out is None else out
        assert o.dtype == torch.bfloat16 and o.stride(1) == 1 and o.shape == (B * Lq, H * 64)
        lse = self.empty((B, H, Lq), torch.float32)
        e0 = self._t0()
        self._chk(self.lib.dw_attn_fwd_ex(_p(q), _p(k), _p(v), _p(o), _p(lse), B, H, Lq, Lk, q.stride(0), k.stride(0),
                                          v.stride(0), o.stride(0), Lq, Lk if kv_batch_rows is None else kv_batch_rows,
                                          int(causal), float(scale), self._stream()), "attn_fwd")
        self._t1(e0, "attn_fwd", 4.0 * B * H * Lq * Lk * 64)
        return o, lse

    def attn_bwd(self, q, k, v, o, do, lse, B, H, Lq, Lk, causal, scale, dq=None, dk=None, dv=None, dq_colsum=None,
                 dv_colsum=None):
        if dq is None:
            dq = self.empty((B * Lq, H * 64), torch.bfloat16)
        if dk is None:
            dk = self.empty((B * Lk, H * 64), torch.bfloat16)
        if dv is None:
            dv = self.empty((B * Lk, H * 64), torch.bfloat16)
        delta = self.empty((2, B, H, Lq), torch.float32)
        for t in (q, k, v, o, do, dq, dk, dv):
            assert t.dtype == torch.bfloat16 and t.stride(1) == 1
        e0 = self._t0()
        for t in (dq_colsum, dv_colsum):
            assert t is None or (t.dtype == torch.float32 and t.numel() == H * 64 and t.is_contiguous())
        part = None
        if dq_colsum is not None or dv_colsum is not None:
            key = (B, H)
            if not hasattr(self, "_attn_cs"):
                self._attn_cs = {}
            if key not in self._attn_cs:
                self._attn_cs[key] = self.zeros((2, B, H * 64), torch.float32)
            part = self._attn_cs[key]
            part.zero_()
        self._chk(self.lib.dw_attn_bwd_ex(_p(q), _p(k), _p(v), _p(o), _p(do), _p(lse), _p(delta), _p(dq), _p(dk), _p(dv),
                                          B, H, Lq, Lk, q.stride(0), k.stride(0), v.stride(0), o.stride(0), do.stride(0),
                                          dq.stride(0), dk.stride(0), dv.stride(0), int(causal), float(scale),
                                          _p(part[0]) if dq_colsum is not None else None,
                                          _p(part[1]) if dv_colsum is not None else None, self._stream()), "attn_bwd")
        for i, dst in enumerate((dq_colsum, dv_colsum)):
            if dst is not None:
                self._chk(self.lib.dw_reduce_slices(_p(part[i]), H * 64, B, _p(dst), H * 64, 1, self._stream()),
                          "reduce_slices")
        self._t1(e0, "attn_bwd", 10.0 * B * H * Lq * Lk * 64)
        return dq, dk, dv

    def distill_loss(self, s_logits, t_logits, labels, V, temperature, ce_weight, kl_weight, grad_scale, want_grad,
                     grad_out=None, weights_dev=None):
        rows, ld = s_logits.shape
        if grad_out is not None:
            assert want_grad and grad_out.shape == s_logits.shape and grad_out.dtype == torch.bfloat16 and grad_out.is_contiguous()
        assert s_logits.dtype == torch.bfloat16 and t_logits.dtype == torch.bfloat16
        assert s_logits.is_contiguous() and t_logits.is_contiguous() and t_logits.shape == s_logits.shape
        assert labels.dtype == torch.int64 and labels.numel() == rows and labels.is_contiguous()
        losses = self.empty((4,), torch.float32)
        row_ce = self.empty((rows,), torch.float32)
        row_kl = self.empty((rows,), torch.float32)
        counts = self.empty((2,), torch.int32)
        dl = (_p(s_logits) if grad_out is None else _p(grad_out)) if want_grad else None
        if weights_dev is not None:
            assert weights_dev.dtype == torch.float32 and weights_dev.numel() == 2 and weights_dev.is_contiguous()
            self._chk(self.lib.dw_distill_loss_w(_p(s_logits), _p(t_logits), _p(labels), rows, V, ld, float(temperature),
                                                 _p(weights_dev), float(grad_scale), _p(losses), dl, _p(row_ce), _p(row_kl),
                                                 _p(counts), self._stream()), "distill_loss_w")
            return losses
        self._chk(self.lib.dw_distill_loss(_p(s_logits), _p(t_logits), _p(labels), rows, V, ld, float(temperature),
                                           float(ce_weight), float(kl_weight), float(grad_scale), _p(losses), dl,
                                           _p(row_ce), _p(row_kl), _p(counts),
                                           self._stream()), "distill_loss")
        return losses

    def embed_fwd(self, ids, tok, pos, out_dtype, rows_alloc=0):
        B, T = ids.shape
        D = tok.shape[1]
        assert ids.dtype == torch.int64 and ids.is_contiguous() and tok.is_contiguous() and pos.is_contiguous()
        assert tok.dtype == pos.dtype
        if rows_alloc > B * T:
            out = self.empty((rows_alloc, D), out_dtype)
            out[B * T:].zero_()
        else:
            out = self.empty((B * T, D), out_dtype)
        self._chk(self.lib.dw_embed_fwd(_p(ids), _p(tok), _p(pos), _dt(tok), _p(out), _dt(out), B, T, D,
                                        self._stream()), "embed_fwd")
        return out

    def embed_bwd(self, dx, ids, dtok, dpos):
        B, T = ids.shape
        D = dx.shape[1]
        assert dx.dtype == torch.float32 and dx.is_contiguous() and dtok.dtype == torch.float32
        self._chk(self.lib.dw_embed_bwd(_p(dx), _p(ids), _p(dtok), _p(dpos), B, T, D, self._stream()), "embed_bwd")

    def im2col_mel(self, mel, kpad, out=None):
        B, Cc, T = mel.shape
        assert mel.dtype == torch.float32 and mel.is_contiguous()
        if out is None:
            out = self.empty((B * T, kpad), torch.bfloat16)
        assert out.is_contiguous() and out.shape == (B * T, kpad)
        self._chk(self.lib.dw_im2col_mel(_p(mel), _p(out), B, Cc, T, kpad, self._stream()), "im2col_mel")
        return out

    def im2col_s2(self, a, B, T, out=None):
        Cc = a.shape[1]
        assert a.dtype == torch.bfloat16 and a.is_contiguous() and a.shape[0] == B * T
        if out is None:
            out = self.empty((B * T // 2, 3 * Cc), torch.bfloat16)
        assert out.is_contiguous() and out.shape == (B * T // 2, 3 * Cc)
        self._chk(self.lib.dw_im2col_s2(_p(a), _p(out), B, T, Cc, self._stream()), "im2col_s2")
        return out

    def col2im_s2_gelu_bwd(self, dxcol, z, B, T, out=None):
        Cc = z.shape[1]
        assert dxcol.is_contiguous() and z.is_contiguous() and dxcol.dtype == torch.bfloat16
        dz = self.empty((B * T, Cc), torch.bfloat16) if out is None else out
        assert dz.is_contiguous() and dz.shape == (B * T, Cc)
        self._chk(self.lib.dw_col2im_s2_gelu_bwd(_p(dxcol), _p(z), _p(dz), B, T, Cc, self._stream()), "col2im")
        return dz

    def gelu_bwd(self, dy, z, out=None):
        assert dy.is_contiguous() and z.is_contiguous() and z.dtype == torch.bfloat16 and dy.shape == z.shape
        dz = self.empty(z.shape, torch.bfloat16) if out is None else out
        assert dz.is_contiguous() and dz.shape == z.shape
        self._chk(self.lib.dw_gelu_bwd(_p(dy), _dt(dy), _p(z), _p(dz), z.numel(), self._stream()), "gelu_bwd")
        return dz

    def pack_conv_weight(self, w, kpad, out=None):
        D, Cc, _ = w.shape
        assert w.dtype == torch.float32 and w.is_contiguous()
        if out is None:
            out = self.empty((D, kpad), torch.bfloat16)
        self._chk(self.lib.dw_pack_conv_weight(_p(w), _p(out), D, Cc, kpad, self._stream()), "pack_conv_weight")
        return out

    def unpack_conv_grad(self, gwp, gw, accumulate):
        D, Cc, _ = gw.shape
        assert gwp.dtype == torch.float32 and gwp.is_contiguous() and gw.is_contiguous()
        self._chk(self.lib.dw_unpack_conv_grad(_p(gwp), _p(gw), D, Cc, gwp.shape[1], int(accumulate), self._stream()),
                  "unpack_conv_grad")

    def cast_bf16(self, x, out=None):
        assert x.dtype == torch.float32 and x.is_contiguous()
        if out is None:
            out = self.empty(x.shape, torch.bfloat16)
        self._chk(self.lib.dw_cast_f32_bf16(_p(x), _p(out), x.numel(), self._stream()), "cast_f32_bf16")
        return out

    def cast_f32(self, x, out=None):
        assert x.dtype == torch.bfloat16 and x.is_contiguous()
        if out is None:
            out = self.empty(x.shape, torch.float32)
        self._chk(self.lib.dw_cast_bf16_f32(_p(x), _p(out), x.numel(), self._stream()), "cast_bf16_f32")
        return out

    def colsum(self, x, out, accumulate):
        rows, cols = x.shape
        assert x.dtype == torch.bfloat16 and x.stride(1) == 1 and out.dtype == torch.float32
        self._chk(self.lib.dw_colsum_bf16(_p(x), x.stride(0), rows, cols, _p(out), int(accumulate), self._stream()),
                  "colsum")
        return out

    def gather_rows(self, src, idx, out):
        n, rb = idx.numel(), src.shape[1] * src.element_size()
        assert src.stride(1) == 1 and out.stride(1) == 1 and out.shape[1] == src.shape[1] and out.dtype == src.dtype
        assert idx.dtype == torch.int32 and idx.is_contiguous() and out.shape[0] >= n
        self._chk(self.lib.dw_move_rows(_p(src), src.stride(0) * src.element_size(), _p(out),
                                        out.stride(0) * out.element_size(), _p(idx), n, rb, 0, self._stream()), "move_rows")
        return out

    def scatter_rows(self, src, idx, out):
        n, rb = idx.numel(), src.shape[1] * src.element_size()
        assert src.stride(1) == 1 and out.stride(1) == 1 and out.shape[1] == src.shape[1] and out.dtype == src.dtype
        assert idx.dtype == torch.int32 and idx.is_contiguous() and src.shape[0] >= n
        self._chk(self.lib.dw_move_rows(_p(src), src.stride(0) * src.element_size(), _p(out),
                                        out.stride(0) * out.element_size(), _p(idx), n, rb, 1, self._stream()), "move_rows")
        return out

    def add(self, a, b, out_dtype):
        assert a.is_contiguous() and b.is_contiguous() and a.shape == b.shape
        y = self.empty(a.shape, out_dtype)
        self._chk(self.lib.dw_add(_p(a), _dt(a), _p(b), _dt(b), _p(y), _dt(y), a.numel(), self._stream()), "add")
        return y

    def sumsq(self, g, out):
        assert g.dtype == torch.float32 and g.is_contiguous()
        if getattr(self, "_sumsq_ws", None) is None:
            self._sumsq_ws = self.empty((2048,), torch.float32)
        self._chk(self.lib.dw_sumsq_f32(_p(g), g.numel(), _p(out), _p(self._sumsq_ws), self._stream()), "sumsq")
        return out

    def greedy_select(self, logits, V, tokens, n, cur, *, suppress=None, begin_suppress=None, first=False, no_eos=False,
                      forced=False, ts_begin=-1, max_initial=-1, begin_index=1, eos=-1, fill=-1, done=None):
        B = tokens.shape[0]
        assert tokens.dtype == torch.int64 and tokens.is_contiguous() and cur.dtype == torch.int64 and cur.is_contiguous()
        if not forced:
            assert logits.dtype == torch.bfloat16 and logits.stride(1) == 1 and logits.shape[0] >= B
        for m in (suppress, begin_suppress):
            assert m is None or (m.dtype == torch.uint8 and m.numel() >= V and m.is_contiguous())
        assert done is None or (done.dtype == torch.bool and done.is_contiguous())
        self._chk(self.lib.dw_greedy_select(_p(logits), B, int(V), logits.stride(0) if logits is not None else 0,
                                            _p(suppress), _p(begin_suppress), int(first), int(no_eos), int(forced),
                                            int(ts_begin), int(max_initial), _p(tokens), tokens.stride(0), int(n),
                                            int(begin_index), int(eos), int(fill), _p(done), _p(cur), self._stream()),
                  "greedy_select")

    def adamw(self, p, g, m, v, shadow, sumsq, max_norm, grad_mul, lr, beta1, beta2, eps, weight_decay, step):
        assert p.is_contiguous() and g.is_contiguous() and m.is_contiguous() and v.is_contiguous()
        self._chk(self.lib.dw_adamw(_p(p), _p(g), _p(m), _p(v), _p(shadow), p.numel(), _p(sumsq), float(max_norm),
                                    float(grad_mul), float(lr), float(beta1), float(beta2), float(eps),
                                    float(weight_decay), int(step), self._stream()), "adamw")

    def adam_state(self, lr, beta1, beta2, step=0):
        return torch.tensor([lr, step, beta1, beta2, 0, 0, 0, 0], dtype=torch.float64, device=self.device)

    def adam_tick(self, state, gate=None):
        assert state.dtype == torch.float64 and state.numel() == 8 and (gate is None or gate.dtype == torch.float32)
        self._chk(self.lib.dw_adam_tick(_p(state), _p(gate), self._stream()), "adam_tick")

    def adamw_dev(self, p, g, m, v, shadow, sumsq, max_norm, grad_mul, state, eps, weight_decay):
        assert p.is_contiguous() and g.is_contiguous() and m.is_contiguous() and v.is_contiguous()
        self._chk(self.lib.dw_adamw_dev(_p(p), _p(g), _p(m), _p(v), _p(shadow), p.numel(), _p(sumsq), float(max_norm),
                                        float(grad_mul), _p(state), float(eps), float(weight_decay), self._stream()),
                  "adamw_dev")


def _timed(key):
    def deco(fn):
        def wrapper(self, *a, **k):
            e0 = self._t0()
            r = fn(self, *a, **k)
            self._t1(e0, key)
            return r
        wrapper.__name__, wrapper.__doc__ = fn.__name__, fn.__doc__
        return wrapper
    return deco


for _name, _key in (("layernorm_fwd", "ln_fwd"), ("layernorm_bwd", "ln_bwd"), ("distill_loss", "loss"),
                    ("logmel", "logmel"), ("adamw", "adamw"), ("adamw_dev", "adamw"), ("cast_bf16", "cast"), ("colsum", "colsum"),
                    ("sumsq", "sumsq"), ("embed_fwd", "embed"), ("embed_bwd", "embed"), ("im2col_mel", "conv_aux"),
                    ("im2col_s2", "conv_aux"), ("col2im_s2_gelu_bwd", "conv_aux"), ("gelu_bwd", "conv_aux"),
                    ("pack_conv_weight", "conv_aux"), ("unpack_conv_grad", "conv_aux"), ("greedy_select", "select")):
    setattr(HipOps, _name, _timed(_key)(getattr(HipOps, _name)))
```

### include/dwamd.h

```cpp
#ifndef DWAMD_H
#define DWAMD_H
#include <stdint.h>
#ifdef __cplusplus
extern "C" {
#endif

#define DW_OK 0
#define DW_EINVAL (-1)
#define DW_EUNSUP (-2)

#define DW_F32 0
#define DW_BF16 1

int dw_version(void);

int dw_logmel(const float* audio, int batch, int n_samples, const float* mel_filters, int n_mels,
              const float* twiddle, const float* window, float* out, float* clipmax, void* stream);

typedef struct DwGemm {
    const void* a;
    const void* b;
    void* c;
    const float* bias;
    void* z_out;
    const void* zgrad_in;
    const void* r;
    int64_t lda, ldb, ldc, ldz, ldzg, ldr;
    int32_t m, n, k;
    int32_t trans_a, trans_b;
    int32_t act;
    int32_t c_dtype;
    int32_t r_dtype;
    int32_t r_row_mod;
    int32_t round_res;
    int32_t tile;
    int32_t split_k;
    int32_t atomic_acc;
    int64_t slice_stride;
    const void* ln_x;
    const float* ln_gamma;
    const float* ln_beta;
    void* kv_out;
    int64_t ld_lnx, kv_ld;
    int32_t ln_x_dtype;
    int32_t kv_split, kv_rows_per_batch, kv_batch_pitch, kv_row0;
    float ln_eps;
    int32_t z_is_gelu_grad;
    float* colsum_out;
} DwGemm;
int dw_gemm_bf16(const DwGemm* g, void* stream);
int dw_reduce_slices(const float* part, int64_t stride, int slices, float* out, int64_t n, int accumulate, void* stream);
int dw_reduce_slices_ld(const float* part, int64_t slice_stride, int64_t ld_part, int slices, float* out, int64_t ld_out,
                        int rows, int cols, int accumulate, void* stream);

int dw_layernorm_fwd(const void* x, int x_dtype, const float* gamma, const float* beta, void* y, float* mean,
                     float* rstd, int rows, int cols, float eps, void* stream);
int dw_layernorm_bwd(const void* dy_bf16, const void* x, int x_dtype, const float* mean, const float* rstd,
                     const float* gamma, float* dres, int accumulate, float* dgamma, float* dbeta, void* dres_lowp,
                     float* dres_colsum, int rows, int cols, void* stream);
int dw_layernorm_fwd_ld(const void* x, int x_dtype, const float* gamma, const float* beta, void* y, float* mean,
                        float* rstd, int rows, int cols, float eps, int64_t ldx, int64_t ldy, void* stream);
int dw_layernorm_bwd_ld(const void* dy_bf16, const void* x, int x_dtype, const float* mean, const float* rstd,
                        const float* gamma, float* dres, int accumulate, float* dgamma, float* dbeta, void* dres_lowp,
                        float* dres_colsum, int rows, int cols, int64_t lddy, int64_t ldx, int64_t lddres,
                        int64_t ldlowp, void* stream);

int dw_attn_fwd(const void* q, const void* k, const void* v, void* o, float* lse, int B, int H, int Lq, int Lk,
                int64_t ldq, int64_t ldk, int64_t ldv, int64_t ldo, int causal, float scale, void* stream);
int dw_attn_fwd_ex(const void* q, const void* k, const void* v, void* o, float* lse, int B, int H, int Lq, int Lk,
                   int64_t ldq, int64_t ldk, int64_t ldv, int64_t ldo, int64_t q_batch_rows, int64_t kv_batch_rows,
                   int causal, float scale, void* stream);
int dw_attn_fwd_varlen(const void* q, const void* k, const void* v, void* o, int n_seq, int H, int max_q, int Lk, int64_t ldq,
                       int64_t ldk, int64_t ldv, int64_t ldo, const int32_t* q_start, const int32_t* q_len,
                       const int32_t* kv_start, const int32_t* kv_len, int kv_batches, int64_t kv_batch_rows, int causal,
                       float scale, void* stream);
int dw_attn_bwd(const void* q, const void* k, const void* v, const void* o, const void* d_o, const float* lse,
                float* delta, void* dq, void* dk, void* dv, int B, int H, int Lq, int Lk, int64_t ldq, int64_t ldk,
                int64_t ldv, int64_t ldo, int64_t lddo, int64_t lddq, int64_t lddk, int64_t lddv, int causal,
                float scale, void* stream);
int dw_attn_bwd_ex(const void* q, const void* k, const void* v, const void* o, const void* d_o, const float* lse,
                   float* delta, void* dq, void* dk, void* dv, int B, int H, int Lq, int Lk, int64_t ldq, int64_t ldk,
                   int64_t ldv, int64_t ldo, int64_t lddo, int64_t lddq, int64_t lddk, int64_t lddv, int causal,
                   float scale, float* dq_colsum, float* dv_colsum, void* stream);

int dw_distill_loss(const void* s_logits, const void* t_logits, const int64_t* labels, int rows, int V, int64_t ld,
                    float temperature, float ce_weight, float kl_weight, float grad_scale, float* losses,
                    void* dlogits, float* row_ce, float* row_kl, int32_t* counts, void* stream);
int dw_distill_loss_w(const void* s_logits, const void* t_logits, const int64_t* labels, int rows, int V, int64_t ld,
                      float temperature, const float* weights, float grad_scale, float* losses, void* dlogits,
                      float* row_ce, float* row_kl, int32_t* counts, void* stream);

int dw_embed_fwd(const int64_t* ids, const void* tok, const void* pos, int tab_dtype, void* out, int out_dtype,
                 int B, int T, int D, void* stream);
int dw_embed_bwd(const float* dx, const int64_t* ids, float* dtok, float* dpos, int B, int T, int D, void* stream);

int dw_im2col_mel(const float* mel, void* xcol, int B, int C, int T, int kpad, void* stream);
int dw_im2col_s2(const void* a, void* xcol, int B, int T, int C, void* stream);
int dw_col2im_s2_gelu_bwd(const void* dxcol, const void* z, void* dz, int B, int T, int C, void* stream);
int dw_gelu_bwd(const void* dy, int dy_dtype, const void* z, void* dz, int64_t n, void* stream);
int dw_pack_conv_weight(const float* w, void* wp_bf16, int D, int C, int kpad, void* stream);
int dw_unpack_conv_grad(const float* gwp, float* gw, int D, int C, int kpad, int accumulate, void* stream);

int dw_cast_f32_bf16(const float* x, void* y, int64_t n, void* stream);
int dw_cast_bf16_f32(const void* x, float* y, int64_t n, void* stream);
int dw_colsum_bf16(const void* x, int64_t ld, int rows, int cols, float* out, int accumulate, void* stream);
int dw_move_rows(const void* src, int64_t src_pitch_bytes, void* dst, int64_t dst_pitch_bytes, const int32_t* idx, int n,
                 int row_bytes, int scatter, void* stream);
int dw_add(const void* a, int a_dtype, const void* b, int b_dtype, void* y, int y_dtype, int64_t n, void* stream);

#define DW_SUMSQ_PARTIALS 2048
int dw_sumsq_f32(const float* g, int64_t n, float* out, float* partials, void* stream);
int dw_adamw(float* p, const float* g, float* m, float* v, void* shadow_bf16, int64_t n, const float* sumsq,
             float max_norm, float grad_mul, double lr, double beta1, double beta2, double eps, double weight_decay,
             int step, void* stream);
int dw_adam_tick(double* state, const float* gate, void* stream);
int dw_adamw_dev(float* p, const float* g, float* m, float* v, void* shadow_bf16, int64_t n, const float* sumsq,
                 float max_norm, float grad_mul, const double* state, double eps, double weight_decay, void* stream);

int dw_greedy_select(const void* logits, int B, int V, int64_t ld, const uint8_t* suppress,
                     const uint8_t* begin_suppress, int first, int no_eos, int forced, int ts_begin, int max_initial,
                     int64_t* tokens, int64_t tok_ld, int n, int begin_index, int eos, int fill, uint8_t* done,
                     int64_t* cur, void* stream);

typedef struct DwDecoderLayer {
    const float *ln1_g, *ln1_b;
    const void* wqkv;
    const float* bqkv;
    const void* wo;  const float* bo;
    const float *ln2_g, *ln2_b;
    const void* wq;  const float* bq;
    const void* wo2; const float* bo2;
    const float *ln3_g, *ln3_b;
    const void* w1;  const float* b1;
    const void* w2;  const float* b2;
    void* self_kv;
    const void* cross_kv;
} DwDecoderLayer;
typedef struct DwDecodeStep {
    int32_t batch, n_new;
    int32_t d_model, heads, ffn, n_layers;
    int32_t src_len, max_len;
    int32_t t;
    int32_t vocab, ldv;
    int32_t stream_dtype;
    int32_t cross_kv_ld;
    const int64_t* ids;
    const void* tok_emb;
    const void* pos_emb;
    const float *lnf_g, *lnf_b;
    const void* lm_head;
    const DwDecoderLayer* layers;
    void *x, *h, *qkv, *o, *a;
    void* logits;
} DwDecodeStep;
int dw_decode_step(const DwDecodeStep* d, void* stream);

int dw_selftest_tr16(int32_t* out, void* stream);
int dw_debug_set(int key, int value);

#ifdef __cplusplus
}
#endif
#endif
```

Baseline: 2869.

## Fuse next LayerNorm into residual GEMM epilogue via per-row-tile tickets

```diff
diff --git a/distil_whisper_amd/build.py b/distil_whisper_amd/build.py
--- a/distil_whisper_amd/build.py
+++ b/distil_whisper_amd/build.py
@@ -33,7 +33,7 @@
     hipcc = os.environ.get("HIPCC", "/opt/rocm/bin/hipcc")
     objdir = os.path.join(HERE, "build")
     os.makedirs(objdir, exist_ok=True)
-    headers = [os.path.join(CSRC, "common.h"), os.path.join(CSRC, "gemm_common.h"), os.path.join(CSRC, "gemm_kernel.h"), os.path.join(CSRC, "gemm_wp.h"), os.path.join(CSRC, "gemm_wp16.h"),
+    headers = [os.path.join(CSRC, "common.h"), os.path.join(CSRC, "gemm_common.h"), os.path.join(CSRC, "gemm_kernel.h"), os.path.join(CSRC, "gemm_wp.h"), os.path.join(CSRC, "gemm_wp16.h"), os.path.join(CSRC, "gemm_ln.h"), os.path.join(CSRC, "ln_row.h"),
                os.path.join(HERE, "..", "include", "dwamd.h")]
     objs, procs = [], []
     flags = FLAGS + (["-DDW_ABLATE"] if os.environ.get("DW_ABLATE") else [])
diff --git a/distil_whisper_amd/csrc/gemm.hip b/distil_whisper_amd/csrc/gemm.hip
--- a/distil_whisper_amd/csrc/gemm.hip
+++ b/distil_whisper_amd/csrc/gemm.hip
@@ -1,4 +1,5 @@
 #include "gemm_common.h"
+#include "gemm_ln.h"
 #include <mutex>
 #include <unordered_map>
 
@@ -38,6 +39,7 @@
 static int g_gemm_stage_next = 1;
 static int g_gemm_dynamic = 1;
 static int g_gemm_small_m = 1;
+static int g_gemm_ln_fuse = 1;
 static int g_gemm_row_tail = 1;
 
 static int* gemm_sched_slot(hipStream_t s) {
@@ -70,6 +72,7 @@
     if (key == 22) { g_gemm_row_tail = value; return DW_OK; }
     if (key == 25) { if (value < 0 || value > 1) return DW_EINVAL; g_gemm_small_m = value; return DW_OK; }
     if (key == 26) { g_attn_fwd_pipe = value; return DW_OK; }
+    if (key == 29) { if (value < 0 || value > 1) return DW_EINVAL; g_gemm_ln_fuse = value; return DW_OK; }
     if (key == 18) { g_attn_plain_order = value; return DW_OK; }
     if (key == 23) { if (value < 0 || value > 64) return DW_EINVAL; g_attn_defer = value; return DW_OK; }
     if (key == 16) { g_attn_fwd_waves = value; return DW_OK; }
@@ -186,9 +189,25 @@
     return K_TILE256;
 }
 
-extern "C" int dw_gemm_bf16(const DwGemm* g, void* stream) {
+extern "C" int dw_layernorm_fwd_ld(const void* x, int x_dtype, const float* gamma, const float* beta, void* y, float* mean,
+                                   float* rstd, int rows, int cols, float eps, int64_t ldx, int64_t ldy, void* stream);
+
+static bool gemm_ln_fusable(const DwGemm* g, const DwGemmLn* ln) {
+    if (g->n > GEMM_LN_MAXCOLS || ((uintptr_t)ln->gamma & 15) || ((uintptr_t)ln->beta & 15)) return false;
+    if (g->c_dtype == DW_F32) return (g->n & 3) == 0 && (g->ldc & 3) == 0 && (ln->ldy & 3) == 0 && ((uintptr_t)g->c & 15) == 0 && ((uintptr_t)ln->y & 7) == 0;
+    return (g->n & 7) == 0 && ((g->ldc | ln->ldy) & 7) == 0 && ((uintptr_t)g->c & 15) == 0 && ((uintptr_t)ln->y & 15) == 0;
+}
+
+static int gemm_run(const DwGemm* g, const DwGemmLn* ln, void* stream) {
     DW_CLEAR_ERR();
     if (!g || (!g->a && !g->ln_x) || !g->b || !g->c) return DW_EINVAL;
+    if (ln) {
+        if (!ln->gamma || !ln->beta || !ln->y || !ln->tickets || (ln->mean == nullptr) != (ln->rstd == nullptr)) return DW_EINVAL;
+        if (g->split_k > 1 || g->atomic_acc || g->trans_a || g->trans_b || g->ln_x || g->kv_out || g->tile == 16) return DW_EINVAL;
+        if (ln->cols != g->n || ln->rows <= 0 || ln->rows > g->m || ln->ldy < g->n || (g->n & 3) || g->n > 2048) return DW_EINVAL;
+        if ((ln->ldy & 3) || (g->ldc & 3) || ((uintptr_t)ln->y & 7)) return DW_EINVAL;
+        if ((long)ln->n_tickets * 128 < g->m) return DW_EINVAL;
+    }
     if (g->m <= 0 || g->n <= 0 || g->k <= 0 || (g->k & 63)) return DW_EINVAL;
     if ((g->lda & 7) || (g->ldb & 7)) return DW_EINVAL;
     if ((g->a && ((uintptr_t)g->a & 15)) || ((uintptr_t)g->b & 15)) return DW_EINVAL;
@@ -241,6 +260,18 @@
     hipStream_t s = (hipStream_t)stream;
     if (g->tile == 16 && !dw_gemm_skinny_ok(p, g->trans_a, g->trans_b)) return DW_EINVAL;
     const GemmKernel kern = gemm_choose(g, p);
+    if (ln) {
+        if (kern == K_SKINNY) return DW_EINVAL;
+        const bool in_kernel = (kern == K_WP8_320 || kern == K_WP8_M128 || kern == K_WP8_NN) && g_gemm_ln_fuse && gemm_ln_fusable(g, ln);
+        if (!in_kernel) {
+            const int rc = gemm_run(g, nullptr, stream);
+            if (rc != DW_OK) return rc;
+            return dw_layernorm_fwd_ld(g->c, g->c_dtype, ln->gamma, ln->beta, ln->y, ln->mean, ln->rstd, ln->rows, g->n, ln->eps, g->ldc,
+                                       ln->ldy, stream);
+        }
+        p.fln.g = ln->gamma; p.fln.b = ln->beta; p.fln.y = (bf16*)ln->y; p.fln.mean = ln->mean; p.fln.rstd = ln->rstd;
+        p.fln.tickets = ln->tickets; p.fln.ldy = ln->ldy; p.fln.rows = ln->rows; p.fln.eps = ln->eps;
+    }
     if (kern == K_SKINNY) {
         if (g->colsum_out) return DW_EINVAL;
         return dw_gemm_skinny_launch(p, s);
@@ -252,6 +283,7 @@
     if (g_gemm_dynamic) p.sched = gemm_sched_slot(s);
     if (kern == K_WP8_M128) return g->trans_b ? dw_gemm_wp8_nt128_launch(p, s) : dw_gemm_wp8_nn128_launch(p, s);
     if (g->k <= 1024) p.stage_next |= 128;
+    if (p.fln.y) p.stage_next &= ~128;
     switch (kern) {
     case K_WP16_SMALL: return g->trans_b ? dw_gemm_wp16_nt_small_launch(p, s) : dw_gemm_wp16_nn_small_launch(p, s);
     case K_WP8_320: return g->trans_b ? dw_gemm_wp8_nt320_launch(p, s) : dw_gemm_wp8_nn320_launch(p, s);
@@ -280,3 +312,9 @@
     default: return dw_gemm_tile256_launch(p, g->trans_a, g->trans_b, s);
     }
 }
+
+extern "C" int dw_gemm_bf16(const DwGemm* g, void* stream) { return gemm_run(g, nullptr, stream); }
+extern "C" int dw_gemm_bf16_ln(const DwGemm* g, const DwGemmLn* ln, void* stream) {
+    if (!ln) return DW_EINVAL;
+    return gemm_run(g, ln, stream);
+}
diff --git a/distil_whisper_amd/csrc/gemm_common.h b/distil_whisper_amd/csrc/gemm_common.h
--- a/distil_whisper_amd/csrc/gemm_common.h
+++ b/distil_whisper_amd/csrc/gemm_common.h
@@ -2,6 +2,17 @@
 #include "common.h"
 #include "../../include/dwamd.h"
 
+struct GemmLnP {
+    bf16* y = nullptr;
+    int* tickets = nullptr;
+    const float* g = nullptr;
+    const float* b = nullptr;
+    float* mean = nullptr;
+    float* rstd = nullptr;
+    long ldy = 0;
+    int rows = 0;
+    float eps = 0.f;
+};
 struct GemmP {
     const bf16* a;
     const bf16* b;
@@ -31,6 +42,7 @@
     int zg_f16;
     int* sched;
     float* colsum;
+    GemmLnP fln;
 };
 
 __device__ __forceinline__ void gemm_job_range(const GemmP& p, int& job_first, int& job_count, int& job_step) {
diff --git a/distil_whisper_amd/csrc/gemm_ln.h b/distil_whisper_amd/csrc/gemm_ln.h
--- /dev/null
+++ b/distil_whisper_amd/csrc/gemm_ln.h
@@ -0,0 +1,172 @@
+#pragma once
+#include "gemm_common.h"
+#include "ln_row.h"
+
+constexpr int GEMM_LN_MAXCOLS = 1280;
+
+typedef __attribute__((address_space(4))) const char gemm_karg_t;
+__device__ __forceinline__ gemm_karg_t* gemm_ln_kargs() {
+    gemm_karg_t* ka = (gemm_karg_t*)__builtin_amdgcn_kernarg_segment_ptr();
+    asm volatile("" : "+s"(ka));
+    return ka + offsetof(GemmP, fln);
+}
+template <class T>
+__device__ __forceinline__ T gemm_karg(gemm_karg_t* ka, size_t off) {
+    typedef const __attribute__((address_space(4))) T karg_value_t;
+    return *(karg_value_t*)(ka + off);
+}
+__device__ __forceinline__ GemmLnP gemm_ln_args() {
+    gemm_karg_t* const ka = gemm_ln_kargs();
+    GemmLnP L;
+    L.y = gemm_karg<bf16*>(ka, offsetof(GemmLnP, y));
+    L.tickets = gemm_karg<int*>(ka, offsetof(GemmLnP, tickets));
+    L.g = gemm_karg<const float*>(ka, offsetof(GemmLnP, g));
+    L.b = gemm_karg<const float*>(ka, offsetof(GemmLnP, b));
+    L.mean = gemm_karg<float*>(ka, offsetof(GemmLnP, mean));
+    L.rstd = gemm_karg<float*>(ka, offsetof(GemmLnP, rstd));
+    L.ldy = gemm_karg<long>(ka, offsetof(GemmLnP, ldy));
+    L.rows = gemm_karg<int>(ka, offsetof(GemmLnP, rows));
+    L.eps = gemm_karg<float>(ka, offsetof(GemmLnP, eps));
+    return L;
+}
+struct GemmLnHead { bf16* y; int* tickets; int rows; };
+__device__ __forceinline__ GemmLnHead gemm_ln_head() {
+    gemm_karg_t* const ka = gemm_ln_kargs();
+    GemmLnHead h;
+    h.y = gemm_karg<bf16*>(ka, offsetof(GemmLnP, y));
+    h.tickets = gemm_karg<int*>(ka, offsetof(GemmLnP, tickets));
+    h.rows = gemm_karg<int>(ka, offsetof(GemmLnP, rows));
+    return h;
+}
+
+template <int NW, int BM>
+__device__ __forceinline__ void gemm_ln_finish(const GemmP& p, char* flag_lds, int wave, int lane, int m0) {
+    typedef __attribute__((address_space(3))) volatile int lds_vint_t;
+    lds_vint_t* const flag = (lds_vint_t*)flag_lds;
+    wait_vm0();
+    __syncthreads();
+    if (threadIdx.x == 0) {
+        __builtin_amdgcn_fence(__ATOMIC_RELEASE, "agent");
+        wait_vm0();
+        int* const ticket = gemm_ln_head().tickets + m0 / BM;
+        const int t = __hip_atomic_fetch_add(ticket, 1, __ATOMIC_RELAXED, __HIP_MEMORY_SCOPE_AGENT);
+        const int last = t == p.tiles_n - 1;
+        if (last) {
+            __hip_atomic_store(ticket, 0, __ATOMIC_RELAXED, __HIP_MEMORY_SCOPE_AGENT);
+            __builtin_amdgcn_fence(__ATOMIC_ACQUIRE, "agent");
+            wait_vm0();
+        }
+        *flag = last;
+    }
+    __syncthreads();
+    if (!*flag) return;
+    const GemmLnP L = gemm_ln_args();
+
+    asm volatile("" : "+v"(lane));
+    int cols = p.n;
+    asm volatile("" : "+s"(cols));
+    int rend = m0 + BM;
+    if (rend > L.rows) rend = L.rows;
+    int row = m0 + wave;
+    if (row >= rend) return;
+    if (p.c_dtype == DW_F32) {
+        constexpr int NV = GEMM_LN_MAXCOLS / 256;
+        const int nvec = cols >> 2;
+        const float* x = (const float*)p.c;
+        f32x4 v[NV], nx[NV];
+#pragma unroll
+        for (int j = 0; j < NV; ++j) {
+            const int idx = lane + 64 * j;
+            if (idx < nvec) v[j] = *(const f32x4*)(x + (long)row * p.ldc + idx * 4);
+        }
+        for (; row < rend; row += NW) {
+            const int nrow = row + NW;
+            if (nrow < rend) {
+#pragma unroll
+                for (int j = 0; j < NV; ++j) {
+                    const int idx = lane + 64 * j;
+                    if (idx < nvec) nx[j] = *(const f32x4*)(x + (long)nrow * p.ldc + idx * 4);
+                }
+            }
+            float s = 0.f;
+#pragma unroll
+            for (int j = 0; j < NV; ++j)
+                if (lane + 64 * j < nvec) s += ln_sum4(v[j]);
+            const float mu = ln_mean(s, cols, lane);
+            float q = 0.f;
+#pragma unroll
+            for (int j = 0; j < NV; ++j)
+                if (lane + 64 * j < nvec) q = ln_sqdev4(q, v[j], mu);
+            const float rs = ln_rstd(q, cols, L.eps, lane);
+#pragma unroll
+            for (int j = 0; j < NV; ++j) {
+                const int idx = lane + 64 * j;
+                if (idx < nvec) {
+                    const f32x4 g = *(const f32x4*)(L.g + idx * 4);
+                    const f32x4 bt = *(const f32x4*)(L.b + idx * 4);
+                    ln_store<1>((bf16x4*)(L.y + (long)row * L.ldy + idx * 4), ln_out4(v[j], mu, rs, g, bt));
+                }
+            }
+            if (lane == 0 && L.mean) { L.mean[row] = mu; L.rstd[row] = rs; }
+#pragma unroll
+            for (int j = 0; j < NV; ++j) v[j] = nx[j];
+        }
+    } else {
+        constexpr int NV8 = (GEMM_LN_MAXCOLS / 8 + 63) / 64;
+        const int nvec = cols >> 3;
+        const bf16* x = (const bf16*)p.c;
+        bf16x8 t[NV8], nt[NV8];
+#pragma unroll
+        for (int j = 0; j < NV8; ++j) {
+            const int idx = lane + 64 * j;
+            if (idx < nvec) t[j] = *(const bf16x8*)(x + (long)row * p.ldc + idx * 8);
+        }
+        for (; row < rend; row += NW) {
+            const int nrow = row + NW;
+            if (nrow < rend) {
+#pragma unroll
+                for (int j = 0; j < NV8; ++j) {
+                    const int idx = lane + 64 * j;
+                    if (idx < nvec) nt[j] = *(const bf16x8*)(x + (long)nrow * p.ldc + idx * 8);
+                }
+            }
+            float v[NV8][8];
+            float s = 0.f;
+#pragma unroll
+            for (int j = 0; j < NV8; ++j) {
+                if (lane + 64 * j < nvec) {
+#pragma unroll
+                    for (int e = 0; e < 8; ++e) { v[j][e] = bf2f(t[j][e]); s += v[j][e]; }
+                }
+            }
+            const float mu = ln_mean(s, cols, lane);
+            float q = 0.f;
+#pragma unroll
+            for (int j = 0; j < NV8; ++j) {
+                if (lane + 64 * j < nvec) {
+#pragma unroll
+                    for (int e = 0; e < 8; ++e) q = ln_sqdev1(q, v[j][e], mu);
+                }
+            }
+            const float rs = ln_rstd(q, cols, L.eps, lane);
+#pragma unroll
+            for (int j = 0; j < NV8; ++j) {
+                const int idx = lane + 64 * j;
+                if (idx < nvec) {
+                    const f32x4 g0 = *(const f32x4*)(L.g + idx * 8), g1 = *(const f32x4*)(L.g + idx * 8 + 4);
+                    const f32x4 b0 = *(const f32x4*)(L.b + idx * 8), b1 = *(const f32x4*)(L.b + idx * 8 + 4);
+                    bf16x8 o;
+#pragma unroll
+                    for (int e = 0; e < 4; ++e) {
+                        o[e] = ln_out1(v[j][e], mu, rs, g0[e], b0[e]);
+                        o[e + 4] = ln_out1(v[j][e + 4], mu, rs, g1[e], b1[e]);
+                    }
+                    ln_store<1>((bf16x8*)(L.y + (long)row * L.ldy + idx * 8), o);
+                }
+            }
+            if (lane == 0 && L.mean) { L.mean[row] = mu; L.rstd[row] = rs; }
+#pragma unroll
+            for (int j = 0; j < NV8; ++j) t[j] = nt[j];
+        }
+    }
+}
diff --git a/distil_whisper_amd/csrc/gemm_wp.h b/distil_whisper_amd/csrc/gemm_wp.h
--- a/distil_whisper_amd/csrc/gemm_wp.h
+++ b/distil_whisper_amd/csrc/gemm_wp.h
@@ -1,5 +1,6 @@
 #pragma once
 #include "gemm_common.h"
+#include "gemm_ln.h"
 
 #define PINF(f) asm volatile("" : "+v"((f)[0]), "+v"((f)[1]), "+v"((f)[2]), "+v"((f)[3]))
 #define PINF2(f) asm volatile("" : "+v"((f)[0]), "+v"((f)[1]))
@@ -333,6 +334,14 @@
         }
         gemm_epilogue<FM, FN, TN, (BM == 320 ? EPF : 8), GemmNoHook, TN == 64>(p, acc, smem + (TN == 64 && STAGE >= NW * 8192 ? STAGE : 0), wave, lane, m0,
                                                                           wm0, n0, wn0, ks, GemmNoHook(), tile_in ? bias_lds : nullptr);
+        if constexpr (!TA && !TB) {
+            const GemmLnHead L = gemm_ln_head();
+            if (L.y) {
+                const int m0u = __builtin_amdgcn_readfirstlane(m0);
+                if (m0u < L.rows)
+                    gemm_ln_finish<NW, BM>(p, smem + (TN == 64 && STAGE >= NW * 8192 ? 0 : NST * STAGE - 16), wave, lane, m0u);
+            }
+        }
         gemm_lds_barrier();
         gemm_jobs_advance(jobs, job_slot);
     }
diff --git a/distil_whisper_amd/csrc/ln_row.h b/distil_whisper_amd/csrc/ln_row.h
--- /dev/null
+++ b/distil_whisper_amd/csrc/ln_row.h
@@ -0,0 +1,37 @@
+#pragma once
+#include "common.h"
+
+#ifndef DW_NT_LN
+#define DW_NT_LN 0
+#endif
+template <int LEVEL, class T>
+__device__ __forceinline__ void ln_store(T* dst, const T& v) {
+    if constexpr (LEVEL <= DW_NT_LN) __builtin_nontemporal_store(v, dst);
+    else *dst = v;
+}
+
+__device__ __forceinline__ float ln_mean(float s, int cols) { return wave_sum(s) / cols; }
+__device__ __forceinline__ float ln_rstd(float q, int cols, float eps) { return rsqrtf(wave_sum(q) / cols + eps); }
+__device__ __forceinline__ float ln_wave_sum_at(float v, int lane) {
+#pragma unroll
+    for (int o = 32; o > 0; o >>= 1) v += __int_as_float(__builtin_amdgcn_ds_bpermute((lane ^ o) << 2, __float_as_int(v)));
+    return v;
+}
+__device__ __forceinline__ float ln_mean(float s, int cols, int lane) { return ln_wave_sum_at(s, lane) / cols; }
+__device__ __forceinline__ float ln_rstd(float q, int cols, float eps, int lane) { return rsqrtf(ln_wave_sum_at(q, lane) / cols + eps); }
+
+__device__ __forceinline__ float ln_sum4(const f32x4 v) { return v[0] + v[1] + v[2] + v[3]; }
+__device__ __forceinline__ float ln_sqdev4(float q, const f32x4 v, float mu) {
+#pragma unroll
+    for (int e = 0; e < 4; ++e) { const float d = v[e] - mu; q += d * d; }
+    return q;
+}
+__device__ __forceinline__ bf16x4 ln_out4(const f32x4 v, float mu, float rs, const f32x4 g, const f32x4 bt) {
+    bf16x4 o;
+#pragma unroll
+    for (int e = 0; e < 4; ++e) o[e] = f2bf((v[e] - mu) * rs * g[e] + bt[e]);
+    return o;
+}
+
+__device__ __forceinline__ float ln_sqdev1(float q, float v, float mu) { const float d = v - mu; return q + d * d; }
+__device__ __forceinline__ bf16 ln_out1(float v, float mu, float rs, float g, float bt) { return f2bf((v - mu) * rs * g + bt); }
diff --git a/distil_whisper_amd/csrc/norm.hip b/distil_whisper_amd/csrc/norm.hip
--- a/distil_whisper_amd/csrc/norm.hip
+++ b/distil_whisper_amd/csrc/norm.hip
@@ -1,4 +1,5 @@
 #include "common.h"
+#include "ln_row.h"
 #include "../../include/dwamd.h"
 
 #define LN_MAXV 8
@@ -33,18 +34,10 @@
     }
 }
 
-#ifndef DW_NT_LN
-#define DW_NT_LN 0
-#endif
 template <class T>
 __device__ __forceinline__ T ln_load_in(const T* src) {
     if constexpr (DW_NT_LN_IN != 0) return __builtin_nontemporal_load(src);
     else return *src;
-}
-template <int LEVEL, class T>
-__device__ __forceinline__ void ln_store(T* dst, const T& v) {
-    if constexpr (LEVEL <= DW_NT_LN) __builtin_nontemporal_store(v, dst);
-    else *dst = v;
 }
 
 template <bool XBF, int NV>
@@ -61,32 +54,26 @@
         const int idx = lane + 64 * j;
         if (idx < nvec) {
             v[j] = ld4<XBF>(x, (long)row * ldx + idx * 4);
-            s += v[j][0] + v[j][1] + v[j][2] + v[j][3];
-        }
-    }
-    s = wave_sum(s);
-    const float mu = s / cols;
+            s += ln_sum4(v[j]);
+        }
+    }
+    const float mu = ln_mean(s, cols);
     float q = 0.f;
 #pragma unroll
     for (int j = 0; j < NV; ++j) {
         const int idx = lane + 64 * j;
         if (idx < nvec) {
-#pragma unroll
-            for (int e = 0; e < 4; ++e) { const float d = v[j][e] - mu; q += d * d; }
-        }
-    }
-    q = wave_sum(q);
-    const float rs = rsqrtf(q / cols + eps);
+            q = ln_sqdev4(q, v[j], mu);
+        }
+    }
+    const float rs = ln_rstd(q, cols, eps);
 #pragma unroll
     for (int j = 0; j < NV; ++j) {
         const int idx = lane + 64 * j;
         if (idx < nvec) {
             const f32x4 g = *(const f32x4*)(gamma + idx * 4);
             const f32x4 bt = *(const f32x4*)(beta + idx * 4);
-            bf16x4 o;
-#pragma unroll
-            for (int e = 0; e < 4; ++e) o[e] = f2bf((v[j][e] - mu) * rs * g[e] + bt[e]);
-            ln_store<1>((bf16x4*)(y + (long)row * ldy + idx * 4), o);
+            ln_store<1>((bf16x4*)(y + (long)row * ldy + idx * 4), ln_out4(v[j], mu, rs, g, bt));
         }
     }
     if (lane == 0 && mean) { mean[row] = mu; rstd[row] = rs; }
@@ -118,28 +105,22 @@
         float s = 0.f;
 #pragma unroll
         for (int j = 0; j < NV; ++j)
-            if (lane + 64 * j < nvec) s += v[j][0] + v[j][1] + v[j][2] + v[j][3];
-        s = wave_sum(s);
-        const float mu = s / cols;
+            if (lane + 64 * j < nvec) s += ln_sum4(v[j]);
+        const float mu = ln_mean(s, cols);
         float q = 0.f;
 #pragma unroll
         for (int j = 0; j < NV; ++j)
             if (lane + 64 * j < nvec) {
-#pragma unroll
-                for (int e = 0; e < 4; ++e) { const float d = v[j][e] - mu; q += d * d; }
-            }
-        q = wave_sum(q);
-        const float rs = rsqrtf(q / cols + eps);
+                q = ln_sqdev4(q, v[j], mu);
+            }
+        const float rs = ln_rstd(q, cols, eps);
 #pragma unroll
         for (int j = 0; j < NV; ++j) {
             const int idx = lane + 64 * j;
             if (idx < nvec) {
                 const f32x4 g = *(const f32x4*)(gamma + idx * 4);
                 const f32x4 bt = *(const f32x4*)(beta + idx * 4);
-                bf16x4 o;
-#pragma unroll
-                for (int e = 0; e < 4; ++e) o[e] = f2bf((v[j][e] - mu) * rs * g[e] + bt[e]);
-                ln_store<1>((bf16x4*)(y + (long)row * ldy + idx * 4), o);
+                ln_store<1>((bf16x4*)(y + (long)row * ldy + idx * 4), ln_out4(v[j], mu, rs, g, bt));
             }
         }
         if (lane == 0 && mean) { mean[row] = mu; rstd[row] = rs; }
@@ -166,19 +147,17 @@
             for (int e = 0; e < 8; ++e) { v[j][e] = bf2f(t[e]); s += v[j][e]; }
         }
     }
-    s = wave_sum(s);
-    const float mu = s / cols;
+    const float mu = ln_mean(s, cols);
     float q = 0.f;
 #pragma unroll
     for (int j = 0; j < NV8; ++j) {
         const int idx = lane + 64 * j;
         if (idx < nvec) {
 #pragma unroll
-            for (int e = 0; e < 8; ++e) { const float d = v[j][e] - mu; q += d * d; }
-        }
-    }
-    q = wave_sum(q);
-    const float rs = rsqrtf(q / cols + eps);
+            for (int e = 0; e < 8; ++e) q = ln_sqdev1(q, v[j][e], mu);
+        }
+    }
+    const float rs = ln_rstd(q, cols, eps);
 #pragma unroll
     for (int j = 0; j < NV8; ++j) {
         const int idx = lane + 64 * j;
@@ -188,8 +167,8 @@
             bf16x8 o;
 #pragma unroll
             for (int e = 0; e < 4; ++e) {
-                o[e] = f2bf((v[j][e] - mu) * rs * g0[e] + b0[e]);
-                o[e + 4] = f2bf((v[j][e + 4] - mu) * rs * g1[e] + b1[e]);
+                o[e] = ln_out1(v[j][e], mu, rs, g0[e], b0[e]);
+                o[e + 4] = ln_out1(v[j][e + 4], mu, rs, g1[e], b1[e]);
             }
             ln_store<1>((bf16x8*)(y + (long)row * ldy + idx * 8), o);
         }
diff --git a/distil_whisper_amd/engine.py b/distil_whisper_amd/engine.py
--- a/distil_whisper_amd/engine.py
+++ b/distil_whisper_amd/engine.py
@@ -280,6 +280,27 @@
                                            self.st.p[f"{name}.bias"], 1e-5, save_stats=save, out=y[:R])
         return y, mu, rs
 
+    fuse_gemm_ln = 0
+
+    def _fuse_ln(self, M, N):
+        if not self.fuse_gemm_ln or not getattr(self.ops, "gemm_ln", False):
+            return False
+        if self.ops.pick_tile(M, N) == 128:
+            return bool(self.fuse_gemm_ln & 4)
+        return bool(self.fuse_gemm_ln & (1 if self.stream == torch.float32 else 2))
+
+    def _ln_req(self, name, cols, R, save, rows_alloc=None, zero_pad=None, pad=0):
+        y = self.act(R if rows_alloc is None else rows_alloc, cols, zero_pad=save if zero_pad is None else zero_pad, pad=pad)
+        return y, (self.st.p[f"{name}.weight"], self.st.p[f"{name}.bias"], 1e-5, y[:R], save)
+
+    def _gemm_ln(self, fuse, spec, R, save, a, w, **kw):
+        if not fuse or spec is None:
+            return self.ops.gemm(a, w, **kw), None
+        name, rows_alloc, zero_pad, pad = spec
+        y, req = self._ln_req(name, w.shape[0], R, save, rows_alloc, zero_pad, pad)
+        x, (_, mu, rs) = self.ops.gemm(a, w, ln_next=req, **kw)
+        return x, (y, mu, rs)
+
     def _ln_bwd(self, name, dy, x, mu, rs, dres, R, emit=False, colsum_to=None):
         if self.st.is_trainable(f"{name}.weight"):
             dg, db = self.st.g[f"{name}.weight"], self.st.g[f"{name}.bias"]
@@ -386,16 +407,19 @@
             ctx.update(xcol1=xcol1, z1=z1, xcol2=xcol2, z2=z2)
         else:
             del xcol1, a1, z1, xcol2, z2
+        hn = None
         for i in range(d.enc_layers):
-            x, lc = self._layer_fwd(f"model.encoder.layers.{i}", x, B, L, None, 0, False, save)
+            nxt = (f"model.encoder.layers.{i + 1}.self_attn_layer_norm", R, None, self.row_pad) if i + 1 < d.enc_layers else \
+                ("model.encoder.layer_norm", None, True, 0)
+            x, lc, hn = self._layer_fwd(f"model.encoder.layers.{i}", x, B, L, None, 0, False, save, h_in=hn, next_ln=nxt)
             if save:
                 ctx["layers"].append(lc)
-        y, mu, rs = self._ln("model.encoder.layer_norm", x, R, save, zero_pad=True)
+        y, mu, rs = hn if hn is not None else self._ln("model.encoder.layer_norm", x, R, save, zero_pad=True)
         if save:
             ctx.update(x_final=x, mu=mu, rs=rs, enc_out=y)
         return y, ctx
 
-    def _layer_fwd(self, p, x, B, L, enc_out, Lk, causal, save, Rg=None, live=None):
+    def _layer_fwd(self, p, x, B, L, enc_out, Lk, causal, save, Rg=None, live=None, h_in=None, next_ln=None):
         ops, st, d = self.ops, self.st, self.dims
         D, H, Rp = d.d_model, d.heads, B * L
         R = Rp if live is None else live.n
@@ -436,7 +460,8 @@
             ops.gather_rows(op, live.idx, o)
             return o, None
         av = st.attn_views(f"{p}.self_attn")
-        h, mu, rs = self._ln(f"{p}.self_attn_layer_norm", x, R, save, Rg, pad=self.row_pad)
+        fuse = self._fuse_ln(Rg, D)
+        h, mu, rs = h_in if h_in is not None else self._ln(f"{p}.self_attn_layer_norm", x, R, save, Rg, pad=self.row_pad)
         qkv = self.act(Rg, 3 * D, zero_pad=save, pad=self.row_pad)
         ops.gemm(h[:Rg], av["wqkv"], bias=av["bqkv"], out=qkv[:Rg])
         if live is None:
@@ -444,7 +469,9 @@
         else:
             o, lse = attend(qkv, None, None, L, causal, 3 * D)
         xp = self.stream_row_pad // (4 if self.stream == torch.float32 else 2)
-        x1 = ops.gemm(o[:Rg], av["wo"], bias=av["bo"], residual=x, round_res=True, out_dtype=self.stream, out_row_pad=xp)
+        ln2 = f"{p}.encoder_attn_layer_norm" if enc_out is not None else f"{p}.final_layer_norm"
+        x1, hn = self._gemm_ln(fuse, (ln2, Rg, None, self.row_pad), R, save, o[:Rg], av["wo"], bias=av["bo"], residual=x, round_res=True,
+                               out_dtype=self.stream, out_row_pad=xp)
         if save:
             lc.update(x0=x, mu0=mu, rs0=rs, h0=h, qkv=qkv, o0=o, lse0=lse)
             if live is not None:
@@ -453,29 +480,30 @@
         if enc_out is not None:
             cv = st.attn_views(f"{p}.encoder_attn")
             Re = B * Lk
-            h, mu, rs = self._ln(f"{p}.encoder_attn_layer_norm", x, R, save, Rg, pad=self.row_pad)
+            h, mu, rs = hn if hn is not None else self._ln(f"{p}.encoder_attn_layer_norm", x, R, save, Rg, pad=self.row_pad)
             q = self.act(Rg, D, zero_pad=save, pad=self.row_pad)
             ops.gemm(h[:Rg], cv["wqkv"][:D], bias=cv["bqkv"][:D], out=q[:Rg])
             kv = self.act(Re, 2 * D, zero_pad=save, pad=self.row_pad)
             ops.gemm(enc_out[:Re], cv["wqkv"][D:], bias=cv["bqkv"][D:], out=kv[:Re])
             o, lse = attend(q, kv[:Re, :D], kv[:Re, D:], Lk, False, D)
-            x1 = ops.gemm(o[:Rg], cv["wo"], bias=cv["bo"], residual=x, round_res=True, out_dtype=self.stream, out_row_pad=xp)
+            x1, hn = self._gemm_ln(fuse, (f"{p}.final_layer_norm", Rg, None, self.row_pad), R, save, o[:Rg], cv["wo"], bias=cv["bo"],
+                                   residual=x, round_res=True, out_dtype=self.stream, out_row_pad=xp)
             if save:
                 lc.update(x1=x, mu1=mu, rs1=rs, h1=h, q1=q, kv1=kv, o1=o, lse1=lse)
                 if live is not None:
                     lc.update(q1_r=rect["x"][0], o1_r=rect["x"][1])
             x = x1
-        h, mu, rs = self._ln(f"{p}.final_layer_norm", x, R, save, Rg, pad=self.row_pad)
+        h, mu, rs = hn if hn is not None else self._ln(f"{p}.final_layer_norm", x, R, save, Rg, pad=self.row_pad)
         a = self.act(Rg, d.ffn, zero_pad=save, pad=self.ffn_row_pad)
         res = ops.gemm(h[:Rg], st.s[f"{p}.fc1.weight"], bias=st.p[f"{p}.fc1.bias"], act=1,
                        want_z=("grad" if self.ffn_keeps_gelu_grad else True) if save else False, out=a[:Rg],
                        z_row_pad=self.ffn_row_pad)
         z = res[1] if save else None
-        x2 = ops.gemm(a[:Rg], st.s[f"{p}.fc2.weight"], bias=st.p[f"{p}.fc2.bias"], residual=x, round_res=True,
-                      out_dtype=self.stream, out_row_pad=xp)
+        x2, hn = self._gemm_ln(fuse, next_ln, R, save, a[:Rg], st.s[f"{p}.fc2.weight"], bias=st.p[f"{p}.fc2.bias"], residual=x,
+                               round_res=True, out_dtype=self.stream, out_row_pad=xp)
         if save:
             lc.update(x2=x, mu2=mu, rs2=rs, h2=h, a=a, z=z)
-        return x2, lc
+        return x2, lc, hn
 
     def decode(self, ids, enc_out, save=False, live=None):
         ops, st, d = self.ops, self.st, self.dims
@@ -501,17 +529,20 @@
             xp, x = x, ops.empty((Rg, d.d_model), self.stream)
             ops.gather_rows(xp, live.idx, x)
             del xp
-        for i in range(d.dec_layers):
-            x, lc = self._layer_fwd(f"model.decoder.layers.{i}", x, B, T, enc_out, Lk, True, save, Rg,
-                                    live if packed else None)
-            if save:
-                ctx["layers"].append(lc)
         Rh = live.n if live is not None else R
         Rl = Rh
         if save and self.pad_lm_rows and Rh >= self.pad_gemm_rows_min:
             Rl = _rup(Rh, 320)
             Rl = Rl if Rl - Rh <= Rh * self.pad_gemm_rows_slack else Rh
-        hf, mu, rs = self._ln("model.decoder.layer_norm", x, Rv, save, max(Rl, Rv))
+        hn = None
+        for i in range(d.dec_layers):
+            nxt = (f"model.decoder.layers.{i + 1}.self_attn_layer_norm", Rg, None, self.row_pad) if i + 1 < d.dec_layers else \
+                ("model.decoder.layer_norm", max(Rl, Rv), None, 0)
+            x, lc, hn = self._layer_fwd(f"model.decoder.layers.{i}", x, B, T, enc_out, Lk, True, save, Rg,
+                                        live if packed else None, h_in=hn, next_ln=nxt)
+            if save:
+                ctx["layers"].append(lc)
+        hf, mu, rs = hn if hn is not None else self._ln("model.decoder.layer_norm", x, Rv, save, max(Rl, Rv))
         if live is not None and save and not packed:
             hfp, hf = hf, self.act(Rl, d.d_model)
             ops.gather_rows(hfp, live.idx, hf)
diff --git a/distil_whisper_amd/ops_hip.py b/distil_whisper_amd/ops_hip.py
--- a/distil_whisper_amd/ops_hip.py
+++ b/distil_whisper_amd/ops_hip.py
@@ -28,6 +28,14 @@
     ]
 
 
+class DwGemmLn(C.Structure):
+    _fields_ = [
+        ("gamma", C.c_void_p), ("beta", C.c_void_p), ("y", C.c_void_p), ("mean", C.c_void_p), ("rstd", C.c_void_p),
+        ("tickets", C.c_void_p), ("ldy", C.c_int64), ("rows", C.c_int32), ("cols", C.c_int32), ("n_tickets", C.c_int32),
+        ("eps", C.c_float),
+    ]
+
+
 class DwDecoderLayer(C.Structure):
     _fields_ = [(n, C.c_void_p) for n in (
         "ln1_g", "ln1_b", "wqkv", "bqkv", "wo", "bo", "ln2_g", "ln2_b", "wq", "bq", "wo2", "bo2", "ln3_g", "ln3_b",
@@ -47,6 +55,7 @@
     "dw_logmel": ([C.c_void_p, C.c_int, C.c_int, C.c_void_p, C.c_int, C.c_void_p, C.c_void_p, C.c_void_p, C.c_void_p,
                    C.c_void_p], C.c_int),
     "dw_gemm_bf16": ([C.POINTER(DwGemm), C.c_void_p], C.c_int),
+    "dw_gemm_bf16_ln": ([C.POINTER(DwGemm), C.POINTER(DwGemmLn), C.c_void_p], C.c_int),
     "dw_layernorm_fwd": ([C.c_void_p, C.c_int, C.c_void_p, C.c_void_p, C.c_void_p, C.c_void_p, C.c_void_p, C.c_int,
                           C.c_int, C.c_float, C.c_void_p], C.c_int),
     "dw_layernorm_bwd": ([C.c_void_p, C.c_void_p, C.c_int, C.c_void_p, C.c_void_p, C.c_void_p, C.c_void_p, C.c_int,
@@ -139,6 +148,8 @@
         self.profile = None
         self._prof_events = []
         self.profile_detail = False
+        self._ln_ticket_pool = [self.zeros((self.LN_TICKETS,), torch.int32) for _ in range(4)]
+        self._ln_tickets = {}
 
     def _stream(self):
         return C.c_void_p(torch.cuda.current_stream(self.device).cuda_stream)
@@ -179,6 +190,17 @@
         t256 = ((M + 255) // 256) * ((N + 255) // 256)
         return 256 if t256 >= 512 else 128
 
+    gemm_ln = True
+    LN_TICKETS = 4096
+
+    def _tickets(self):
+        key = torch.cuda.current_stream(self.device).cuda_stream
+        t = self._ln_tickets.get(key)
+        if t is None:
+            t = self._ln_ticket_pool.pop() if self._ln_ticket_pool else self.zeros((self.LN_TICKETS,), torch.int32)
+            self._ln_tickets[key] = t
+        return t
+
     wgrad_slab_pad = 0
 
     def empty(self, shape, dtype):
@@ -205,7 +227,7 @@
 
     def gemm(self, a, b, *, trans_a=False, trans_b=False, bias=None, act=0, want_z=False, zgrad=None, residual=None,
              r_row_mod=0, round_res=True, out_dtype=None, out=None, tile=0, atomic_acc=False, split_k=0, ln=None,
-             kv_append=None, colsum=None, z_row_pad=0, out_row_pad=0, overwrite=False):
+             kv_append=None, colsum=None, z_row_pad=0, out_row_pad=0, overwrite=False, ln_next=None):
         assert b.dtype == torch.bfloat16 and (a.dtype == torch.bfloat16 or ln is not None)
         assert a.stride(1) == 1 and b.stride(1) == 1
         if trans_a:
@@ -293,7 +315,26 @@
             g.r_row_mod = int(r_row_mod)
             g.round_res = int(bool(round_res))
         e0 = self._t0()
-        self._chk(self.lib.dw_gemm_bf16(C.byref(g), self._stream()), f"gemm m={M} n={N} k={K} ta={trans_a} tb={trans_b}")
+        lnr = None
+        if ln_next is not None:
+            gamma, beta, eps, y, save_stats = ln_next
+            rows = y.shape[0]
+            assert not atomic_acc and ln is None and kv_append is None and not trans_a and not trans_b
+            assert gamma.dtype == torch.float32 and beta.dtype == torch.float32 and gamma.numel() == N == beta.numel()
+            assert y.dtype == torch.bfloat16 and y.shape == (rows, N) and y.stride(1) == 1 and 0 < rows <= M
+            mean = self.empty((rows,), torch.float32) if save_stats else None
+            rstd = self.empty((rows,), torch.float32) if save_stats else None
+            tk = self._tickets()
+            gl = DwGemmLn()
+            gl.gamma, gl.beta, gl.y, gl.mean, gl.rstd = gamma.data_ptr(), beta.data_ptr(), y.data_ptr(), _p(mean), _p(rstd)
+            gl.tickets, gl.n_tickets, gl.ldy, gl.rows, gl.cols, gl.eps = tk.data_ptr(), tk.numel(), y.stride(0), rows, N, float(eps)
+            rc = self.lib.dw_gemm_bf16_ln(C.byref(g), C.byref(gl), self._stream())
+            if rc != 0:
+                tk.zero_()
+            self._chk(rc, f"gemm+ln m={M} n={N} k={K} rows={rows}")
+            lnr = (y, mean, rstd)
+        else:
+            self._chk(self.lib.dw_gemm_bf16(C.byref(g), self._stream()), f"gemm m={M} n={N} k={K} ta={trans_a} tb={trans_b}")
         if ws is not None:
             self._chk(self.lib.dw_reduce_slices_ld(ws.data_ptr(), g.slice_stride, g.ldc, g.split_k, out.data_ptr(), out.stride(0),
                                                    M, N, 0 if overwrite else 1, self._stream()), "reduce_slices")
@@ -305,6 +346,8 @@
                     f"{' r' + ('f32' if residual.dtype == torch.float32 else 'bf16') if residual is not None else ''}"
                     f"{' sk%d' % g.split_k if g.split_k else ''}")
         self._t1(e0, key, 2.0 * M * N * K)
+        if lnr is not None:
+            return (out, z, lnr) if want_z else (out, lnr)
         return (out, z) if want_z else out
 
     def decode_pass(self, desc):
diff --git a/include/dwamd.h b/include/dwamd.h
--- a/include/dwamd.h
+++ b/include/dwamd.h
@@ -49,6 +49,20 @@
     float* colsum_out;
 } DwGemm;
 int dw_gemm_bf16(const DwGemm* g, void* stream);
+typedef struct DwGemmLn {
+    const float* gamma;
+    const float* beta;
+    void* y;
+    float* mean;
+    float* rstd;
+    int32_t* tickets;
+    int64_t ldy;
+    int32_t rows;
+    int32_t cols;
+    int32_t n_tickets;
+    float eps;
+} DwGemmLn;
+int dw_gemm_bf16_ln(const DwGemm* g, const DwGemmLn* ln, void* stream);
 int dw_reduce_slices(const float* part, int64_t stride, int slices, float* out, int64_t n, int accumulate, void* stream);
 int dw_reduce_slices_ld(const float* part, int64_t slice_stride, int64_t ld_part, int slices, float* out, int64_t ld_out,
                         int rows, int cols, int accumulate, void* stream);
```

Result: no change. 2867 (median of 2 runs) (-0.1%).
